# YangHai-1218/RADet

Hardware: AMD Instinct MI355X
Metric: images/sec train-step, r50_ycbv_pbr 640x480 bs=4/GPU (higher is better)
Workload: dtype f32

## Files before the change

### include/radet_hip.h

```cpp
#ifndef RADET_HIP_H
#define RADET_HIP_H
#include <stdint.h>

#ifdef __cplusplus
extern "C" {
#endif


typedef struct RadetConvDesc {
    const float* w;
    const float* bias;
    const float* bn_gamma;
    const float* bn_beta;
    const float* bn_mean;
    const float* bn_var;
    float* wf;
    float* wft;
    float* bias_f;
    const float* dwf_slabs;
    const float* dbias_partials;
    float* dw;
    float* dbias;
    float* dgamma;
    float* dbeta;
// ... 124 lines not shown
                     void* stream);

int radet_gn_workspace_floats(int B, const int* seg_desc, int nseg);
int radet_gn_relu_fwd(const float* z, const float* gamma, const float* beta, float* y, float* stats ,
                      float* partial_ws, int B, int C, int groups, float eps, int relu, const int* seg_desc, int nseg,
                      void* stream);
int radet_gn_relu_bwd(const float* dy, const float* z, const float* stats, const float* gamma, const float* beta,
                      float* dz, float* dgamma, float* dbeta, float* partial_ws, int B, int C, int groups, int relu,
                      const int* seg_desc, int nseg, void* stream);

int radet_upsample_add(float* dst, const float* src, int B, int Ho, int Wo, int Hi, int Wi, int C, void* stream);
int radet_upsample_add_bwd(float* dsrc, const float* ddst, int B, int Ho, int Wo, int Hi, int Wi, int C, void* stream);
int radet_relu_bwd(const float* dy, const float* addend, const float* act, float* dx, size_t n, void* stream);
int radet_stem_conv_bn_relu_h(const float* img_nchw, const float* wf_ohwi, const float* bias, void* y_nhwc, int B, int H,
                              int W, void* stream);
int radet_maxpool3x3s2_h(const void* x, void* y, int B, int H, int W, int C, void* stream);
int radet_gn_relu_fwd_pair(const float* z0, const float* gamma0, const float* beta0, float* y0, float* stats0,
                           float* partial_ws0, const float* z1, const float* gamma1, const float* beta1, float* y1,
                           float* stats1, float* partial_ws1, int B, int C, int groups, float eps, int relu,
                           const int* seg_desc, int nseg, void* stream);
int radet_gn_relu_fwd_pair_h(const void* z0, const float* gamma0, const float* beta0, void* y0, float* stats0,
                             float* partial_ws0, const void* z1, const float* gamma1, const float* beta1, void* y1,
                             float* stats1, float* partial_ws1, int B, int C, int groups, float eps, int relu,
                             const int* seg_desc, int nseg, void* stream);
int radet_gn_relu_fwd_h(const void* z, const float* gamma, const float* beta, void* y, float* stats, float* partial_ws,
                        int B, int C, int groups, float eps, int relu, const int* seg_desc, int nseg, void* stream);
int radet_gn_relu_bwd_h(const void* dy, const void* z, const float* stats, const float* gamma, const float* beta, void* dz,
                        float* dgamma, float* dbeta, float* partial_ws, int B, int C, int groups, int relu,
                        const int* seg_desc, int nseg, void* stream);
int radet_upsample_add_h(void* dst, const void* src, int B, int Ho, int Wo, int Hi, int Wi, int C, void* stream);
int radet_upsample_add_bwd_h(void* dsrc, const void* ddst, int B, int Ho, int Wo, int Hi, int Wi, int C, void* stream);
int radet_relu_bwd_h(const void* dy, const void* addend, const void* act, void* dx, size_t n, void* stream);
int radet_convert_rows(const void* src, void* dst, size_t rows, int ncols, int src_ld, int src_off, int dst_ld,
                       int dst_off, int to_bf16, void* stream);
int radet_split_planes(const float* src, void* dst_planes, size_t rows, int C, int src_ld, void* stream);
int radet_merge_planes(const void* src_planes, float* dst, size_t rows, int C, int dst_ld, void* stream);
int radet_split_pairs(const float* src, void* dst_pairs, size_t rows, int C, int src_ld, const void* src_amax, void* dst_amax,
                      void* stream);
int radet_merge_pairs(const void* src_pairs, float* dst, size_t rows, int C, int dst_ld, const void* amax, void* stream);
int radet_gn_relu_fwd_q(const float* z, const float* gamma, const float* beta, float* y, void* yq, float* stats,
                        float* partial_ws, int B, int C, int groups, float eps, int relu, const int* seg_desc, int nseg,
                        void* stream, void* y_amax, void* yq_amax, void* zhat_amax);
int radet_gn_relu_fwd_pair_q(const float* z0, const float* gamma0, const float* beta0, float* y0, void* yq0, float* stats0,
                             float* partial_ws0, void* y_amax0, void* yq_amax0, void* zhat_amax0, const float* z1,
                             const float* gamma1, const float* beta1, float* y1, void* yq1, float* stats1,
                             float* partial_ws1, void* y_amax1, void* yq_amax1, void* zhat_amax1, int B, int C, int groups,
                             float eps, int relu, const int* seg_desc, int nseg, void* stream);
int radet_gn_relu_bwd_q(const float* dy, const float* z, const float* stats, const float* gamma, const float* beta, float* dz,
                        void* dzq, float* dgamma, float* dbeta, float* partial_ws, int B, int C, int groups, int relu,
                        const int* seg_desc, int nseg, void* stream, const void* dy_amax, const void* zhat_amax,
                        void* dzq_amax);
int radet_maxpool3x3s2_a(const float* x, float* y, int B, int H, int W, int C, void* y_amax, void* stream);
int radet_maxpool3x3s2_q(const float* x, float* y, int B, int H, int W, int C, void* y_amax, void* yq, void* yq_amax,
                         const void* x_amax, void* stream);
int radet_stem_conv_bn_relu_a(const float* img_nchw, const float* wf_ohwi, const float* bias, float* y_nhwc, int B, int H, int W,
                              void* y_amax, void* stream);
int radet_upsample_add_a(float* dst, const float* src, int B, int Ho, int Wo, int Hi, int Wi, int C, void* dst_amax,
                         void* stream);
int radet_upsample_add_bwd_a(float* dsrc, const float* ddst, int B, int Ho, int Wo, int Hi, int Wi, int C, void* dsrc_amax,
                             void* stream);
int radet_relu_bwd_a(const float* dy, const float* addend, const float* act, float* dx, size_t n, void* dx_amax, void* stream);
int radet_absmax(const float* x, size_t n, void* amax, void* stream);
int radet_amax_slot_words(void);
int radet_gn_relu_fwd_p(const float* z, const float* gamma, const float* beta, float* y, void* yp, float* stats,
                        float* partial_ws, int B, int C, int groups, float eps, int relu, const int* seg_desc, int nseg,
                        void* stream);
int radet_gn_relu_fwd_pair_p(const float* z0, const float* gamma0, const float* beta0, float* y0, void* yp0, float* stats0,
                             float* partial_ws0, const float* z1, const float* gamma1, const float* beta1, float* y1,
                             void* yp1, float* stats1, float* partial_ws1, int B, int C, int groups, float eps, int relu,
                             const int* seg_desc, int nseg, void* stream);
int radet_gn_relu_bwd_p(const float* dy, const float* z, const float* stats, const float* gamma, const float* beta,
                        float* dz, void* dzp, float* dgamma, float* dbeta, float* partial_ws, int B, int C, int groups,
                        int relu, const int* seg_desc, int nseg, void* stream);
int radet_nchw_to_nhwc(const float* x, float* y, int B, int C, int H, int W, void* stream);
int radet_nhwc_to_nchw(const float* x, float* y, int B, int C, int H, int W, void* stream);

int radet_head_loss_ws_ints(int R);
int radet_head_loss(const float* cls, const float* reg_u, const float* iou, const float* scales,
                    const float* gt_boxes, const int64_t* gt_labels, const int* gt_off, const int64_t* p2g,
                    const float* pw, const int* level_desc, int nlvl, int B, int num_classes, float alpha,
                    float gamma, float loss_bbox_weight, float giou_eps, const float* grad_scale, float* losses,
                    float* dcls, int dcls_ld, float* dreg_u, int dreg_ld, float* diou, int diou_ld, float* dscales,
                    int64_t* labels_out, float* bbox_targets_out, int flags, int* ws, void* stream);
int radet_scale_relu(const float* reg_u, const float* scales, float* out, const int* level_desc, int nlvl, int B,
                     void* stream);

size_t radet_decode_ws_bytes(int B, int nlvl, int nms_pre);
int radet_decode_candidates(const float* cls, const float* reg_u, const float* iou, const float* scales,
                            const int* level_desc, int nlvl, int B, int num_classes, float score_thr, int nms_pre,
                            const float* img_hw , const float* scale_factor ,
                            float* cand_boxes, float* cand_scores, float* cand_ctr, int64_t* cand_labels,
                            int* cand_count, void* ws, void* stream);

size_t radet_nms_ws_bytes(int B, int cap);
int radet_nms(const float* boxes, const float* cluster_scores, const float* vote_scores, const int64_t* labels,
              const int* counts, int B, int cap, int mode, float iou_thr, int iou_enable, float sigma, int max_out,
              float* out_boxes, float* out_scores, int64_t* out_labels, int* out_count, int64_t* aux0, int64_t* aux1,
              void* ws, void* stream);

size_t radet_assign_ws_bytes(int B, int N);
int radet_assign_points(const float* gt_boxes, const int* gt_off, const uint8_t* masks, int H, int W,
                        const uint32_t* rng_words, int U, const int* level_desc, const float* regress_ranges ,
                        int nlvl, int B, int positive_num, int flags, float neg_threshold, int64_t* p2g, float* pw, int* used,
                        void* ws, void* stream);

int radet_assign_points_f(const float* gt_boxes, const int* gt_off, const float* distance_maps, int H, int W,
                          const uint32_t* rng_words, int U, const int* level_desc, const float* regress_ranges ,
                          int nlvl, int B, int positive_num, int flags, float neg_threshold, int64_t* p2g, float* pw, int* used,
                          void* ws, void* stream);

size_t radet_mbd_ws_bytes(size_t total_px);
int radet_mbd(const uint8_t* images, const int* img_desc_dev, int nimg, const int* seeds_x, const int* seeds_y, float alpha,
              int niter, int base_size, double* dmap, size_t total_px, void* ws, void* stream);
int radet_gdt(const float* cost, const int* img_desc_dev, int nimg, const int* seeds_x, const int* seeds_y, float* dist,
              void* ws_labels , void* stream);

int radet_resize_linear_u8(const uint8_t* src, const int* src_desc, uint8_t* dst, const int* dst_desc, int ncrop,
                           int max_dst_px, int channels, void* stream);
int radet_resize_linear_f(const void* src, const int* src_desc, void* dst, const int* dst_desc, int ncrop, int max_dst_px,
                          int is_f64, void* stream);
#define RESIZE_WIN_DESC_INTS 7
int radet_resize_linear_u8_window(const uint8_t* src, const int* src_desc, uint8_t* dst, const int* win_desc, int ncrop,
                                  int max_dst_px, int channels, void* stream);
#define RESIZE_SRC_WIN_DESC_INTS 8
int radet_resize_linear_u8_src_window(const uint8_t* src, const int* src_desc, uint8_t* dst, const int* win_desc, int ncrop,
                                      int max_dst_px, int channels, void* stream);
int radet_gaussian_blur9_u8(const uint8_t* src, const int* desc, uint8_t* dst, float* tmp, const float* kernel5, int ncrop,
                            int max_px, void* stream);
int radet_sobel_edge(const uint8_t* src, const int* desc, float* edge, uint8_t* gray_ws, uint32_t* max_ws, int ncrop,
                     int max_px, void* stream);

int radet_mask_max(const uint8_t* masks, uint32_t* maxes , int G, size_t hw, void* stream);
int radet_mask_transform(const uint8_t* src, uint8_t* dst, const uint32_t* norm_max, int G, int Hs, int Ws, int Hr, int Wr,
                         int Hd, int Wd, int flip, int pad_val, void* stream);
#define MASK_WIN_INTS 7
int radet_mask_transform_window(const uint8_t* src, uint8_t* dst, const uint32_t* norm_max, const int* win_desc, int G, int Hs,
                                int Ws, int Hd, int Wd, int pad_val, void* stream);
#define MASK_SRC_WIN_INTS 7
int radet_mask_transform_src_window(const uint8_t* src, uint8_t* dst, const uint32_t* norm_max, const int* win_desc, int G, int Hs,
                                    int Ws, int Hd, int Wd, int pad_val, void* stream);

#define RLE_MASK_INTS 5
#define RLE_PART_INTS 2
int radet_rle_masks(const uint32_t* run_ends, int n_ends, const int* part_desc, int n_parts, const int* mask_desc, int G,
                    uint8_t* dst, uint8_t* dst_plain, int Hr, int Wr, int Hd, int Wd, int pad_val, void* stream);
int radet_rle_masks_window(const uint32_t* run_ends, int n_ends, const int* part_desc, int n_parts, const int* mask_desc,
                           const int* win_desc, int G, uint8_t* dst, uint8_t* dst_plain, int Hd, int Wd, int pad_val, void* stream);
int radet_rle_masks_src_window(const uint32_t* run_ends, int n_ends, const int* part_desc, int n_parts, const int* mask_desc,
                               const int* win_desc, int G, uint8_t* dst, uint8_t* dst_plain, int Hd, int Wd, int pad_val,
                               void* stream);

#define JPEG_ROW_INTS 8
#define JPEG_DESC_INTS 20
#define JPEG_HUFF_BYTES 1424
int radet_jpeg_index(const uint8_t* file, int scan_lo, int scan_hi, int ncomp, const int* comp_blocks, const void* huff,
                     int n_mcus, int restart_interval, int seg_mcus, int* rows, int max_rows);
int radet_jpeg_decode(const uint8_t* files, const int* desc, int nimg, const int* wgs, int n_wg, const void* huff,
                      const uint16_t* quant, const int* rows, int n_rows, int16_t* coef, uint8_t* planes, uint8_t* dst,
                      int* err, int max_blocks, int max_px, int stages, void* stream);

#define AUG_PARAM_INTS 16
#define AUG_MAX_W 8192
int radet_augment_merge_hblur(const uint8_t* src, const uint8_t* bg, const int* params, uint8_t* dst, int nimg, int max_h,
                              int max_w, void* stream);
int radet_augment_vblur(const uint8_t* src, const int* params, uint8_t* dst, int nimg, int max_h, int max_w, void* stream);
int radet_augment_sharp(const uint8_t* src, const int* params, uint8_t* dst, unsigned long long* lsum, int nimg, int max_px,
// ... 101 lines not shown
```

### radet_amd/_lib.py

```python
import ctypes as C
import os

_HERE = os.path.dirname(os.path.abspath(__file__))
LIB_PATH = os.path.join(_HERE, os.environ.get("RADET_LIB", "libradet_hip.so"))

_p = C.c_void_p
_i = C.c_int
_f = C.c_float
_sz = C.c_size_t


class RadetConvDesc(C.Structure):
    _fields_ = [("w", _p), ("bias", _p), ("bn_gamma", _p), ("bn_beta", _p), ("bn_mean", _p), ("bn_var", _p),
                ("wf", _p), ("wft", _p), ("bias_f", _p), ("dwf_slabs", _p), ("dbias_partials", _p),
                ("dw", _p), ("dbias", _p), ("dgamma", _p), ("dbeta", _p),
                ("cout", _i), ("cin", _i), ("kh", _i), ("kw", _i), ("nsplit", _i), ("eps", _f),
                ("wft_ld", _i), ("wft_off", _i), ("w16", _i), ("w_amax", _p), ("wfq", _p), ("w_l1", _p), ("bias_amax", _p),
                ("w_l1t", _p)]


class RadetScales(C.Structure):
    _fields_ = [("x_amax", _p), ("w_amax", _p), ("y_amax", _p), ("x1_amax", _p), ("w1_amax", _p), ("y1_amax", _p),
                ("yq", _p), ("yq_amax", _p), ("x_true_amax", _p), ("w_l1", _p), ("bias_amax", _p), ("addend_amax", _p)]


class RadetWgradJob(C.Structure):
    _fields_ = [("dy", _p), ("x", _p), ("slabs", _p), ("dbias_partials", _p), ("gather_table", _p),
                ("M", _i), ("Cin", _i), ("Cout", _i), ("ld_dy", _i), ("KH", _i), ("KW", _i), ("S", _i)]


class RadetTapeOp(C.Structure):
    _fields_ = [("kind", C.c_int32), ("fn", C.c_int32), ("stream", _p), ("event", _p), ("args", C.c_uint64 * 32)]


SIGNATURES = {
    "radet_gather_table_rows": (_i, [_i]),
    "radet_build_gather_table": (_i, [_p, _i, _i, _i, _i, _i, _i, _i, _p, _i, _p]),
    "radet_conv2d_igemm": (_i, [_p, _p, _p, _p, _p, _p, _p, _i, _i, _i, _i, _i, _i, _i, _p, _sz, _p]),
    "radet_conv2d_igemm_pair": (_i, [_p] * 13 + [_i, _i, _i, _i, _i, _i, _i, _p, _sz, _p]),
    "radet_conv2d_igemm_taps": (_i, [_p, _p, _p, _p, _p, _p, _p, _p, _i, _i, _i, _i, _i, _i, _p, _sz, _p]),
    "radet_conv2d_igemm_classes": (_i, [_p, _p, _p, _p, _p, _p, _p, _p, _p, _p, _i, _i, _i, _i, _i, _i, _p, _sz, _p]),
    "radet_conv2d_igemm_s": (_i, [_p, _p, _p, _p, _p, _p, _p, _i, _i, _i, _i, _i, _i, _i, _p, _sz, _p, _p]),
    "radet_conv2d_igemm_pair_s": (_i, [_p] * 13 + [_i, _i, _i, _i, _i, _i, _i, _p, _sz, _p, _p]),
    "radet_conv2d_igemm_taps_s": (_i, [_p, _p, _p, _p, _p, _p, _p, _p, _i, _i, _i, _i, _i, _i, _p, _sz, _p, _p]),
    "radet_conv2d_igemm_classes_s": (_i, [_p, _p, _p, _p, _p, _p, _p, _p, _p, _p, _i, _i, _i, _i, _i, _i, _p, _sz, _p, _p]),
    "radet_conv2d_wgrad_s": (_i, [_p, _p, _p, _p, _p, _i, _i, _i, _i, _i, _i, _i, _i, _p, _p]),
    "radet_split_pairs": (_i, [_p, _p, _sz, _i, _i, _p, _p, _p]),
    "radet_merge_pairs": (_i, [_p, _p, _sz, _i, _i, _p, _p]),
    "radet_gn_relu_fwd_q": (_i, [_p, _p, _p, _p, _p, _p, _p, _i, _i, _i, _f, _i, _p, _i, _p, _p, _p, _p]),
    "radet_gn_relu_fwd_pair_q": (_i, [_p] * 20 + [_i, _i, _i, _f, _i, _p, _i, _p]),
    "radet_gn_relu_bwd_q": (_i, [_p, _p, _p, _p, _p, _p, _p, _p, _p, _p, _i, _i, _i, _i, _p, _i, _p, _p, _p, _p]),
    "radet_maxpool3x3s2_a": (_i, [_p, _p, _i, _i, _i, _i, _p, _p]),
    "radet_maxpool3x3s2_q": (_i, [_p, _p, _i, _i, _i, _i, _p, _p, _p, _p, _p]),
    "radet_stem_conv_bn_relu_a": (_i, [_p, _p, _p, _p, _i, _i, _i, _p, _p]),
    "radet_upsample_add_a": (_i, [_p, _p, _i, _i, _i, _i, _i, _i, _p, _p]),
    "radet_upsample_add_bwd_a": (_i, [_p, _p, _i, _i, _i, _i, _i, _i, _p, _p]),
    "radet_relu_bwd_a": (_i, [_p, _p, _p, _p, _sz, _p, _p]),
    "radet_absmax": (_i, [_p, _sz, _p, _p]),
    "radet_amax_slot_words": (_i, []),
    "radet_pred3x3_patch": (_i, [_p, _i, _p, _i, _p, _p, _p, _i, _p, _p, _p, _i, _p]),
    "radet_conv2d_wgrad_splits": (_i, [_i, _i, _i, _i, _i]),
    "radet_conv2d_wgrad": (_i, [_p, _p, _p, _p, _p, _i, _i, _i, _i, _i, _i, _i, _i, _p]),
    "radet_conv2d_wgrad_group": (_i, [_p, _i, _i, _p]),
    "radet_fold_weights": (_i, [_p, _i, _p]),
    "radet_unfold_grads": (_i, [_p, _i, _i, _p]),
    "radet_stem_conv_bn_relu": (_i, [_p, _p, _p, _p, _i, _i, _i, _p]),
    "radet_maxpool3x3s2": (_i, [_p, _p, _i, _i, _i, _i, _p]),
    "radet_maxpool3x3s2_bwd_relu": (_i, [_p, _p, _p, _i, _i, _i, _i, _p]),
    "radet_stem_wgrad_splits": (_i, [_i, _i, _i]),
    "radet_stem_wgrad": (_i, [_p, _p, _p, _p, _i, _i, _i, _i, _p]),
    "radet_gn_workspace_floats": (_i, [_i, _p, _i]),
    "radet_gn_relu_fwd": (_i, [_p, _p, _p, _p, _p, _p, _i, _i, _i, _f, _i, _p, _i, _p]),
    "radet_gn_relu_fwd_pair": (_i, [_p] * 12 + [_i, _i, _i, _f, _i, _p, _i, _p]),
    "radet_gn_relu_fwd_pair_h": (_i, [_p] * 12 + [_i, _i, _i, _f, _i, _p, _i, _p]),
    "radet_gn_relu_bwd": (_i, [_p, _p, _p, _p, _p, _p, _p, _p, _p, _i, _i, _i, _i, _p, _i, _p]),
    "radet_upsample_add": (_i, [_p, _p, _i, _i, _i, _i, _i, _i, _p]),
    "radet_upsample_add_bwd": (_i, [_p, _p, _i, _i, _i, _i, _i, _i, _p]),
    "radet_relu_bwd": (_i, [_p, _p, _p, _p, _sz, _p]),
    "radet_nchw_to_nhwc": (_i, [_p, _p, _i, _i, _i, _i, _p]),
    "radet_nhwc_to_nchw": (_i, [_p, _p, _i, _i, _i, _i, _p]),
    "radet_head_loss_ws_ints": (_i, [_i]),
    "radet_head_loss": (_i, [_p, _p, _p, _p, _p, _p, _p, _p, _p, _p, _i, _i, _i, _f, _f, _f, _f, _p, _p, _p, _i, _p,
                             _i, _p, _i, _p, _p, _p, _i, _p, _p]),
    "radet_scale_relu": (_i, [_p, _p, _p, _p, _i, _i, _p]),
    "radet_decode_ws_bytes": (_sz, [_i, _i, _i]),
    "radet_decode_candidates": (_i, [_p, _p, _p, _p, _p, _i, _i, _i, _f, _i, _p, _p, _p, _p, _p, _p, _p, _p, _p]),
    "radet_nms_ws_bytes": (_sz, [_i, _i]),
    "radet_nms": (_i, [_p, _p, _p, _p, _p, _i, _i, _i, _f, _i, _f, _i, _p, _p, _p, _p, _p, _p, _p, _p]),
    "radet_assign_ws_bytes": (_sz, [_i, _i]),
    "radet_assign_points": (_i, [_p, _p, _p, _i, _i, _p, _i, _p, _p, _i, _i, _i, _i, _f, _p, _p, _p, _p, _p]),
    "radet_assign_points_f": (_i, [_p, _p, _p, _i, _i, _p, _i, _p, _p, _i, _i, _i, _i, _f, _p, _p, _p, _p, _p]),
    "radet_resize_linear_u8": (_i, [_p, _p, _p, _p, _i, _i, _i, _p]),
    "radet_resize_linear_u8_window": (_i, [_p, _p, _p, _p, _i, _i, _i, _p]),
    "radet_resize_linear_u8_src_window": (_i, [_p, _p, _p, _p, _i, _i, _i, _p]),
    "radet_resize_linear_f": (_i, [_p, _p, _p, _p, _i, _i, _i, _p]),
    "radet_warp_affine_u8": (_i, [_p, _sz, _p, _sz, _p, _i, _i, _i, _p]),
    "radet_gaussian_blur9_u8": (_i, [_p, _p, _p, _p, _p, _i, _i, _p]),
    "radet_sobel_edge": (_i, [_p, _p, _p, _p, _p, _i, _i, _p]),
    "radet_stem_conv_bn_relu_h": (_i, [_p, _p, _p, _p, _i, _i, _i, _p]),
    "radet_maxpool3x3s2_h": (_i, [_p, _p, _i, _i, _i, _i, _p]),
    "radet_gn_relu_fwd_h": (_i, [_p, _p, _p, _p, _p, _p, _i, _i, _i, _f, _i, _p, _i, _p]),
    "radet_gn_relu_bwd_h": (_i, [_p, _p, _p, _p, _p, _p, _p, _p, _p, _i, _i, _i, _i, _p, _i, _p]),
    "radet_upsample_add_h": (_i, [_p, _p, _i, _i, _i, _i, _i, _i, _p]),
    "radet_upsample_add_bwd_h": (_i, [_p, _p, _i, _i, _i, _i, _i, _i, _p]),
    "radet_relu_bwd_h": (_i, [_p, _p, _p, _p, _sz, _p]),
    "radet_convert_rows": (_i, [_p, _p, _sz, _i, _i, _i, _i, _i, _i, _p]),
    "radet_split_planes": (_i, [_p, _p, _sz, _i, _i, _p]),
    "radet_merge_planes": (_i, [_p, _p, _sz, _i, _i, _p]),
    "radet_gn_relu_fwd_p": (_i, [_p, _p, _p, _p, _p, _p, _p, _i, _i, _i, _f, _i, _p, _i, _p]),
    "radet_gn_relu_fwd_pair_p": (_i, [_p] * 14 + [_i, _i, _i, _f, _i, _p, _i, _p]),
    "radet_gn_relu_bwd_p": (_i, [_p, _p, _p, _p, _p, _p, _p, _p, _p, _p, _i, _i, _i, _i, _p, _i, _p]),
    "radet_mbd_ws_bytes": (_sz, [_sz]),
    "radet_mbd": (_i, [_p, _p, _i, _p, _p, _f, _i, _i, _p, _sz, _p, _p]),
    "radet_gdt": (_i, [_p, _p, _i, _p, _p, _p, _p, _p]),
    "radet_mask_max": (_i, [_p, _p, _i, _sz, _p]),
    "radet_mask_transform": (_i, [_p, _p, _p, _i, _i, _i, _i, _i, _i, _i, _i, _i, _p]),
    "radet_mask_transform_window": (_i, [_p, _p, _p, _p, _i, _i, _i, _i, _i, _i, _p]),
    "radet_mask_transform_src_window": (_i, [_p, _p, _p, _p, _i, _i, _i, _i, _i, _i, _p]),
    "radet_rle_masks": (_i, [_p, _i, _p, _i, _p, _i, _p, _p, _i, _i, _i, _i, _i, _p]),
    "radet_rle_masks_window": (_i, [_p, _i, _p, _i, _p, _p, _i, _p, _p, _i, _i, _i, _p]),
    "radet_rle_masks_src_window": (_i, [_p, _i, _p, _i, _p, _p, _i, _p, _p, _i, _i, _i, _p]),
    "radet_jpeg_index": (_i, [_p, _i, _i, _i, _p, _p, _i, _i, _i, _p, _i]),
    "radet_jpeg_decode": (_i, [_p, _p, _i, _p, _i, _p, _p, _p, _i, _p, _p, _p, _p, _i, _i, _i, _p]),
    "radet_augment_merge_hblur": (_i, [_p, _p, _p, _p, _i, _i, _i, _p]),
    "radet_augment_vblur": (_i, [_p, _p, _p, _i, _i, _i, _p]),
    "radet_augment_sharp": (_i, [_p, _p, _p, _p, _i, _i, _p]),
    "radet_augment_finish": (_i, [_p, _p, _p, _p, _i, _i, _i, _f, _f, _f, _f, _f, _f, _p]),
    "radet_augment_hsv_noise": (_i, [_p, _p, _p, _i, _i, _p]),
    "radet_augment_box": (_i, [_p, _p, _p, _sz, _i, _i, _i, _p]),
    "radet_crop_canvases": (_i, [_p, _sz, _p, _p, _i, _p, _i, _i, _p, _sz, _p]),
    "radet_paste_maps": (_i, [_p, _sz, _i, _p, _i, _i, _i, _p, _p]),
    "radet_preprocess_frames": (_i, [_p, _i, _i, _i, _f, _f, _f, _f, _f, _f, _p, _p]),
    "radet_grid_anchors": (_i, [_p, _p, _i, _i, _p]),
    "radet_bbox_overlaps": (_i, [_p, _p, _p, _i, _i, _i, _i, _i, _f, _p]),
    "radet_tblr_encode": (_i, [_p, _p, _p, _i, _p, _i, _p]),
    "radet_tblr_decode": (_i, [_p, _p, _p, _i, _p, _i, _f, _f, _i, _p]),
    "radet_loss_partials": (_i, [_sz]),
    "radet_loss_finalize": (_i, [_p, _i, _p, _f, _p, _p]),
    "radet_sigmoid_focal_loss": (_i, [_p, _p, _p, _i, _sz, _i, _f, _f, _p, _f, _p, _p]),
    "radet_sigmoid_focal_loss_bwd": (_i, [_p, _p, _p, _i, _sz, _i, _f, _f, _p, _p, _p, _f, _p, _p]),
    "radet_bce_logits_loss": (_i, [_p, _p, _p, _i, _sz, _i, _p, _f, _p, _p]),
    "radet_bce_logits_loss_bwd": (_i, [_p, _p, _p, _i, _sz, _i, _p, _p, _p, _f, _p, _p]),
    "radet_giou_loss": (_i, [_p, _p, _p, _sz, _f, _p, _f, _p, _p]),
    "radet_giou_loss_bwd": (_i, [_p, _p, _p, _sz, _f, _p, _p, _p, _f, _p, _p]),
    "radet_threshold_compact": (_i, [_p, _sz, _f, _p, _p, _p]),
    "radet_sqnorm_partials": (_i, [_p, _sz, _p, _i, _p]),
    "radet_adamw_step": (_i, [_p, _p, _p, _p, _sz, _f, _f, _f, _f, _f, _i, _f, _f, _p, _i, _p, _p]),
    "radet_coco_match": (_i, [_p, _p, _p, _p, _p, _p, _i, _i, _p, _i, _p, _i, _p, _p, _p, _p, _p]),
    "radet_coco_accumulate": (_i, [_p, _p, _p, _p, _p, _p, _p, _p, _i, _i, _i, _i, _i, _p, _p, _p, _p]),
    "radet_tape_fn_index": (_i, [C.c_char_p]),
    "radet_tape_replay": (_i, [_p, _i, _i, _p]),
    "radet_fill_zero": (_i, [_p, _sz, _p]),
    "radet_copy_d2d": (_i, [_p, _p, _sz, _p]),
    "radet_stream_create_cumask": (_i, [_p, _i, _p]),
    "radet_copy_segments": (_i, [_p, _i, _i, _p]),
}

_lib = None


class RadetHipError(RuntimeError):
    pass


def load():
    global _lib
# ... 41 lines not shown
```

### radet_amd/csrc/loss.hip

```cpp
#include "common.h"
#include "../../include/radet_hip.h"

struct LossLevels {
    int n;
    int h[RADET_MAX_SEG], w[RADET_MAX_SEG], stride[RADET_MAX_SEG];
    int row_off[RADET_MAX_SEG + 1];
    int pt_off[RADET_MAX_SEG + 1];
};

struct RowInfo { int lvl, n, pix, pt; float cx, cy, stride; };

__device__ __forceinline__ RowInfo decode_row(const LossLevels& L, int r) {
    RowInfo o;
    int l = 0;
#pragma unroll
    for (int i = 1; i < RADET_MAX_SEG; ++i)
        if (i < L.n && r >= L.row_off[i]) l = i;
    const int hw = L.h[l] * L.w[l];
    const int local = r - L.row_off[l];
    o.lvl = l;
    o.n = local / hw;
    o.pix = local - o.n * hw;
    o.pt = L.pt_off[l] + o.pix;
    const int iy = o.pix / L.w[l], ix = o.pix - iy * L.w[l];
// ... 26 lines not shown
        const int G = gt_off[ri.n + 1] - gt_off[ri.n];
        const int64_t g = p2g[(size_t)ri.n * N + ri.pt];
        int64_t lab = num_classes;
        if (G > 0 && g > -1) lab = gt_labels[gt_off[ri.n] + (g == 0 ? G - 1 : (int)g - 1)];
        if (labels_out) labels_out[r] = lab;
        if (tgt_out) {
            float4 t = make_float4(0.f, 0.f, 0.f, 0.f);
            if (G > 0 && g > 0) {
                const float* gb = gt_boxes + (size_t)(gt_off[ri.n] + (int)g - 1) * 4;
                const float hw8 = 8.f * ri.stride;
                t.x = (ri.cy - gb[1]) / hw8 / 0.125f;
                t.y = (gb[3] - ri.cy) / hw8 / 0.125f;
                t.z = (ri.cx - gb[0]) / hw8 / 0.125f;
                t.w = (gb[2] - ri.cx) / hw8 / 0.125f;
            }
            *reinterpret_cast<float4*>(tgt_out + (size_t)r * 4) = t;
        }
        if (lab >= 0 && lab < num_classes) {
            pos = true;
            w = pw[(size_t)ri.n * N + ri.pt];
        }
    }
    const unsigned long long bal = __ballot(pos);
    const int before = __popcll(bal & ((1ull << lane) - 1ull));
    const float wsum = wave_sum(w);
    __shared__ int wc[LP_BLK / 64];
    __shared__ float ww[LP_BLK / 64];
    if (lane == 0) { wc[wave] = __popcll(bal); ww[wave] = wsum; }
    __syncthreads();
    int base = 0;
    for (int i = 0; i < wave; ++i) base += wc[i];
    int* scratch = lp_scratch(ws, R);
    const int nb = lp_blocks(R);
    if (pos) scratch[blockIdx.x * LP_BLK + base + before] = r;
    if (tid == 0) {
        scratch[nb * LP_BLK + blockIdx.x] = (wc[0] + wc[1]) + (wc[2] + wc[3]);
        scratch[nb * LP_BLK + nb + blockIdx.x] = __float_as_int((ww[0] + ww[1]) + (ww[2] + ww[3]));
    }
}

__global__ __launch_bounds__(1024) void loss_prep_scan_kernel(int R, int* __restrict__ ws) {
    const int tid = threadIdx.x;
    const int nb = lp_blocks(R);
    const int* scratch = lp_scratch(ws, R);
    const int* bcnt = scratch + nb * LP_BLK;
    const int* bw = bcnt + nb;
    const int per = (nb + 1023) / 1024;
    const int b0 = tid * per, b1 = min(nb, b0 + per);
    int cnt = 0;
    float wsum = 0.f;
    for (int b = b0; b < b1; ++b) {
        cnt += bcnt[b];
        wsum += __int_as_float(bw[b]);
    }
    __shared__ int scnt[1024];
    __shared__ float swt[1024];
    scnt[tid] = cnt;
    swt[tid] = wsum;
    __syncthreads();
    for (int o = 1; o < 1024; o <<= 1) {
        const int v = tid >= o ? scnt[tid - o] : 0;
        __syncthreads();
        scnt[tid] += v;
        __syncthreads();
    }
    for (int o = 512; o > 0; o >>= 1) {
        if (tid < o) swt[tid] += swt[tid + o];
        __syncthreads();
    }
    int pos = scnt[tid] - cnt;
    for (int b = b0; b < b1; ++b) {
        const int n = bcnt[b];
        for (int i = 0; i < n; ++i) ws[WS_HDR + pos + i] = scratch[b * LP_BLK + i];
        pos += n;
    }
    if (tid == 0) {
        ws[0] = scnt[1023];
        ws[1] = __float_as_int(swt[0]);
    }
}

__device__ __forceinline__ float softplus_f(float x) { return fmaxf(x, 0.f) + log1pf(expf(-fabsf(x))); }

__global__ __launch_bounds__(256) void focal_kernel(const float* __restrict__ cls, const int64_t* __restrict__ gt_labels,
                                                    const int* __restrict__ gt_off, const int64_t* __restrict__ p2g,
                                                    const float* __restrict__ pw, const LossLevels L, int B, int N,
                                                    int R, int C, float alpha, float gamma,
                                                    const float* __restrict__ grad_scale, float* __restrict__ dcls,
                                                    int dcls_ld, int* __restrict__ ws) {
    const float num_pos = __int_as_float(ws[1]);
    const float avg = num_pos + (float)B;
    const float gs = (grad_scale ? grad_scale[0] : 1.f) / avg;
    const size_t total = (size_t)R * C;
    float acc = 0.f;
    for (size_t i = (size_t)blockIdx.x * 256 + threadIdx.x; i < total; i += (size_t)gridDim.x * 256) {
        const int r = (int)(i / C);
        const int c = (int)(i - (size_t)r * C);
        const RowInfo ri = decode_row(L, r);
        const int G = gt_off[ri.n + 1] - gt_off[ri.n];
        const int64_t g = p2g[(size_t)ri.n * N + ri.pt];
        int64_t lab = C;
        if (G > 0 && g > -1) lab = gt_labels[gt_off[ri.n] + (g == 0 ? G - 1 : (int)g - 1)];
        const float wt = pw[(size_t)ri.n * N + ri.pt];
        const float x = cls[i];
        const float p = 1.f / (1.f + expf(-x));
        float loss, dx;
        if (lab == c) {
            const float q = 1.f - p;
            const float logp = -softplus_f(-x);
            const float mod = gamma == 2.f ? q * q : powf(q, gamma);
            loss = -alpha * mod * logp;
            dx = alpha * mod * (gamma * p * logp - q);
        } else {
            const float log1mp = -softplus_f(x);
            const float mod = gamma == 2.f ? p * p : powf(p, gamma);
            loss = -(1.f - alpha) * mod * log1mp;
            dx = (1.f - alpha) * mod * (p - gamma * (1.f - p) * log1mp);
        }
        acc += loss * wt;
        dcls[(size_t)r * dcls_ld + c] = dx * wt * gs;
    }
    __shared__ float red[4];
    acc = wave_sum(acc);
    if ((threadIdx.x & 63) == 0) red[threadIdx.x >> 6] = acc;
    __syncthreads();
    if (threadIdx.x == 0) ws[WS_HDR + R + blockIdx.x] = __float_as_int((red[0] + red[1]) + (red[2] + red[3]));
}

struct PosTerms { float w, one_minus_giou, bce, pwt; };

__device__ __forceinline__ float sel_gt(float a, float b) { return a > b ? 1.f : (a == b ? 0.5f : 0.f); }
__device__ __forceinline__ float sel_lt(float a, float b) { return a < b ? 1.f : (a == b ? 0.5f : 0.f); }

template <int NT>
__device__ __forceinline__ float block_sum(float v, float* red) {
    const int tid = threadIdx.x;
    __syncthreads();
    red[tid] = v;
    __syncthreads();
    for (int o = NT / 2; o > 0; o >>= 1) {
        if (tid < o) red[tid] += red[tid + o];
        __syncthreads();
    }
    const float r = red[0];
    __syncthreads();
    return r;
}

__global__ __launch_bounds__(256) void pos_loss_kernel(const float* __restrict__ reg_u, const float* __restrict__ iou_logit,
                                                       const float* __restrict__ scales,
                                                       const float* __restrict__ gt_boxes,
                                                       const int* __restrict__ gt_off, const int64_t* __restrict__ p2g,
                                                       const float* __restrict__ pw, const LossLevels L, int B, int N,
                                                       int R, float lbw, float eps, const float* __restrict__ grad_scale,
                                                       float* __restrict__ losses, float* __restrict__ dreg_u,
                                                       int dreg_ld, float* __restrict__ diou, int diou_ld,
                                                       float* __restrict__ dscales, const int* __restrict__ ws,
                                                       int n_focal_partials, int postact) {
    __shared__ float red[256];
    const int tid = threadIdx.x;
    const int P = ws[0];
    const float num_pos = __int_as_float(ws[1]);
    {
        double a = 0.0;
        for (int k = tid; k < n_focal_partials; k += 256) a += (double)__int_as_float(ws[WS_HDR + R + k]);
        const float s = block_sum<256>((float)a, red);
        if (tid == 0) losses[0] = s / (num_pos + (float)B);
    }
    if (!(num_pos > 0.f)) {
        if (tid == 0) { losses[1] = 0.f; losses[2] = 0.f; }
        if (tid < L.n) dscales[tid] = 0.f;
        return;
    }
    float sw = 0.f, swl = 0.f, sb = 0.f, sp = 0.f;
    for (int pass = 0; pass < 2; ++pass) {
        float inv_sw = 0.f, inv_sp = 0.f, g1 = 1.f, g2 = 1.f;
        float ds[RADET_MAX_SEG];
#pragma unroll
        for (int l = 0; l < RADET_MAX_SEG; ++l) ds[l] = 0.f;
        if (pass == 1) {
            inv_sw = 1.f / sw;
            inv_sp = 1.f / sp;
            if (grad_scale) { g1 = grad_scale[1]; g2 = grad_scale[2]; }
        }
        for (int k = tid; k < P; k += 256) {
            const int r = ws[WS_HDR + k];
            const RowInfo ri = decode_row(L, r);
            const int64_t g = p2g[(size_t)ri.n * N + ri.pt];
            const float pwt = pw[(size_t)ri.n * N + ri.pt];
            const float sc = scales[ri.lvl];
            const float4 u = *reinterpret_cast<const float4*>(reg_u + (size_t)r * 4);
            const float v0 = u.x * sc, v1 = u.y * sc, v2 = u.z * sc, v3 = u.w * sc;
            const float p0 = postact ? v0 : fmaxf(v0, 0.f), p1 = postact ? v1 : fmaxf(v1, 0.f);
            const float p2 = postact ? v2 : fmaxf(v2, 0.f), p3 = postact ? v3 : fmaxf(v3, 0.f);
            float t0 = 0.f, t1 = 0.f, t2 = 0.f, t3 = 0.f;
            if (g > 0) {
                const float* gb = gt_boxes + (size_t)(gt_off[ri.n] + (int)g - 1) * 4;
                const float hw8 = 8.f * ri.stride;
                t0 = (ri.cy - gb[1]) / hw8 / 0.125f;
                t1 = (gb[3] - ri.cy) / hw8 / 0.125f;
                t2 = (ri.cx - gb[0]) / hw8 / 0.125f;
                t3 = (gb[2] - ri.cx) / hw8 / 0.125f;
            }
            const float hw8 = 8.f * ri.stride;
            const float px1 = ri.cx - p2 * 0.125f * hw8, py1 = ri.cy - p0 * 0.125f * hw8;
            const float px2 = ri.cx + p3 * 0.125f * hw8, py2 = ri.cy + p1 * 0.125f * hw8;
            const float tx1 = ri.cx - t2 * 0.125f * hw8, ty1 = ri.cy - t0 * 0.125f * hw8;
            const float tx2 = ri.cx + t3 * 0.125f * hw8, ty2 = ri.cy + t1 * 0.125f * hw8;
            const float area1 = (px2 - px1) * (py2 - py1), area2 = (tx2 - tx1) * (ty2 - ty1);
            const float ltx = fmaxf(px1, tx1), lty = fmaxf(py1, ty1), rbx = fminf(px2, tx2), rby = fminf(py2, ty2);
            const float dw = rbx - ltx, dh = rby - lty;
            const float iw = fmaxf(dw, 0.f), ih = fmaxf(dh, 0.f);
            const float I = iw * ih;
            const float Uraw = area1 + area2 - I;
            const float U = fmaxf(Uraw, eps);
            const float iou = I / U;
            const float eltx = fminf(px1, tx1), elty = fminf(py1, ty1), erbx = fmaxf(px2, tx2), erby = fmaxf(py2, ty2);
            const float dew = erbx - eltx, deh = erby - elty;
            const float ew = fmaxf(dew, 0.f), eh = fmaxf(deh, 0.f);
            const float Eraw = ew * eh;
            const float E = fmaxf(Eraw, eps);
            const float giou = iou - (E - U) / E;
            const float wgt = fmaxf(iou, 1e-12f) * pwt;
            const float x = iou_logit[r];
            if (pass == 0) {
                sw += wgt;
                swl += wgt * (1.f - giou);
                sb += pwt * (fmaxf(x, 0.f) - x * iou + log1pf(expf(-fabsf(x))));
                sp += pwt;
            } else {
                const float gg = -lbw * wgt * inv_sw * g1;
                const float g_E = -gg * U / (E * E);
                float g_U = gg / E - gg * I / (U * U);
                float g_I = gg / U;
                const float g_Uraw = g_U * sel_gt(Uraw, eps);
                const float g_area1 = g_Uraw;
                g_I -= g_Uraw;
                const float g_dw = g_I * ih * (dw >= 0.f ? 1.f : 0.f);
                const float g_dh = g_I * iw * (dh >= 0.f ? 1.f : 0.f);
                const float g_Eraw = g_E * sel_gt(Eraw, eps);
                const float g_dew = g_Eraw * eh * (dew >= 0.f ? 1.f : 0.f);
                const float g_deh = g_Eraw * ew * (deh >= 0.f ? 1.f : 0.f);
                float gx1 = -g_dw * sel_gt(px1, tx1) - g_dew * sel_lt(px1, tx1) - g_area1 * (py2 - py1);
                float gy1 = -g_dh * sel_gt(py1, ty1) - g_deh * sel_lt(py1, ty1) - g_area1 * (px2 - px1);
                float gx2 = g_dw * sel_lt(px2, tx2) + g_dew * sel_gt(px2, tx2) + g_area1 * (py2 - py1);
                float gy2 = g_dh * sel_lt(py2, ty2) + g_deh * sel_gt(py2, ty2) + g_area1 * (px2 - px1);
                const float k8 = 0.125f * hw8;
                const float gp0 = -gy1 * k8, gp1 = gy2 * k8, gp2 = -gx1 * k8, gp3 = gx2 * k8;
                const float gv0 = (postact || p0 > 0.f) ? gp0 : 0.f, gv1 = (postact || p1 > 0.f) ? gp1 : 0.f;
                const float gv2 = (postact || p2 > 0.f) ? gp2 : 0.f, gv3 = (postact || p3 > 0.f) ? gp3 : 0.f;
                float4 du;
                du.x = gv0 * sc; du.y = gv1 * sc; du.z = gv2 * sc; du.w = gv3 * sc;
                *reinterpret_cast<float4*>(dreg_u + (size_t)r * dreg_ld) = du;
                const float dsv = (gv0 * u.x + gv1 * u.y) + (gv2 * u.z + gv3 * u.w);
#pragma unroll
                for (int l = 0; l < RADET_MAX_SEG; ++l)
                    if (l == ri.lvl) ds[l] += dsv;
                const float sig = 1.f / (1.f + expf(-x));
                diou[(size_t)r * diou_ld] = pwt * (sig - iou) * inv_sp * g2;
            }
        }
        if (pass == 0) {
            sw = block_sum<256>(sw, red);
            swl = block_sum<256>(swl, red);
            sb = block_sum<256>(sb, red);
            sp = block_sum<256>(sp, red);
            if (tid == 0) {
                losses[1] = lbw * swl / sw;
                losses[2] = sb / sp;
            }
        } else {
#pragma unroll
            for (int l = 0; l < RADET_MAX_SEG; ++l) {
                if (l < L.n) {
                    const float s = block_sum<256>(ds[l], red);
                    if (tid == 0) dscales[l] = s;
                }
            }
        }
    }
}

__global__ void zero_sparse_kernel(float* __restrict__ dreg, int dreg_ld, float* __restrict__ diou, int diou_ld, int R) {
    const int r = blockIdx.x * blockDim.x + threadIdx.x;
    if (r < R) {
        *reinterpret_cast<float4*>(dreg + (size_t)r * dreg_ld) = make_float4(0.f, 0.f, 0.f, 0.f);
        diou[(size_t)r * diou_ld] = 0.f;
    }
}

static int fill_levels(LossLevels* L, const int* level_desc, int nlvl, int B) {
    if (nlvl < 1 || nlvl > RADET_MAX_SEG) return RADET_ERR_ARG;
    L->n = nlvl;
    int row = 0, pt = 0;
    for (int l = 0; l < nlvl; ++l) {
        L->h[l] = level_desc[3 * l];
        L->w[l] = level_desc[3 * l + 1];
        L->stride[l] = level_desc[3 * l + 2];
        L->row_off[l] = row;
        L->pt_off[l] = pt;
        row += B * L->h[l] * L->w[l];
        pt += L->h[l] * L->w[l];
    }
    L->row_off[nlvl] = row;
    L->pt_off[nlvl] = pt;
    for (int l = nlvl; l < RADET_MAX_SEG; ++l) { L->h[l] = 1; L->w[l] = 1; L->stride[l] = 1; }
    return RADET_OK;
}

#define FOCAL_BLOCKS 1024

static_assert(FOCAL_BLOCKS == 1024, "lp_scratch() hard-codes the focal partial count");
extern "C" int radet_head_loss_ws_ints(int R) {
    const int nb = (R + LP_BLK - 1) / LP_BLK;
    return WS_HDR + R + FOCAL_BLOCKS + 16 + nb * LP_BLK + 2 * nb;
}

extern "C" int radet_head_loss(const float* cls, const float* reg_u, const float* iou, const float* scales,
                               const float* gt_boxes, const int64_t* gt_labels, const int* gt_off, const int64_t* p2g,
                               const float* pw, const int* level_desc, int nlvl, int B, int num_classes, float alpha,
                               float gamma, float loss_bbox_weight, float giou_eps, const float* grad_scale,
                               float* losses, float* dcls, int dcls_ld, float* dreg_u, int dreg_ld, float* diou,
                               int diou_ld, float* dscales, int64_t* labels_out, float* bbox_targets_out, int flags,
                               int* ws, void* stream) {
    LossLevels L;
    int rc = fill_levels(&L, level_desc, nlvl, B);
    if (rc) return rc;
    const int R = L.row_off[nlvl], N = L.pt_off[nlvl];
    if (dcls_ld < num_classes || dreg_ld < 4 || (dreg_ld & 3) || diou_ld < 1) return RADET_ERR_ARG;
    hipStream_t st = (hipStream_t)stream;
    hipLaunchKernelGGL(loss_prep_rows_kernel, dim3((R + LP_BLK - 1) / LP_BLK), dim3(LP_BLK), 0, st, gt_labels, gt_boxes,
                       gt_off, p2g, pw, L, B, N, R, num_classes, labels_out, bbox_targets_out, ws);
    hipLaunchKernelGGL(loss_prep_scan_kernel, dim3(1), dim3(1024), 0, st, R, ws);
    const size_t total = (size_t)R * num_classes;
    int fb = (int)((total + 255) / 256);
    if (fb > FOCAL_BLOCKS) fb = FOCAL_BLOCKS;
    hipLaunchKernelGGL(focal_kernel, dim3(fb), dim3(256), 0, st, cls, gt_labels, gt_off, p2g, pw, L, B, N, R, num_classes,
                       alpha, gamma, grad_scale, dcls, dcls_ld, ws);
    hipLaunchKernelGGL(zero_sparse_kernel, dim3((R + 255) / 256), dim3(256), 0, st, dreg_u, dreg_ld, diou, diou_ld, R);
    hipLaunchKernelGGL(pos_loss_kernel, dim3(1), dim3(256), 0, st, reg_u, iou, scales, gt_boxes, gt_off, p2g, pw, L, B, N,
                       R, loss_bbox_weight, giou_eps, grad_scale, losses, dreg_u, dreg_ld, diou, diou_ld, dscales, ws,
                       fb, flags & 1);
    return radet_check_launch();
}

__global__ void scale_relu_kernel(const float4* __restrict__ u, const float* __restrict__ scales, float4* __restrict__ out,
                                  const LossLevels L, int R) {
    for (int r = blockIdx.x * blockDim.x + threadIdx.x; r < R; r += gridDim.x * blockDim.x) {
        int l = 0;
#pragma unroll
        for (int i = 1; i < RADET_MAX_SEG; ++i)
            if (i < L.n && r >= L.row_off[i]) l = i;
        const float s = scales[l];
        const float4 v = u[r];
        out[r] = make_float4(fmaxf(v.x * s, 0.f), fmaxf(v.y * s, 0.f), fmaxf(v.z * s, 0.f), fmaxf(v.w * s, 0.f));
    }
}

extern "C" int radet_scale_relu(const float* reg_u, const float* scales, float* out, const int* level_desc, int nlvl,
                                int B, void* stream) {
    LossLevels L;
    int rc = fill_levels(&L, level_desc, nlvl, B);
    if (rc) return rc;
    const int R = L.row_off[nlvl];
    hipLaunchKernelGGL(scale_relu_kernel, dim3((R + 255) / 256), dim3(256), 0, (hipStream_t)stream, (const float4*)reg_u,
                       scales, (float4*)out, L, R);
    return radet_check_launch();
}

__global__ void anchors_kernel(float4* __restrict__ out, const LossLevels L, int base_scale) {
    const int N = L.pt_off[L.n];
    for (int p = blockIdx.x * blockDim.x + threadIdx.x; p < N; p += gridDim.x * blockDim.x) {
        int l = 0;
#pragma unroll
        for (int i = 1; i < RADET_MAX_SEG; ++i)
            if (i < L.n && p >= L.pt_off[i]) l = i;
        const int pix = p - L.pt_off[l];
        const int iy = pix / L.w[l], ix = pix - iy * L.w[l];
        const float half = 0.5f * (float)(base_scale * L.stride[l]);
        const float cx = (float)(ix * L.stride[l]), cy = (float)(iy * L.stride[l]);
        out[p] = make_float4(cx - half, cy - half, cx + half, cy + half);
    }
}

extern "C" int radet_grid_anchors(float* out, const int* level_desc, int nlvl, int octave_base_scale, void* stream) {
    LossLevels L;
    int rc = fill_levels(&L, level_desc, nlvl, 1);
    if (rc) return rc;
    const int N = L.pt_off[nlvl];
    hipLaunchKernelGGL(anchors_kernel, dim3((N + 255) / 256), dim3(256), 0, (hipStream_t)stream, (float4*)out, L,
                       octave_base_scale);
    return radet_check_launch();
}
```

### radet_amd/csrc/tape_thunks.c

```c
#include <stdint.h>
#include <stddef.h>
#include <string.h>
#include "radet_hip.h"

static float f32(uint64_t w) { uint32_t u = (uint32_t)w; float f; memcpy(&f, &u, 4); return f; }

static int t_radet_absmax(const uint64_t* a) { return radet_absmax((void*)(uintptr_t)a[0], (size_t)a[1], (void*)(uintptr_t)a[2], (void*)(uintptr_t)a[3]); }
static int t_radet_adamw_step(const uint64_t* a) { return radet_adamw_step((void*)(uintptr_t)a[0], (void*)(uintptr_t)a[1], (void*)(uintptr_t)a[2], (void*)(uintptr_t)a[3], (size_t)a[4], f32(a[5]), f32(a[6]), f32(a[7]), f32(a[8]), f32(a[9]), (int)(int64_t)a[10], f32(a[11]), f32(a[12]), (void*)(uintptr_t)a[13], (int)(int64_t)a[14], (void*)(uintptr_t)a[15], (void*)(uintptr_t)a[16]); }
static int t_radet_amax_slot_words(const uint64_t* a) { (void)a; return radet_amax_slot_words(); }
static int t_radet_assign_points(const uint64_t* a) { return radet_assign_points((void*)(uintptr_t)a[0], (void*)(uintptr_t)a[1], (void*)(uintptr_t)a[2], (int)(int64_t)a[3], (int)(int64_t)a[4], (void*)(uintptr_t)a[5], (int)(int64_t)a[6], (void*)(uintptr_t)a[7], (void*)(uintptr_t)a[8], (int)(int64_t)a[9], (int)(int64_t)a[10], (int)(int64_t)a[11], (int)(int64_t)a[12], f32(a[13]), (void*)(uintptr_t)a[14], (void*)(uintptr_t)a[15], (void*)(uintptr_t)a[16], (void*)(uintptr_t)a[17], (void*)(uintptr_t)a[18]); }
static int t_radet_assign_points_f(const uint64_t* a) { return radet_assign_points_f((void*)(uintptr_t)a[0], (void*)(uintptr_t)a[1], (void*)(uintptr_t)a[2], (int)(int64_t)a[3], (int)(int64_t)a[4], (void*)(uintptr_t)a[5], (int)(int64_t)a[6], (void*)(uintptr_t)a[7], (void*)(uintptr_t)a[8], (int)(int64_t)a[9], (int)(int64_t)a[10], (int)(int64_t)a[11], (int)(int64_t)a[12], f32(a[13]), (void*)(uintptr_t)a[14], (void*)(uintptr_t)a[15], (void*)(uintptr_t)a[16], (void*)(uintptr_t)a[17], (void*)(uintptr_t)a[18]); }
static int t_radet_augment_box(const uint64_t* a) { return radet_augment_box((void*)(uintptr_t)a[0], (void*)(uintptr_t)a[1], (void*)(uintptr_t)a[2], (size_t)a[3], (int)(int64_t)a[4], (int)(int64_t)a[5], (int)(int64_t)a[6], (void*)(uintptr_t)a[7]); }
static int t_radet_augment_finish(const uint64_t* a) { return radet_augment_finish((void*)(uintptr_t)a[0], (void*)(uintptr_t)a[1], (void*)(uintptr_t)a[2], (void*)(uintptr_t)a[3], (int)(int64_t)a[4], (int)(int64_t)a[5], (int)(int64_t)a[6], f32(a[7]), f32(a[8]), f32(a[9]), f32(a[10]), f32(a[11]), f32(a[12]), (void*)(uintptr_t)a[13]); }
static int t_radet_augment_hsv_noise(const uint64_t* a) { return radet_augment_hsv_noise((void*)(uintptr_t)a[0], (void*)(uintptr_t)a[1], (void*)(uintptr_t)a[2], (int)(int64_t)a[3], (int)(int64_t)a[4], (void*)(uintptr_t)a[5]); }
static int t_radet_augment_merge_hblur(const uint64_t* a) { return radet_augment_merge_hblur((void*)(uintptr_t)a[0], (void*)(uintptr_t)a[1], (void*)(uintptr_t)a[2], (void*)(uintptr_t)a[3], (int)(int64_t)a[4], (int)(int64_t)a[5], (int)(int64_t)a[6], (void*)(uintptr_t)a[7]); }
static int t_radet_augment_sharp(const uint64_t* a) { return radet_augment_sharp((void*)(uintptr_t)a[0], (void*)(uintptr_t)a[1], (void*)(uintptr_t)a[2], (void*)(uintptr_t)a[3], (int)(int64_t)a[4], (int)(int64_t)a[5], (void*)(uintptr_t)a[6]); }
static int t_radet_augment_vblur(const uint64_t* a) { return radet_augment_vblur((void*)(uintptr_t)a[0], (void*)(uintptr_t)a[1], (void*)(uintptr_t)a[2], (int)(int64_t)a[3], (int)(int64_t)a[4], (int)(int64_t)a[5], (void*)(uintptr_t)a[6]); }
static int t_radet_bbox_overlaps(const uint64_t* a) { return radet_bbox_overlaps((void*)(uintptr_t)a[0], (void*)(uintptr_t)a[1], (void*)(uintptr_t)a[2], (int)(int64_t)a[3], (int)(int64_t)a[4], (int)(int64_t)a[5], (int)(int64_t)a[6], (int)(int64_t)a[7], f32(a[8]), (void*)(uintptr_t)a[9]); }
static int t_radet_bce_logits_loss(const uint64_t* a) { return radet_bce_logits_loss((void*)(uintptr_t)a[0], (void*)(uintptr_t)a[1], (void*)(uintptr_t)a[2], (int)(int64_t)a[3], (size_t)a[4], (int)(int64_t)a[5], (void*)(uintptr_t)a[6], f32(a[7]), (void*)(uintptr_t)a[8], (void*)(uintptr_t)a[9]); }
static int t_radet_bce_logits_loss_bwd(const uint64_t* a) { return radet_bce_logits_loss_bwd((void*)(uintptr_t)a[0], (void*)(uintptr_t)a[1], (void*)(uintptr_t)a[2], (int)(int64_t)a[3], (size_t)a[4], (int)(int64_t)a[5], (void*)(uintptr_t)a[6], (void*)(uintptr_t)a[7], (void*)(uintptr_t)a[8], f32(a[9]), (void*)(uintptr_t)a[10], (void*)(uintptr_t)a[11]); }
static int t_radet_build_gather_table(const uint64_t* a) { return radet_build_gather_table((void*)(uintptr_t)a[0], (int)(int64_t)a[1], (int)(int64_t)a[2], (int)(int64_t)a[3], (int)(int64_t)a[4], (int)(int64_t)a[5], (int)(int64_t)a[6], (int)(int64_t)a[7], (void*)(uintptr_t)a[8], (int)(int64_t)a[9], (void*)(uintptr_t)a[10]); }
static int t_radet_coco_accumulate(const uint64_t* a) { return radet_coco_accumulate((void*)(uintptr_t)a[0], (void*)(uintptr_t)a[1], (void*)(uintptr_t)a[2], (void*)(uintptr_t)a[3], (void*)(uintptr_t)a[4], (void*)(uintptr_t)a[5], (void*)(uintptr_t)a[6], (void*)(uintptr_t)a[7], (int)(int64_t)a[8], (int)(int64_t)a[9], (int)(int64_t)a[10], (int)(int64_t)a[11], (int)(int64_t)a[12], (void*)(uintptr_t)a[13], (void*)(uintptr_t)a[14], (void*)(uintptr_t)a[15], (void*)(uintptr_t)a[16]); }
static int t_radet_coco_match(const uint64_t* a) { return radet_coco_match((void*)(uintptr_t)a[0], (void*)(uintptr_t)a[1], (void*)(uintptr_t)a[2], (void*)(uintptr_t)a[3], (void*)(uintptr_t)a[4], (void*)(uintptr_t)a[5], (int)(int64_t)a[6], (int)(int64_t)a[7], (void*)(uintptr_t)a[8], (int)(int64_t)a[9], (void*)(uintptr_t)a[10], (int)(int64_t)a[11], (void*)(uintptr_t)a[12], (void*)(uintptr_t)a[13], (void*)(uintptr_t)a[14], (void*)(uintptr_t)a[15], (void*)(uintptr_t)a[16]); }
static int t_radet_conv2d_igemm(const uint64_t* a) { return radet_conv2d_igemm((void*)(uintptr_t)a[0], (void*)(uintptr_t)a[1], (void*)(uintptr_t)a[2], (void*)(uintptr_t)a[3], (void*)(uintptr_t)a[4], (void*)(uintptr_t)a[5], (void*)(uintptr_t)a[6], (int)(int64_t)a[7], (int)(int64_t)a[8], (int)(int64_t)a[9], (int)(int64_t)a[10], (int)(int64_t)a[11], (int)(int64_t)a[12], (int)(int64_t)a[13], (void*)(uintptr_t)a[14], (size_t)a[15], (void*)(uintptr_t)a[16]); }
static int t_radet_conv2d_igemm_classes(const uint64_t* a) { return radet_conv2d_igemm_classes((void*)(uintptr_t)a[0], (void*)(uintptr_t)a[1], (void*)(uintptr_t)a[2], (void*)(uintptr_t)a[3], (void*)(uintptr_t)a[4], (void*)(uintptr_t)a[5], (void*)(uintptr_t)a[6], (void*)(uintptr_t)a[7], (void*)(uintptr_t)a[8], (void*)(uintptr_t)a[9], (int)(int64_t)a[10], (int)(int64_t)a[11], (int)(int64_t)a[12], (int)(int64_t)a[13], (int)(int64_t)a[14], (int)(int64_t)a[15], (void*)(uintptr_t)a[16], (size_t)a[17], (void*)(uintptr_t)a[18]); }
static int t_radet_conv2d_igemm_classes_s(const uint64_t* a) { return radet_conv2d_igemm_classes_s((void*)(uintptr_t)a[0], (void*)(uintptr_t)a[1], (void*)(uintptr_t)a[2], (void*)(uintptr_t)a[3], (void*)(uintptr_t)a[4], (void*)(uintptr_t)a[5], (void*)(uintptr_t)a[6], (void*)(uintptr_t)a[7], (void*)(uintptr_t)a[8], (void*)(uintptr_t)a[9], (int)(int64_t)a[10], (int)(int64_t)a[11], (int)(int64_t)a[12], (int)(int64_t)a[13], (int)(int64_t)a[14], (int)(int64_t)a[15], (void*)(uintptr_t)a[16], (size_t)a[17], (void*)(uintptr_t)a[18], (void*)(uintptr_t)a[19]); }
static int t_radet_conv2d_igemm_pair(const uint64_t* a) { return radet_conv2d_igemm_pair((void*)(uintptr_t)a[0], (void*)(uintptr_t)a[1], (void*)(uintptr_t)a[2], (void*)(uintptr_t)a[3], (void*)(uintptr_t)a[4], (void*)(uintptr_t)a[5], (void*)(uintptr_t)a[6], (void*)(uintptr_t)a[7], (void*)(uintptr_t)a[8], (void*)(uintptr_t)a[9], (void*)(uintptr_t)a[10], (void*)(uintptr_t)a[11], (void*)(uintptr_t)a[12], (int)(int64_t)a[13], (int)(int64_t)a[14], (int)(int64_t)a[15], (int)(int64_t)a[16], (int)(int64_t)a[17], (int)(int64_t)a[18], (int)(int64_t)a[19], (void*)(uintptr_t)a[20], (size_t)a[21], (void*)(uintptr_t)a[22]); }
static int t_radet_conv2d_igemm_pair_s(const uint64_t* a) { return radet_conv2d_igemm_pair_s((void*)(uintptr_t)a[0], (void*)(uintptr_t)a[1], (void*)(uintptr_t)a[2], (void*)(uintptr_t)a[3], (void*)(uintptr_t)a[4], (void*)(uintptr_t)a[5], (void*)(uintptr_t)a[6], (void*)(uintptr_t)a[7], (void*)(uintptr_t)a[8], (void*)(uintptr_t)a[9], (void*)(uintptr_t)a[10], (void*)(uintptr_t)a[11], (void*)(uintptr_t)a[12], (int)(int64_t)a[13], (int)(int64_t)a[14], (int)(int64_t)a[15], (int)(int64_t)a[16], (int)(int64_t)a[17], (int)(int64_t)a[18], (int)(int64_t)a[19], (void*)(uintptr_t)a[20], (size_t)a[21], (void*)(uintptr_t)a[22], (void*)(uintptr_t)a[23]); }
static int t_radet_conv2d_igemm_s(const uint64_t* a) { return radet_conv2d_igemm_s((void*)(uintptr_t)a[0], (void*)(uintptr_t)a[1], (void*)(uintptr_t)a[2], (void*)(uintptr_t)a[3], (void*)(uintptr_t)a[4], (void*)(uintptr_t)a[5], (void*)(uintptr_t)a[6], (int)(int64_t)a[7], (int)(int64_t)a[8], (int)(int64_t)a[9], (int)(int64_t)a[10], (int)(int64_t)a[11], (int)(int64_t)a[12], (int)(int64_t)a[13], (void*)(uintptr_t)a[14], (size_t)a[15], (void*)(uintptr_t)a[16], (void*)(uintptr_t)a[17]); }
static int t_radet_conv2d_igemm_taps(const uint64_t* a) { return radet_conv2d_igemm_taps((void*)(uintptr_t)a[0], (void*)(uintptr_t)a[1], (void*)(uintptr_t)a[2], (void*)(uintptr_t)a[3], (void*)(uintptr_t)a[4], (void*)(uintptr_t)a[5], (void*)(uintptr_t)a[6], (void*)(uintptr_t)a[7], (int)(int64_t)a[8], (int)(int64_t)a[9], (int)(int64_t)a[10], (int)(int64_t)a[11], (int)(int64_t)a[12], (int)(int64_t)a[13], (void*)(uintptr_t)a[14], (size_t)a[15], (void*)(uintptr_t)a[16]); }
static int t_radet_conv2d_igemm_taps_s(const uint64_t* a) { return radet_conv2d_igemm_taps_s((void*)(uintptr_t)a[0], (void*)(uintptr_t)a[1], (void*)(uintptr_t)a[2], (void*)(uintptr_t)a[3], (void*)(uintptr_t)a[4], (void*)(uintptr_t)a[5], (void*)(uintptr_t)a[6], (void*)(uintptr_t)a[7], (int)(int64_t)a[8], (int)(int64_t)a[9], (int)(int64_t)a[10], (int)(int64_t)a[11], (int)(int64_t)a[12], (int)(int64_t)a[13], (void*)(uintptr_t)a[14], (size_t)a[15], (void*)(uintptr_t)a[16], (void*)(uintptr_t)a[17]); }
static int t_radet_conv2d_wgrad(const uint64_t* a) { return radet_conv2d_wgrad((void*)(uintptr_t)a[0], (void*)(uintptr_t)a[1], (void*)(uintptr_t)a[2], (void*)(uintptr_t)a[3], (void*)(uintptr_t)a[4], (int)(int64_t)a[5], (int)(int64_t)a[6], (int)(int64_t)a[7], (int)(int64_t)a[8], (int)(int64_t)a[9], (int)(int64_t)a[10], (int)(int64_t)a[11], (int)(int64_t)a[12], (void*)(uintptr_t)a[13]); }
static int t_radet_conv2d_wgrad_group(const uint64_t* a) { return radet_conv2d_wgrad_group((void*)(uintptr_t)a[0], (int)(int64_t)a[1], (int)(int64_t)a[2], (void*)(uintptr_t)a[3]); }
static int t_radet_conv2d_wgrad_s(const uint64_t* a) { return radet_conv2d_wgrad_s((void*)(uintptr_t)a[0], (void*)(uintptr_t)a[1], (void*)(uintptr_t)a[2], (void*)(uintptr_t)a[3], (void*)(uintptr_t)a[4], (int)(int64_t)a[5], (int)(int64_t)a[6], (int)(int64_t)a[7], (int)(int64_t)a[8], (int)(int64_t)a[9], (int)(int64_t)a[10], (int)(int64_t)a[11], (int)(int64_t)a[12], (void*)(uintptr_t)a[13], (void*)(uintptr_t)a[14]); }
static int t_radet_conv2d_wgrad_splits(const uint64_t* a) { return radet_conv2d_wgrad_splits((int)(int64_t)a[0], (int)(int64_t)a[1], (int)(int64_t)a[2], (int)(int64_t)a[3], (int)(int64_t)a[4]); }
static int t_radet_convert_rows(const uint64_t* a) { return radet_convert_rows((void*)(uintptr_t)a[0], (void*)(uintptr_t)a[1], (size_t)a[2], (int)(int64_t)a[3], (int)(int64_t)a[4], (int)(int64_t)a[5], (int)(int64_t)a[6], (int)(int64_t)a[7], (int)(int64_t)a[8], (void*)(uintptr_t)a[9]); }
static int t_radet_copy_d2d(const uint64_t* a) { return radet_copy_d2d((void*)(uintptr_t)a[0], (void*)(uintptr_t)a[1], (size_t)a[2], (void*)(uintptr_t)a[3]); }
static int t_radet_copy_segments(const uint64_t* a) { return radet_copy_segments((void*)(uintptr_t)a[0], (int)(int64_t)a[1], (int)(int64_t)a[2], (void*)(uintptr_t)a[3]); }
static int t_radet_crop_canvases(const uint64_t* a) { return radet_crop_canvases((void*)(uintptr_t)a[0], (size_t)a[1], (void*)(uintptr_t)a[2], (void*)(uintptr_t)a[3], (int)(int64_t)a[4], (void*)(uintptr_t)a[5], (int)(int64_t)a[6], (int)(int64_t)a[7], (void*)(uintptr_t)a[8], (size_t)a[9], (void*)(uintptr_t)a[10]); }
static int t_radet_decode_candidates(const uint64_t* a) { return radet_decode_candidates((void*)(uintptr_t)a[0], (void*)(uintptr_t)a[1], (void*)(uintptr_t)a[2], (void*)(uintptr_t)a[3], (void*)(uintptr_t)a[4], (int)(int64_t)a[5], (int)(int64_t)a[6], (int)(int64_t)a[7], f32(a[8]), (int)(int64_t)a[9], (void*)(uintptr_t)a[10], (void*)(uintptr_t)a[11], (void*)(uintptr_t)a[12], (void*)(uintptr_t)a[13], (void*)(uintptr_t)a[14], (void*)(uintptr_t)a[15], (void*)(uintptr_t)a[16], (void*)(uintptr_t)a[17], (void*)(uintptr_t)a[18]); }
static int t_radet_fill_zero(const uint64_t* a) { return radet_fill_zero((void*)(uintptr_t)a[0], (size_t)a[1], (void*)(uintptr_t)a[2]); }
static int t_radet_fold_weights(const uint64_t* a) { return radet_fold_weights((void*)(uintptr_t)a[0], (int)(int64_t)a[1], (void*)(uintptr_t)a[2]); }
static int t_radet_gather_table_rows(const uint64_t* a) { return radet_gather_table_rows((int)(int64_t)a[0]); }
static int t_radet_gaussian_blur9_u8(const uint64_t* a) { return radet_gaussian_blur9_u8((void*)(uintptr_t)a[0], (void*)(uintptr_t)a[1], (void*)(uintptr_t)a[2], (void*)(uintptr_t)a[3], (void*)(uintptr_t)a[4], (int)(int64_t)a[5], (int)(int64_t)a[6], (void*)(uintptr_t)a[7]); }
static int t_radet_gdt(const uint64_t* a) { return radet_gdt((void*)(uintptr_t)a[0], (void*)(uintptr_t)a[1], (int)(int64_t)a[2], (void*)(uintptr_t)a[3], (void*)(uintptr_t)a[4], (void*)(uintptr_t)a[5], (void*)(uintptr_t)a[6], (void*)(uintptr_t)a[7]); }
static int t_radet_giou_loss(const uint64_t* a) { return radet_giou_loss((void*)(uintptr_t)a[0], (void*)(uintptr_t)a[1], (void*)(uintptr_t)a[2], (size_t)a[3], f32(a[4]), (void*)(uintptr_t)a[5], f32(a[6]), (void*)(uintptr_t)a[7], (void*)(uintptr_t)a[8]); }
static int t_radet_giou_loss_bwd(const uint64_t* a) { return radet_giou_loss_bwd((void*)(uintptr_t)a[0], (void*)(uintptr_t)a[1], (void*)(uintptr_t)a[2], (size_t)a[3], f32(a[4]), (void*)(uintptr_t)a[5], (void*)(uintptr_t)a[6], (void*)(uintptr_t)a[7], f32(a[8]), (void*)(uintptr_t)a[9], (void*)(uintptr_t)a[10]); }
static int t_radet_gn_relu_bwd(const uint64_t* a) { return radet_gn_relu_bwd((void*)(uintptr_t)a[0], (void*)(uintptr_t)a[1], (void*)(uintptr_t)a[2], (void*)(uintptr_t)a[3], (void*)(uintptr_t)a[4], (void*)(uintptr_t)a[5], (void*)(uintptr_t)a[6], (void*)(uintptr_t)a[7], (void*)(uintptr_t)a[8], (int)(int64_t)a[9], (int)(int64_t)a[10], (int)(int64_t)a[11], (int)(int64_t)a[12], (void*)(uintptr_t)a[13], (int)(int64_t)a[14], (void*)(uintptr_t)a[15]); }
static int t_radet_gn_relu_bwd_h(const uint64_t* a) { return radet_gn_relu_bwd_h((void*)(uintptr_t)a[0], (void*)(uintptr_t)a[1], (void*)(uintptr_t)a[2], (void*)(uintptr_t)a[3], (void*)(uintptr_t)a[4], (void*)(uintptr_t)a[5], (void*)(uintptr_t)a[6], (void*)(uintptr_t)a[7], (void*)(uintptr_t)a[8], (int)(int64_t)a[9], (int)(int64_t)a[10], (int)(int64_t)a[11], (int)(int64_t)a[12], (void*)(uintptr_t)a[13], (int)(int64_t)a[14], (void*)(uintptr_t)a[15]); }
static int t_radet_gn_relu_bwd_p(const uint64_t* a) { return radet_gn_relu_bwd_p((void*)(uintptr_t)a[0], (void*)(uintptr_t)a[1], (void*)(uintptr_t)a[2], (void*)(uintptr_t)a[3], (void*)(uintptr_t)a[4], (void*)(uintptr_t)a[5], (void*)(uintptr_t)a[6], (void*)(uintptr_t)a[7], (void*)(uintptr_t)a[8], (void*)(uintptr_t)a[9], (int)(int64_t)a[10], (int)(int64_t)a[11], (int)(int64_t)a[12], (int)(int64_t)a[13], (void*)(uintptr_t)a[14], (int)(int64_t)a[15], (void*)(uintptr_t)a[16]); }
static int t_radet_gn_relu_bwd_q(const uint64_t* a) { return radet_gn_relu_bwd_q((void*)(uintptr_t)a[0], (void*)(uintptr_t)a[1], (void*)(uintptr_t)a[2], (void*)(uintptr_t)a[3], (void*)(uintptr_t)a[4], (void*)(uintptr_t)a[5], (void*)(uintptr_t)a[6], (void*)(uintptr_t)a[7], (void*)(uintptr_t)a[8], (void*)(uintptr_t)a[9], (int)(int64_t)a[10], (int)(int64_t)a[11], (int)(int64_t)a[12], (int)(int64_t)a[13], (void*)(uintptr_t)a[14], (int)(int64_t)a[15], (void*)(uintptr_t)a[16], (void*)(uintptr_t)a[17], (void*)(uintptr_t)a[18], (void*)(uintptr_t)a[19]); }
static int t_radet_gn_relu_fwd(const uint64_t* a) { return radet_gn_relu_fwd((void*)(uintptr_t)a[0], (void*)(uintptr_t)a[1], (void*)(uintptr_t)a[2], (void*)(uintptr_t)a[3], (void*)(uintptr_t)a[4], (void*)(uintptr_t)a[5], (int)(int64_t)a[6], (int)(int64_t)a[7], (int)(int64_t)a[8], f32(a[9]), (int)(int64_t)a[10], (void*)(uintptr_t)a[11], (int)(int64_t)a[12], (void*)(uintptr_t)a[13]); }
static int t_radet_gn_relu_fwd_h(const uint64_t* a) { return radet_gn_relu_fwd_h((void*)(uintptr_t)a[0], (void*)(uintptr_t)a[1], (void*)(uintptr_t)a[2], (void*)(uintptr_t)a[3], (void*)(uintptr_t)a[4], (void*)(uintptr_t)a[5], (int)(int64_t)a[6], (int)(int64_t)a[7], (int)(int64_t)a[8], f32(a[9]), (int)(int64_t)a[10], (void*)(uintptr_t)a[11], (int)(int64_t)a[12], (void*)(uintptr_t)a[13]); }
static int t_radet_gn_relu_fwd_p(const uint64_t* a) { return radet_gn_relu_fwd_p((void*)(uintptr_t)a[0], (void*)(uintptr_t)a[1], (void*)(uintptr_t)a[2], (void*)(uintptr_t)a[3], (void*)(uintptr_t)a[4], (void*)(uintptr_t)a[5], (void*)(uintptr_t)a[6], (int)(int64_t)a[7], (int)(int64_t)a[8], (int)(int64_t)a[9], f32(a[10]), (int)(int64_t)a[11], (void*)(uintptr_t)a[12], (int)(int64_t)a[13], (void*)(uintptr_t)a[14]); }
static int t_radet_gn_relu_fwd_pair(const uint64_t* a) { return radet_gn_relu_fwd_pair((void*)(uintptr_t)a[0], (void*)(uintptr_t)a[1], (void*)(uintptr_t)a[2], (void*)(uintptr_t)a[3], (void*)(uintptr_t)a[4], (void*)(uintptr_t)a[5], (void*)(uintptr_t)a[6], (void*)(uintptr_t)a[7], (void*)(uintptr_t)a[8], (void*)(uintptr_t)a[9], (void*)(uintptr_t)a[10], (void*)(uintptr_t)a[11], (int)(int64_t)a[12], (int)(int64_t)a[13], (int)(int64_t)a[14], f32(a[15]), (int)(int64_t)a[16], (void*)(uintptr_t)a[17], (int)(int64_t)a[18], (void*)(uintptr_t)a[19]); }
static int t_radet_gn_relu_fwd_pair_h(const uint64_t* a) { return radet_gn_relu_fwd_pair_h((void*)(uintptr_t)a[0], (void*)(uintptr_t)a[1], (void*)(uintptr_t)a[2], (void*)(uintptr_t)a[3], (void*)(uintptr_t)a[4], (void*)(uintptr_t)a[5], (void*)(uintptr_t)a[6], (void*)(uintptr_t)a[7], (void*)(uintptr_t)a[8], (void*)(uintptr_t)a[9], (void*)(uintptr_t)a[10], (void*)(uintptr_t)a[11], (int)(int64_t)a[12], (int)(int64_t)a[13], (int)(int64_t)a[14], f32(a[15]), (int)(int64_t)a[16], (void*)(uintptr_t)a[17], (int)(int64_t)a[18], (void*)(uintptr_t)a[19]); }
static int t_radet_gn_relu_fwd_pair_p(const uint64_t* a) { return radet_gn_relu_fwd_pair_p((void*)(uintptr_t)a[0], (void*)(uintptr_t)a[1], (void*)(uintptr_t)a[2], (void*)(uintptr_t)a[3], (void*)(uintptr_t)a[4], (void*)(uintptr_t)a[5], (void*)(uintptr_t)a[6], (void*)(uintptr_t)a[7], (void*)(uintptr_t)a[8], (void*)(uintptr_t)a[9], (void*)(uintptr_t)a[10], (void*)(uintptr_t)a[11], (void*)(uintptr_t)a[12], (void*)(uintptr_t)a[13], (int)(int64_t)a[14], (int)(int64_t)a[15], (int)(int64_t)a[16], f32(a[17]), (int)(int64_t)a[18], (void*)(uintptr_t)a[19], (int)(int64_t)a[20], (void*)(uintptr_t)a[21]); }
static int t_radet_gn_relu_fwd_pair_q(const uint64_t* a) { return radet_gn_relu_fwd_pair_q((void*)(uintptr_t)a[0], (void*)(uintptr_t)a[1], (void*)(uintptr_t)a[2], (void*)(uintptr_t)a[3], (void*)(uintptr_t)a[4], (void*)(uintptr_t)a[5], (void*)(uintptr_t)a[6], (void*)(uintptr_t)a[7], (void*)(uintptr_t)a[8], (void*)(uintptr_t)a[9], (void*)(uintptr_t)a[10], (void*)(uintptr_t)a[11], (void*)(uintptr_t)a[12], (void*)(uintptr_t)a[13], (void*)(uintptr_t)a[14], (void*)(uintptr_t)a[15], (void*)(uintptr_t)a[16], (void*)(uintptr_t)a[17], (void*)(uintptr_t)a[18], (void*)(uintptr_t)a[19], (int)(int64_t)a[20], (int)(int64_t)a[21], (int)(int64_t)a[22], f32(a[23]), (int)(int64_t)a[24], (void*)(uintptr_t)a[25], (int)(int64_t)a[26], (void*)(uintptr_t)a[27]); }
static int t_radet_gn_relu_fwd_q(const uint64_t* a) { return radet_gn_relu_fwd_q((void*)(uintptr_t)a[0], (void*)(uintptr_t)a[1], (void*)(uintptr_t)a[2], (void*)(uintptr_t)a[3], (void*)(uintptr_t)a[4], (void*)(uintptr_t)a[5], (void*)(uintptr_t)a[6], (int)(int64_t)a[7], (int)(int64_t)a[8], (int)(int64_t)a[9], f32(a[10]), (int)(int64_t)a[11], (void*)(uintptr_t)a[12], (int)(int64_t)a[13], (void*)(uintptr_t)a[14], (void*)(uintptr_t)a[15], (void*)(uintptr_t)a[16], (void*)(uintptr_t)a[17]); }
static int t_radet_gn_workspace_floats(const uint64_t* a) { return radet_gn_workspace_floats((int)(int64_t)a[0], (void*)(uintptr_t)a[1], (int)(int64_t)a[2]); }
static int t_radet_grid_anchors(const uint64_t* a) { return radet_grid_anchors((void*)(uintptr_t)a[0], (void*)(uintptr_t)a[1], (int)(int64_t)a[2], (int)(int64_t)a[3], (void*)(uintptr_t)a[4]); }
static int t_radet_head_loss(const uint64_t* a) { return radet_head_loss((void*)(uintptr_t)a[0], (void*)(uintptr_t)a[1], (void*)(uintptr_t)a[2], (void*)(uintptr_t)a[3], (void*)(uintptr_t)a[4], (void*)(uintptr_t)a[5], (void*)(uintptr_t)a[6], (void*)(uintptr_t)a[7], (void*)(uintptr_t)a[8], (void*)(uintptr_t)a[9], (int)(int64_t)a[10], (int)(int64_t)a[11], (int)(int64_t)a[12], f32(a[13]), f32(a[14]), f32(a[15]), f32(a[16]), (void*)(uintptr_t)a[17], (void*)(uintptr_t)a[18], (void*)(uintptr_t)a[19], (int)(int64_t)a[20], (void*)(uintptr_t)a[21], (int)(int64_t)a[22], (void*)(uintptr_t)a[23], (int)(int64_t)a[24], (void*)(uintptr_t)a[25], (void*)(uintptr_t)a[26], (void*)(uintptr_t)a[27], (int)(int64_t)a[28], (void*)(uintptr_t)a[29], (void*)(uintptr_t)a[30]); }
static int t_radet_head_loss_ws_ints(const uint64_t* a) { return radet_head_loss_ws_ints((int)(int64_t)a[0]); }
static int t_radet_jpeg_decode(const uint64_t* a) { return radet_jpeg_decode((void*)(uintptr_t)a[0], (void*)(uintptr_t)a[1], (int)(int64_t)a[2], (void*)(uintptr_t)a[3], (int)(int64_t)a[4], (void*)(uintptr_t)a[5], (void*)(uintptr_t)a[6], (void*)(uintptr_t)a[7], (int)(int64_t)a[8], (void*)(uintptr_t)a[9], (void*)(uintptr_t)a[10], (void*)(uintptr_t)a[11], (void*)(uintptr_t)a[12], (int)(int64_t)a[13], (int)(int64_t)a[14], (int)(int64_t)a[15], (void*)(uintptr_t)a[16]); }
static int t_radet_jpeg_index(const uint64_t* a) { return radet_jpeg_index((void*)(uintptr_t)a[0], (int)(int64_t)a[1], (int)(int64_t)a[2], (int)(int64_t)a[3], (void*)(uintptr_t)a[4], (void*)(uintptr_t)a[5], (int)(int64_t)a[6], (int)(int64_t)a[7], (int)(int64_t)a[8], (void*)(uintptr_t)a[9], (int)(int64_t)a[10]); }
static int t_radet_loss_finalize(const uint64_t* a) { return radet_loss_finalize((void*)(uintptr_t)a[0], (int)(int64_t)a[1], (void*)(uintptr_t)a[2], f32(a[3]), (void*)(uintptr_t)a[4], (void*)(uintptr_t)a[5]); }
static int t_radet_loss_partials(const uint64_t* a) { return radet_loss_partials((size_t)a[0]); }
static int t_radet_mask_max(const uint64_t* a) { return radet_mask_max((void*)(uintptr_t)a[0], (void*)(uintptr_t)a[1], (int)(int64_t)a[2], (size_t)a[3], (void*)(uintptr_t)a[4]); }
static int t_radet_mask_transform(const uint64_t* a) { return radet_mask_transform((void*)(uintptr_t)a[0], (void*)(uintptr_t)a[1], (void*)(uintptr_t)a[2], (int)(int64_t)a[3], (int)(int64_t)a[4], (int)(int64_t)a[5], (int)(int64_t)a[6], (int)(int64_t)a[7], (int)(int64_t)a[8], (int)(int64_t)a[9], (int)(int64_t)a[10], (int)(int64_t)a[11], (void*)(uintptr_t)a[12]); }
static int t_radet_mask_transform_src_window(const uint64_t* a) { return radet_mask_transform_src_window((void*)(uintptr_t)a[0], (void*)(uintptr_t)a[1], (void*)(uintptr_t)a[2], (void*)(uintptr_t)a[3], (int)(int64_t)a[4], (int)(int64_t)a[5], (int)(int64_t)a[6], (int)(int64_t)a[7], (int)(int64_t)a[8], (int)(int64_t)a[9], (void*)(uintptr_t)a[10]); }
static int t_radet_mask_transform_window(const uint64_t* a) { return radet_mask_transform_window((void*)(uintptr_t)a[0], (void*)(uintptr_t)a[1], (void*)(uintptr_t)a[2], (void*)(uintptr_t)a[3], (int)(int64_t)a[4], (int)(int64_t)a[5], (int)(int64_t)a[6], (int)(int64_t)a[7], (int)(int64_t)a[8], (int)(int64_t)a[9], (void*)(uintptr_t)a[10]); }
static int t_radet_maxpool3x3s2(const uint64_t* a) { return radet_maxpool3x3s2((void*)(uintptr_t)a[0], (void*)(uintptr_t)a[1], (int)(int64_t)a[2], (int)(int64_t)a[3], (int)(int64_t)a[4], (int)(int64_t)a[5], (void*)(uintptr_t)a[6]); }
static int t_radet_maxpool3x3s2_a(const uint64_t* a) { return radet_maxpool3x3s2_a((void*)(uintptr_t)a[0], (void*)(uintptr_t)a[1], (int)(int64_t)a[2], (int)(int64_t)a[3], (int)(int64_t)a[4], (int)(int64_t)a[5], (void*)(uintptr_t)a[6], (void*)(uintptr_t)a[7]); }
static int t_radet_maxpool3x3s2_bwd_relu(const uint64_t* a) { return radet_maxpool3x3s2_bwd_relu((void*)(uintptr_t)a[0], (void*)(uintptr_t)a[1], (void*)(uintptr_t)a[2], (int)(int64_t)a[3], (int)(int64_t)a[4], (int)(int64_t)a[5], (int)(int64_t)a[6], (void*)(uintptr_t)a[7]); }
static int t_radet_maxpool3x3s2_h(const uint64_t* a) { return radet_maxpool3x3s2_h((void*)(uintptr_t)a[0], (void*)(uintptr_t)a[1], (int)(int64_t)a[2], (int)(int64_t)a[3], (int)(int64_t)a[4], (int)(int64_t)a[5], (void*)(uintptr_t)a[6]); }
static int t_radet_maxpool3x3s2_q(const uint64_t* a) { return radet_maxpool3x3s2_q((void*)(uintptr_t)a[0], (void*)(uintptr_t)a[1], (int)(int64_t)a[2], (int)(int64_t)a[3], (int)(int64_t)a[4], (int)(int64_t)a[5], (void*)(uintptr_t)a[6], (void*)(uintptr_t)a[7], (void*)(uintptr_t)a[8], (void*)(uintptr_t)a[9], (void*)(uintptr_t)a[10]); }
static int t_radet_mbd(const uint64_t* a) { return radet_mbd((void*)(uintptr_t)a[0], (void*)(uintptr_t)a[1], (int)(int64_t)a[2], (void*)(uintptr_t)a[3], (void*)(uintptr_t)a[4], f32(a[5]), (int)(int64_t)a[6], (int)(int64_t)a[7], (void*)(uintptr_t)a[8], (size_t)a[9], (void*)(uintptr_t)a[10], (void*)(uintptr_t)a[11]); }
static int t_radet_merge_pairs(const uint64_t* a) { return radet_merge_pairs((void*)(uintptr_t)a[0], (void*)(uintptr_t)a[1], (size_t)a[2], (int)(int64_t)a[3], (int)(int64_t)a[4], (void*)(uintptr_t)a[5], (void*)(uintptr_t)a[6]); }
static int t_radet_merge_planes(const uint64_t* a) { return radet_merge_planes((void*)(uintptr_t)a[0], (void*)(uintptr_t)a[1], (size_t)a[2], (int)(int64_t)a[3], (int)(int64_t)a[4], (void*)(uintptr_t)a[5]); }
static int t_radet_nchw_to_nhwc(const uint64_t* a) { return radet_nchw_to_nhwc((void*)(uintptr_t)a[0], (void*)(uintptr_t)a[1], (int)(int64_t)a[2], (int)(int64_t)a[3], (int)(int64_t)a[4], (int)(int64_t)a[5], (void*)(uintptr_t)a[6]); }
static int t_radet_nhwc_to_nchw(const uint64_t* a) { return radet_nhwc_to_nchw((void*)(uintptr_t)a[0], (void*)(uintptr_t)a[1], (int)(int64_t)a[2], (int)(int64_t)a[3], (int)(int64_t)a[4], (int)(int64_t)a[5], (void*)(uintptr_t)a[6]); }
static int t_radet_nms(const uint64_t* a) { return radet_nms((void*)(uintptr_t)a[0], (void*)(uintptr_t)a[1], (void*)(uintptr_t)a[2], (void*)(uintptr_t)a[3], (void*)(uintptr_t)a[4], (int)(int64_t)a[5], (int)(int64_t)a[6], (int)(int64_t)a[7], f32(a[8]), (int)(int64_t)a[9], f32(a[10]), (int)(int64_t)a[11], (void*)(uintptr_t)a[12], (void*)(uintptr_t)a[13], (void*)(uintptr_t)a[14], (void*)(uintptr_t)a[15], (void*)(uintptr_t)a[16], (void*)(uintptr_t)a[17], (void*)(uintptr_t)a[18], (void*)(uintptr_t)a[19]); }
static int t_radet_paste_maps(const uint64_t* a) { return radet_paste_maps((void*)(uintptr_t)a[0], (size_t)a[1], (int)(int64_t)a[2], (void*)(uintptr_t)a[3], (int)(int64_t)a[4], (int)(int64_t)a[5], (int)(int64_t)a[6], (void*)(uintptr_t)a[7], (void*)(uintptr_t)a[8]); }
static int t_radet_pred3x3_patch(const uint64_t* a) { return radet_pred3x3_patch((void*)(uintptr_t)a[0], (int)(int64_t)a[1], (void*)(uintptr_t)a[2], (int)(int64_t)a[3], (void*)(uintptr_t)a[4], (void*)(uintptr_t)a[5], (void*)(uintptr_t)a[6], (int)(int64_t)a[7], (void*)(uintptr_t)a[8], (void*)(uintptr_t)a[9], (void*)(uintptr_t)a[10], (int)(int64_t)a[11], (void*)(uintptr_t)a[12]); }
static int t_radet_preprocess_frames(const uint64_t* a) { return radet_preprocess_frames((void*)(uintptr_t)a[0], (int)(int64_t)a[1], (int)(int64_t)a[2], (int)(int64_t)a[3], f32(a[4]), f32(a[5]), f32(a[6]), f32(a[7]), f32(a[8]), f32(a[9]), (void*)(uintptr_t)a[10], (void*)(uintptr_t)a[11]); }
static int t_radet_relu_bwd(const uint64_t* a) { return radet_relu_bwd((void*)(uintptr_t)a[0], (void*)(uintptr_t)a[1], (void*)(uintptr_t)a[2], (void*)(uintptr_t)a[3], (size_t)a[4], (void*)(uintptr_t)a[5]); }
static int t_radet_relu_bwd_a(const uint64_t* a) { return radet_relu_bwd_a((void*)(uintptr_t)a[0], (void*)(uintptr_t)a[1], (void*)(uintptr_t)a[2], (void*)(uintptr_t)a[3], (size_t)a[4], (void*)(uintptr_t)a[5], (void*)(uintptr_t)a[6]); }
static int t_radet_relu_bwd_h(const uint64_t* a) { return radet_relu_bwd_h((void*)(uintptr_t)a[0], (void*)(uintptr_t)a[1], (void*)(uintptr_t)a[2], (void*)(uintptr_t)a[3], (size_t)a[4], (void*)(uintptr_t)a[5]); }
static int t_radet_resize_linear_f(const uint64_t* a) { return radet_resize_linear_f((void*)(uintptr_t)a[0], (void*)(uintptr_t)a[1], (void*)(uintptr_t)a[2], (void*)(uintptr_t)a[3], (int)(int64_t)a[4], (int)(int64_t)a[5], (int)(int64_t)a[6], (void*)(uintptr_t)a[7]); }
static int t_radet_resize_linear_u8(const uint64_t* a) { return radet_resize_linear_u8((void*)(uintptr_t)a[0], (void*)(uintptr_t)a[1], (void*)(uintptr_t)a[2], (void*)(uintptr_t)a[3], (int)(int64_t)a[4], (int)(int64_t)a[5], (int)(int64_t)a[6], (void*)(uintptr_t)a[7]); }
static int t_radet_resize_linear_u8_src_window(const uint64_t* a) { return radet_resize_linear_u8_src_window((void*)(uintptr_t)a[0], (void*)(uintptr_t)a[1], (void*)(uintptr_t)a[2], (void*)(uintptr_t)a[3], (int)(int64_t)a[4], (int)(int64_t)a[5], (int)(int64_t)a[6], (void*)(uintptr_t)a[7]); }
static int t_radet_resize_linear_u8_window(const uint64_t* a) { return radet_resize_linear_u8_window((void*)(uintptr_t)a[0], (void*)(uintptr_t)a[1], (void*)(uintptr_t)a[2], (void*)(uintptr_t)a[3], (int)(int64_t)a[4], (int)(int64_t)a[5], (int)(int64_t)a[6], (void*)(uintptr_t)a[7]); }
static int t_radet_rle_masks(const uint64_t* a) { return radet_rle_masks((void*)(uintptr_t)a[0], (int)(int64_t)a[1], (void*)(uintptr_t)a[2], (int)(int64_t)a[3], (void*)(uintptr_t)a[4], (int)(int64_t)a[5], (void*)(uintptr_t)a[6], (void*)(uintptr_t)a[7], (int)(int64_t)a[8], (int)(int64_t)a[9], (int)(int64_t)a[10], (int)(int64_t)a[11], (int)(int64_t)a[12], (void*)(uintptr_t)a[13]); }
static int t_radet_rle_masks_src_window(const uint64_t* a) { return radet_rle_masks_src_window((void*)(uintptr_t)a[0], (int)(int64_t)a[1], (void*)(uintptr_t)a[2], (int)(int64_t)a[3], (void*)(uintptr_t)a[4], (void*)(uintptr_t)a[5], (int)(int64_t)a[6], (void*)(uintptr_t)a[7], (void*)(uintptr_t)a[8], (int)(int64_t)a[9], (int)(int64_t)a[10], (int)(int64_t)a[11], (void*)(uintptr_t)a[12]); }
static int t_radet_rle_masks_window(const uint64_t* a) { return radet_rle_masks_window((void*)(uintptr_t)a[0], (int)(int64_t)a[1], (void*)(uintptr_t)a[2], (int)(int64_t)a[3], (void*)(uintptr_t)a[4], (void*)(uintptr_t)a[5], (int)(int64_t)a[6], (void*)(uintptr_t)a[7], (void*)(uintptr_t)a[8], (int)(int64_t)a[9], (int)(int64_t)a[10], (int)(int64_t)a[11], (void*)(uintptr_t)a[12]); }
static int t_radet_scale_relu(const uint64_t* a) { return radet_scale_relu((void*)(uintptr_t)a[0], (void*)(uintptr_t)a[1], (void*)(uintptr_t)a[2], (void*)(uintptr_t)a[3], (int)(int64_t)a[4], (int)(int64_t)a[5], (void*)(uintptr_t)a[6]); }
static int t_radet_sigmoid_focal_loss(const uint64_t* a) { return radet_sigmoid_focal_loss((void*)(uintptr_t)a[0], (void*)(uintptr_t)a[1], (void*)(uintptr_t)a[2], (int)(int64_t)a[3], (size_t)a[4], (int)(int64_t)a[5], f32(a[6]), f32(a[7]), (void*)(uintptr_t)a[8], f32(a[9]), (void*)(uintptr_t)a[10], (void*)(uintptr_t)a[11]); }
static int t_radet_sigmoid_focal_loss_bwd(const uint64_t* a) { return radet_sigmoid_focal_loss_bwd((void*)(uintptr_t)a[0], (void*)(uintptr_t)a[1], (void*)(uintptr_t)a[2], (int)(int64_t)a[3], (size_t)a[4], (int)(int64_t)a[5], f32(a[6]), f32(a[7]), (void*)(uintptr_t)a[8], (void*)(uintptr_t)a[9], (void*)(uintptr_t)a[10], f32(a[11]), (void*)(uintptr_t)a[12], (void*)(uintptr_t)a[13]); }
static int t_radet_sobel_edge(const uint64_t* a) { return radet_sobel_edge((void*)(uintptr_t)a[0], (void*)(uintptr_t)a[1], (void*)(uintptr_t)a[2], (void*)(uintptr_t)a[3], (void*)(uintptr_t)a[4], (int)(int64_t)a[5], (int)(int64_t)a[6], (void*)(uintptr_t)a[7]); }
static int t_radet_split_pairs(const uint64_t* a) { return radet_split_pairs((void*)(uintptr_t)a[0], (void*)(uintptr_t)a[1], (size_t)a[2], (int)(int64_t)a[3], (int)(int64_t)a[4], (void*)(uintptr_t)a[5], (void*)(uintptr_t)a[6], (void*)(uintptr_t)a[7]); }
static int t_radet_split_planes(const uint64_t* a) { return radet_split_planes((void*)(uintptr_t)a[0], (void*)(uintptr_t)a[1], (size_t)a[2], (int)(int64_t)a[3], (int)(int64_t)a[4], (void*)(uintptr_t)a[5]); }
static int t_radet_sqnorm_partials(const uint64_t* a) { return radet_sqnorm_partials((void*)(uintptr_t)a[0], (size_t)a[1], (void*)(uintptr_t)a[2], (int)(int64_t)a[3], (void*)(uintptr_t)a[4]); }
static int t_radet_stem_conv_bn_relu(const uint64_t* a) { return radet_stem_conv_bn_relu((void*)(uintptr_t)a[0], (void*)(uintptr_t)a[1], (void*)(uintptr_t)a[2], (void*)(uintptr_t)a[3], (int)(int64_t)a[4], (int)(int64_t)a[5], (int)(int64_t)a[6], (void*)(uintptr_t)a[7]); }
static int t_radet_stem_conv_bn_relu_a(const uint64_t* a) { return radet_stem_conv_bn_relu_a((void*)(uintptr_t)a[0], (void*)(uintptr_t)a[1], (void*)(uintptr_t)a[2], (void*)(uintptr_t)a[3], (int)(int64_t)a[4], (int)(int64_t)a[5], (int)(int64_t)a[6], (void*)(uintptr_t)a[7], (void*)(uintptr_t)a[8]); }
static int t_radet_stem_conv_bn_relu_h(const uint64_t* a) { return radet_stem_conv_bn_relu_h((void*)(uintptr_t)a[0], (void*)(uintptr_t)a[1], (void*)(uintptr_t)a[2], (void*)(uintptr_t)a[3], (int)(int64_t)a[4], (int)(int64_t)a[5], (int)(int64_t)a[6], (void*)(uintptr_t)a[7]); }
static int t_radet_stem_wgrad(const uint64_t* a) { return radet_stem_wgrad((void*)(uintptr_t)a[0], (void*)(uintptr_t)a[1], (void*)(uintptr_t)a[2], (void*)(uintptr_t)a[3], (int)(int64_t)a[4], (int)(int64_t)a[5], (int)(int64_t)a[6], (int)(int64_t)a[7], (void*)(uintptr_t)a[8]); }
static int t_radet_stem_wgrad_splits(const uint64_t* a) { return radet_stem_wgrad_splits((int)(int64_t)a[0], (int)(int64_t)a[1], (int)(int64_t)a[2]); }
static int t_radet_stream_create_cumask(const uint64_t* a) { return radet_stream_create_cumask((void*)(uintptr_t)a[0], (int)(int64_t)a[1], (void*)(uintptr_t)a[2]); }
static int t_radet_tblr_decode(const uint64_t* a) { return radet_tblr_decode((void*)(uintptr_t)a[0], (void*)(uintptr_t)a[1], (void*)(uintptr_t)a[2], (int)(int64_t)a[3], (void*)(uintptr_t)a[4], (int)(int64_t)a[5], f32(a[6]), f32(a[7]), (int)(int64_t)a[8], (void*)(uintptr_t)a[9]); }
static int t_radet_tblr_encode(const uint64_t* a) { return radet_tblr_encode((void*)(uintptr_t)a[0], (void*)(uintptr_t)a[1], (void*)(uintptr_t)a[2], (int)(int64_t)a[3], (void*)(uintptr_t)a[4], (int)(int64_t)a[5], (void*)(uintptr_t)a[6]); }
static int t_radet_threshold_compact(const uint64_t* a) { return radet_threshold_compact((void*)(uintptr_t)a[0], (size_t)a[1], f32(a[2]), (void*)(uintptr_t)a[3], (void*)(uintptr_t)a[4], (void*)(uintptr_t)a[5]); }
static int t_radet_unfold_grads(const uint64_t* a) { return radet_unfold_grads((void*)(uintptr_t)a[0], (int)(int64_t)a[1], (int)(int64_t)a[2], (void*)(uintptr_t)a[3]); }
static int t_radet_upsample_add(const uint64_t* a) { return radet_upsample_add((void*)(uintptr_t)a[0], (void*)(uintptr_t)a[1], (int)(int64_t)a[2], (int)(int64_t)a[3], (int)(int64_t)a[4], (int)(int64_t)a[5], (int)(int64_t)a[6], (int)(int64_t)a[7], (void*)(uintptr_t)a[8]); }
static int t_radet_upsample_add_a(const uint64_t* a) { return radet_upsample_add_a((void*)(uintptr_t)a[0], (void*)(uintptr_t)a[1], (int)(int64_t)a[2], (int)(int64_t)a[3], (int)(int64_t)a[4], (int)(int64_t)a[5], (int)(int64_t)a[6], (int)(int64_t)a[7], (void*)(uintptr_t)a[8], (void*)(uintptr_t)a[9]); }
static int t_radet_upsample_add_bwd(const uint64_t* a) { return radet_upsample_add_bwd((void*)(uintptr_t)a[0], (void*)(uintptr_t)a[1], (int)(int64_t)a[2], (int)(int64_t)a[3], (int)(int64_t)a[4], (int)(int64_t)a[5], (int)(int64_t)a[6], (int)(int64_t)a[7], (void*)(uintptr_t)a[8]); }
static int t_radet_upsample_add_bwd_a(const uint64_t* a) { return radet_upsample_add_bwd_a((void*)(uintptr_t)a[0], (void*)(uintptr_t)a[1], (int)(int64_t)a[2], (int)(int64_t)a[3], (int)(int64_t)a[4], (int)(int64_t)a[5], (int)(int64_t)a[6], (int)(int64_t)a[7], (void*)(uintptr_t)a[8], (void*)(uintptr_t)a[9]); }
static int t_radet_upsample_add_bwd_h(const uint64_t* a) { return radet_upsample_add_bwd_h((void*)(uintptr_t)a[0], (void*)(uintptr_t)a[1], (int)(int64_t)a[2], (int)(int64_t)a[3], (int)(int64_t)a[4], (int)(int64_t)a[5], (int)(int64_t)a[6], (int)(int64_t)a[7], (void*)(uintptr_t)a[8]); }
static int t_radet_upsample_add_h(const uint64_t* a) { return radet_upsample_add_h((void*)(uintptr_t)a[0], (void*)(uintptr_t)a[1], (int)(int64_t)a[2], (int)(int64_t)a[3], (int)(int64_t)a[4], (int)(int64_t)a[5], (int)(int64_t)a[6], (int)(int64_t)a[7], (void*)(uintptr_t)a[8]); }
static int t_radet_warp_affine_u8(const uint64_t* a) { return radet_warp_affine_u8((void*)(uintptr_t)a[0], (size_t)a[1], (void*)(uintptr_t)a[2], (size_t)a[3], (void*)(uintptr_t)a[4], (int)(int64_t)a[5], (int)(int64_t)a[6], (int)(int64_t)a[7], (void*)(uintptr_t)a[8]); }

typedef int (*radet_thunk_fn)(const uint64_t*);
const struct RadetTapeThunk { const char* name; radet_thunk_fn fn; int nargs; } radet_tape_thunks[] = {
    {"radet_absmax", t_radet_absmax, 4},
    {"radet_adamw_step", t_radet_adamw_step, 17},
    {"radet_amax_slot_words", t_radet_amax_slot_words, 0},
    {"radet_assign_points", t_radet_assign_points, 19},
    {"radet_assign_points_f", t_radet_assign_points_f, 19},
    {"radet_augment_box", t_radet_augment_box, 8},
    {"radet_augment_finish", t_radet_augment_finish, 14},
    {"radet_augment_hsv_noise", t_radet_augment_hsv_noise, 6},
    {"radet_augment_merge_hblur", t_radet_augment_merge_hblur, 8},
    {"radet_augment_sharp", t_radet_augment_sharp, 7},
    {"radet_augment_vblur", t_radet_augment_vblur, 7},
    {"radet_bbox_overlaps", t_radet_bbox_overlaps, 10},
    {"radet_bce_logits_loss", t_radet_bce_logits_loss, 10},
    {"radet_bce_logits_loss_bwd", t_radet_bce_logits_loss_bwd, 12},
    {"radet_build_gather_table", t_radet_build_gather_table, 11},
    {"radet_coco_accumulate", t_radet_coco_accumulate, 17},
    {"radet_coco_match", t_radet_coco_match, 17},
    {"radet_conv2d_igemm", t_radet_conv2d_igemm, 17},
    {"radet_conv2d_igemm_classes", t_radet_conv2d_igemm_classes, 19},
    {"radet_conv2d_igemm_classes_s", t_radet_conv2d_igemm_classes_s, 20},
    {"radet_conv2d_igemm_pair", t_radet_conv2d_igemm_pair, 23},
    {"radet_conv2d_igemm_pair_s", t_radet_conv2d_igemm_pair_s, 24},
    {"radet_conv2d_igemm_s", t_radet_conv2d_igemm_s, 18},
    {"radet_conv2d_igemm_taps", t_radet_conv2d_igemm_taps, 17},
    {"radet_conv2d_igemm_taps_s", t_radet_conv2d_igemm_taps_s, 18},
    {"radet_conv2d_wgrad", t_radet_conv2d_wgrad, 14},
    {"radet_conv2d_wgrad_group", t_radet_conv2d_wgrad_group, 4},
    {"radet_conv2d_wgrad_s", t_radet_conv2d_wgrad_s, 15},
    {"radet_conv2d_wgrad_splits", t_radet_conv2d_wgrad_splits, 5},
    {"radet_convert_rows", t_radet_convert_rows, 10},
    {"radet_copy_d2d", t_radet_copy_d2d, 4},
    {"radet_copy_segments", t_radet_copy_segments, 4},
    {"radet_crop_canvases", t_radet_crop_canvases, 11},
    {"radet_decode_candidates", t_radet_decode_candidates, 19},
    {"radet_fill_zero", t_radet_fill_zero, 3},
    {"radet_fold_weights", t_radet_fold_weights, 3},
    {"radet_gather_table_rows", t_radet_gather_table_rows, 1},
    {"radet_gaussian_blur9_u8", t_radet_gaussian_blur9_u8, 8},
    {"radet_gdt", t_radet_gdt, 8},
    {"radet_giou_loss", t_radet_giou_loss, 9},
    {"radet_giou_loss_bwd", t_radet_giou_loss_bwd, 11},
    {"radet_gn_relu_bwd", t_radet_gn_relu_bwd, 16},
    {"radet_gn_relu_bwd_h", t_radet_gn_relu_bwd_h, 16},
    {"radet_gn_relu_bwd_p", t_radet_gn_relu_bwd_p, 17},
    {"radet_gn_relu_bwd_q", t_radet_gn_relu_bwd_q, 20},
    {"radet_gn_relu_fwd", t_radet_gn_relu_fwd, 14},
    {"radet_gn_relu_fwd_h", t_radet_gn_relu_fwd_h, 14},
    {"radet_gn_relu_fwd_p", t_radet_gn_relu_fwd_p, 15},
    {"radet_gn_relu_fwd_pair", t_radet_gn_relu_fwd_pair, 20},
    {"radet_gn_relu_fwd_pair_h", t_radet_gn_relu_fwd_pair_h, 20},
    {"radet_gn_relu_fwd_pair_p", t_radet_gn_relu_fwd_pair_p, 22},
    {"radet_gn_relu_fwd_pair_q", t_radet_gn_relu_fwd_pair_q, 28},
    {"radet_gn_relu_fwd_q", t_radet_gn_relu_fwd_q, 18},
    {"radet_gn_workspace_floats", t_radet_gn_workspace_floats, 3},
    {"radet_grid_anchors", t_radet_grid_anchors, 5},
    {"radet_head_loss", t_radet_head_loss, 31},
    {"radet_head_loss_ws_ints", t_radet_head_loss_ws_ints, 1},
    {"radet_jpeg_decode", t_radet_jpeg_decode, 17},
    {"radet_jpeg_index", t_radet_jpeg_index, 11},
    {"radet_loss_finalize", t_radet_loss_finalize, 6},
    {"radet_loss_partials", t_radet_loss_partials, 1},
    {"radet_mask_max", t_radet_mask_max, 5},
    {"radet_mask_transform", t_radet_mask_transform, 13},
    {"radet_mask_transform_src_window", t_radet_mask_transform_src_window, 11},
    {"radet_mask_transform_window", t_radet_mask_transform_window, 11},
    {"radet_maxpool3x3s2", t_radet_maxpool3x3s2, 7},
    {"radet_maxpool3x3s2_a", t_radet_maxpool3x3s2_a, 8},
    {"radet_maxpool3x3s2_bwd_relu", t_radet_maxpool3x3s2_bwd_relu, 8},
    {"radet_maxpool3x3s2_h", t_radet_maxpool3x3s2_h, 7},
    {"radet_maxpool3x3s2_q", t_radet_maxpool3x3s2_q, 11},
    {"radet_mbd", t_radet_mbd, 12},
    {"radet_merge_pairs", t_radet_merge_pairs, 7},
    {"radet_merge_planes", t_radet_merge_planes, 6},
    {"radet_nchw_to_nhwc", t_radet_nchw_to_nhwc, 7},
    {"radet_nhwc_to_nchw", t_radet_nhwc_to_nchw, 7},
    {"radet_nms", t_radet_nms, 20},
    {"radet_paste_maps", t_radet_paste_maps, 9},
    {"radet_pred3x3_patch", t_radet_pred3x3_patch, 13},
    {"radet_preprocess_frames", t_radet_preprocess_frames, 12},
    {"radet_relu_bwd", t_radet_relu_bwd, 6},
    {"radet_relu_bwd_a", t_radet_relu_bwd_a, 7},
    {"radet_relu_bwd_h", t_radet_relu_bwd_h, 6},
    {"radet_resize_linear_f", t_radet_resize_linear_f, 8},
    {"radet_resize_linear_u8", t_radet_resize_linear_u8, 8},
    {"radet_resize_linear_u8_src_window", t_radet_resize_linear_u8_src_window, 8},
    {"radet_resize_linear_u8_window", t_radet_resize_linear_u8_window, 8},
    {"radet_rle_masks", t_radet_rle_masks, 14},
    {"radet_rle_masks_src_window", t_radet_rle_masks_src_window, 13},
    {"radet_rle_masks_window", t_radet_rle_masks_window, 13},
    {"radet_scale_relu", t_radet_scale_relu, 7},
    {"radet_sigmoid_focal_loss", t_radet_sigmoid_focal_loss, 12},
    {"radet_sigmoid_focal_loss_bwd", t_radet_sigmoid_focal_loss_bwd, 14},
    {"radet_sobel_edge", t_radet_sobel_edge, 8},
    {"radet_split_pairs", t_radet_split_pairs, 8},
    {"radet_split_planes", t_radet_split_planes, 6},
    {"radet_sqnorm_partials", t_radet_sqnorm_partials, 5},
    {"radet_stem_conv_bn_relu", t_radet_stem_conv_bn_relu, 8},
    {"radet_stem_conv_bn_relu_a", t_radet_stem_conv_bn_relu_a, 9},
    {"radet_stem_conv_bn_relu_h", t_radet_stem_conv_bn_relu_h, 8},
    {"radet_stem_wgrad", t_radet_stem_wgrad, 9},
    {"radet_stem_wgrad_splits", t_radet_stem_wgrad_splits, 3},
    {"radet_stream_create_cumask", t_radet_stream_create_cumask, 3},
    {"radet_tblr_decode", t_radet_tblr_decode, 10},
    {"radet_tblr_encode", t_radet_tblr_encode, 7},
    {"radet_threshold_compact", t_radet_threshold_compact, 6},
    {"radet_unfold_grads", t_radet_unfold_grads, 4},
    {"radet_upsample_add", t_radet_upsample_add, 9},
    {"radet_upsample_add_a", t_radet_upsample_add_a, 10},
    {"radet_upsample_add_bwd", t_radet_upsample_add_bwd, 9},
    {"radet_upsample_add_bwd_a", t_radet_upsample_add_bwd_a, 10},
    {"radet_upsample_add_bwd_h", t_radet_upsample_add_bwd_h, 9},
    {"radet_upsample_add_h", t_radet_upsample_add_h, 9},
    {"radet_warp_affine_u8", t_radet_warp_affine_u8, 9},
};
const int radet_tape_nthunks = 113;
```

### radet_amd/engine.py

```python
import contextlib
import ctypes as C
import os

import torch

from . import _lib
from . import kernels as K
from .kernels import ConvGeom, Levels

ARCH = {50: (3, 4, 6, 3), 101: (3, 4, 23, 3)}


def conv_out_hw(h, w, k, s, p):
    return (h + 2 * p - k) // s + 1, (w + 2 * p - k) // s + 1


class _StemSplits:

    def __init__(self, nsplit):
        self.nsplit = nsplit


class Conv:

# ... 593 lines not shown
        if blk["po"]:
            K.conv_fwd(c1.geom, x, c1.wf, c1.bias_f, None, relu=True, yq=o1, wmeta=c1.wmeta)
            K.conv_fwd(c2.geom, o1, c2.wf, c2.bias_f, o2, relu=True, tile=c2.geom.fwd_tile_q)
        else:
            K.conv_fwd(blk["c1"].geom, x, blk["c1"].wf, blk["c1"].bias_f, o1, relu=True)
            K.conv_fwd(blk["c2"].geom, o1, blk["c2"].wf, blk["c2"].bias_f, o2, relu=True)
        if blk["ds"] is not None:
            idt = b[pfx + ".idt"]
            K.conv_fwd(blk["ds"].geom, x, blk["ds"].wf, blk["ds"].bias_f, idt)
        else:
            idt = x
        outq = b.get(pfx + ".out@q")
        K.conv_fwd(blk["c3"].geom, o2, blk["c3"].wf, blk["c3"].bias_f, out, addend=idt, relu=True, yq=outq,
                   wmeta=c3.wmeta if outq is not None else None)
        return out

    def _n_frozen_stages(self):
        n = 0
        while n < len(self.stages) and not self.stages[n][0]["train"]:
            n += 1
        return n

    def _prefix_forward(self, img, which):
        B, H, W = self.B, self.H, self.W
        b = self._pfx_sets[which]
        if self.h2:
            K.fill_zero(self.amax_pfx[which])
        K.STAGE = "stem"
        K.stem(img, self.stem.wf, self.stem.bias_f, b["stem"], B, H, W)
        K.maxpool(b["stem"], b["pool"], B, self.stem_hw[0], self.stem_hw[1], 64, yq=b.get("pool@q"))
        x, xq = b["pool"], b.get("pool@q")
        for li in range(self._n_frozen_stages()):
            K.STAGE = f"layer{li + 1}"
            for bi, blk in enumerate(self.stages[li]):
                x = self._block_forward(blk, f"l{li + 1}.{bi}", x, b, xq)
                xq = b.get(f"l{li + 1}.{bi}.out@q")
        return b

    @staticmethod
    def _img_key(img, geo):
        return (img.data_ptr(), img._version, tuple(img.shape), geo)

    def prefetch_prefix(self, next_img):
        if self.stem.trainable or not self.use_streams or next_img is None or self.geo_key is None:
            return False
        if tuple(next_img.shape) != (self.B, 3, self.H, self.W) or not next_img.is_contiguous():
            return False
        other = 1 - self._pfx_active
        if self._pfx_sets[other] is None:
            self._pfx_sets[other] = {}
            if self.h2:
                self.amax_pfx[other] = K.new_amax(self.dev, 128)
            for i, (name, (rows, ch, dt, twin)) in enumerate(self._pfx_shapes.items()):
                if dt == "pairs-only":
                    q = K.Planes(rows, ch, device=self.dev, kind="h2")
                    q.true_amax = self.amax_pfx[other][i]
                    self._pfx_sets[other][name] = q
                    continue
                t = torch.empty(rows, ch, device=self.dev, dtype=dt)
                self._pfx_sets[other][name] = t
                if self.h2 and dt == torch.float32:
                    self._amax_keys.append(K.register_amax(t, self.amax_pfx[other][i], by_storage=True))
                if twin:
                    q = K.Planes(rows, ch, device=self.dev, kind="h2")
                    q.true_amax = self.amax_pfx[other][i]
                    self._pfx_sets[other][name + "@q"] = q
        cs = self._chain_stream()
        self._fork(cs)
        stage = K.STAGE
        if self._pfx_event is None:
            self._pfx_event = torch.cuda.Event()
        ev = self._pfx_event
        with torch.cuda.stream(cs):
            self._prefix_forward(next_img, other)
            K.ev_record(ev)
        K.STAGE = stage
        self._pfx_ready = (self._img_key(next_img, self.geo_key), other, ev, next_img)
        return True

    _pfx_event = None

    def backbone_forward(self, img):
        b = self.buf
        self._img = img if self.stem.trainable else None
        if self.h2:
            K.fill_zero(self.amax_act)
        nf = self._n_frozen_stages() if not self.stem.trainable else 0
        rdy, self._pfx_ready = self._pfx_ready, None
        if not self.stem.trainable and rdy is not None and rdy[3] is img and rdy[0] == self._img_key(img, self.geo_key):
            K.ev_wait(rdy[2])
            self._pfx_active = rdy[1]
            pb = self._pfx_sets[self._pfx_active]
        elif not self.stem.trainable:
            pb = self._prefix_forward(img, self._pfx_active)
        else:
            K.STAGE = "stem"
            K.stem(img, self.stem.wf, self.stem.bias_f, b["stem"], self.B, self.H, self.W)
            K.maxpool(b["stem"], b["pool"], self.B, self.stem_hw[0], self.stem_hw[1], 64, yq=b.get("pool@q"))
            pb = b
        if not self.stem.trainable:
            b.update(pb)
        last = "pool" if nf == 0 else f"l{nf}.{len(self.stages[nf - 1]) - 1}.out"
        x, xq = pb[last], pb.get(last + "@q")
        outs = [pb[f"l{li + 1}.{len(self.stages[li]) - 1}.out"] for li in range(nf)]
        for li in range(nf, len(self.stages)):
            blocks = self.stages[li]
            K.STAGE = f"layer{li + 1}"
            if blocks[0]["train"]:
                self._await_fold()
            for bi, blk in enumerate(blocks):
                x = self._block_forward(blk, f"l{li + 1}.{bi}", x, b, xq)
                xq = b.get(f"l{li + 1}.{bi}.out@q")
            outs.append(x)
        return outs


    def neck_forward(self, feats):
        K.STAGE = "neck"
        self._await_fold()
        b, B = self.buf, self.B
        c = feats[1:]
        for i in range(3):
            cq = b.get(f"l{i + 2}.{len(self.stages[i + 1]) - 1}.out@q")
            if cq is not None and self.lat[i].wfq is not None:
                K.conv_fwd(self.lat[i].geom, cq, self.lat[i].wfq, self.lat[i].bias_f, b[f"lat{i}"], tile=self.lat[i].geom.fwd_tile_q)
            else:
                K.conv_fwd(self.lat[i].geom, c[i], self.lat[i].wf, self.lat[i].bias_f, b[f"lat{i}"])
        hw = self.plv.hw
        for i in (2, 1):
            K.upsample_add(b[f"lat{i - 1}"], b[f"lat{i}"], B, hw[i - 1][0], hw[i - 1][1], hw[i][0], hw[i][1], self.feat)
        P = b["P"]
        for i in range(3):
            r0, r1 = self.plv.level_rows(i)
            K.conv_fwd(self.fpn[i].geom, b[f"lat{i}"], self.fpn[i].wf, self.fpn[i].bias_f, P[r0:r1])
        for i in (3, 4):
            s0, s1 = self.plv.level_rows(i - 1)
            r0, r1 = self.plv.level_rows(i)
            K.conv_fwd(self.fpn[i].geom, P[s0:s1], self.fpn[i].wf, self.fpn[i].bias_f, P[r0:r1])
        return P

    use_streams = True

    _SHARED_STREAMS = {}

    def _shared_stream(self, role):
        key = (torch.device(self.dev).index if torch.device(self.dev).index is not None else torch.cuda.current_device(), role)
        st = Engine._SHARED_STREAMS.get(key)
        if st is None:
            mask = os.environ.get("RADET_WGRAD_CU_MASK")
            if mask and role in ("side", "side2"):
                words = (C.c_uint32 * 8)(*([int(mask, 0) & 0xFFFFFFFF] * 8))
                out = C.c_void_p()
                with torch.cuda.device(self.dev):
                    _lib.check(_lib.load().radet_stream_create_cumask(words, 8, C.byref(out)), "radet_stream_create_cumask")
                st = torch.cuda.ExternalStream(out.value, device=self.dev)
            else:
                st = torch.cuda.Stream(device=self.dev)
            Engine._SHARED_STREAMS[key] = st
        return st

    def caller_stream(self):
        key = (torch.device(self.dev).index if torch.device(self.dev).index is not None else torch.cuda.current_device(), "caller")
        st = Engine._SHARED_STREAMS.get(key)
        if st is None:
            touch = [self._side(), self._side2(), self._chain_stream()]
            touch += [torch.cuda.Stream(device=self.dev) for _ in range(2)]
# ... 157 lines not shown
                                                b[f"cls.stats{i}"], self.gn_ws, b[f"cls.zhat{i}"]),
                                     (zr, p[gr + ".weight"], p[gr + ".bias"], None if pl else yr, yr if pl else None,
                                      b[f"reg.stats{i}"], self.gn_ws2, b[f"reg.zhat{i}"]))
                return yc, yr
            K.gn_relu_fwd_pair_p(self.plv, (zc, p[gc + ".weight"], p[gc + ".bias"], None if pl else yc, yc if pl else None,
                                            b[f"cls.stats{i}"], self.gn_ws),
                                 (zr, p[gr + ".weight"], p[gr + ".bias"], None if pl else yr, yr if pl else None,
                                  b[f"reg.stats{i}"], self.gn_ws2))
            return yc, yr
        if self.h2:
            K.gn_relu_fwd_pair_q(self.plv, (zc, p[gc + ".weight"], p[gc + ".bias"], yc, None, b[f"cls.stats{i}"], self.gn_ws, None),
                                 (zr, p[gr + ".weight"], p[gr + ".bias"], yr, None, b[f"reg.stats{i}"], self.gn_ws2, None))
            return yc, yr
        K.gn_relu_fwd_pair(self.plv, (zc, p[gc + ".weight"], p[gc + ".bias"], yc, b[f"cls.stats{i}"], self.gn_ws),
                           (zr, p[gr + ".weight"], p[gr + ".bias"], yr, b[f"reg.stats{i}"], self.gn_ws2))
        return yc, yr

    def head_forward(self, P):
        K.STAGE = "head"
        b = self.buf
        n = self.stacked_convs
        if self.tower_mode in ("pair", "hybrid", "pairbwd"):
            xc = xr = P
            if self.p3:
                K.split_planes(P, b["Pp"])
                xc = xr = b["Pp"]
            if self.p3 and self.tower_fwd_streams and self.use_streams:
                side = self._side()
                self._fork(side)
                for i in range(n):
                    xc = self._tower_fwd_layer_p("cls", self.cls_tower, i, xc, self.gn_ws)
                    with torch.cuda.stream(side):
                        xr = self._tower_fwd_layer_p("reg", self.reg_tower, i, xr, self.gn_ws2)
            else:
                side = None
                for i in range(n):
                    xc, xr = self._tower_pair_fwd(i, xc, xr)
            reg_stream = torch.cuda.stream(side) if side is not None else contextlib.nullcontext()
            if self.x3 and self.feat % 16 == 0 and self.pred_cls.cout <= 32 and self.pred_reg.cout + self.pred_iou.cout <= 32 \
                    and os.environ.get("RADET_PRED_PATCH", "1") != "0":
                pc, pr, pi = self.pred_cls, self.pred_reg, self.pred_iou
                K.pred_conv_patch(self.plv, xc, (pc.wf, pc.bias_f, b["cls"], pc.cout))
                with reg_stream:
                    K.pred_conv_patch(self.plv, xr, (pr.wf, pr.bias_f, b["reg_u"], pr.cout), (pi.wf, pi.bias_f, b["iou"], pi.cout))
            else:
                K.conv_fwd(self.pred_cls.geom, xc, self.pred_cls.wf, self.pred_cls.bias_f, b["cls"])
                with reg_stream:
                    K.conv_fwd(self.pred_reg.geom, xr, self.pred_reg.wf, self.pred_reg.bias_f, b["reg_u"])
                    K.conv_fwd(self.pred_iou.geom, xr, self.pred_iou.wf, self.pred_iou.bias_f, b["iou"])
            if side is not None:
                self._join(side)
        elif self.use_streams:
            side = self._side()
            self._fork(side)
            xc = xr = P
            for i in range(n):
                xc = self._tower_fwd_layer("cls", self.cls_tower, i, xc, self.gn_ws)
                with torch.cuda.stream(side):
                    xr = self._tower_fwd_layer("reg", self.reg_tower, i, xr, self.gn_ws2)
            K.conv_fwd(self.pred_cls.geom, xc, self.pred_cls.wf, self.pred_cls.bias_f, b["cls"])
            with torch.cuda.stream(side):
                K.conv_fwd(self.pred_reg.geom, xr, self.pred_reg.wf, self.pred_reg.bias_f, b["reg_u"])
                K.conv_fwd(self.pred_iou.geom, xr, self.pred_iou.wf, self.pred_iou.bias_f, b["iou"])
            self._join(side)
        else:
            xc = xr = P
            for i in range(n):
                xc = self._tower_fwd_layer("cls", self.cls_tower, i, xc, self.gn_ws)
            for i in range(n):
                xr = self._tower_fwd_layer("reg", self.reg_tower, i, xr, self.gn_ws)
            K.conv_fwd(self.pred_cls.geom, xc, self.pred_cls.wf, self.pred_cls.bias_f, b["cls"])
            K.conv_fwd(self.pred_reg.geom, xr, self.pred_reg.wf, self.pred_reg.bias_f, b["reg_u"])
            K.conv_fwd(self.pred_iou.geom, xr, self.pred_iou.wf, self.pred_iou.bias_f, b["iou"])
        return b["cls"], b["reg_u"], b["iou"]

    def scales_tensor(self):
        names = [f"bbox_head.scales.{i}.scale" for i in range(len(self.strides))]
        ts = [self.p[n] for n in names]
        base = ts[0].data_ptr()
        if all(t.data_ptr() == base + 4 * i for i, t in enumerate(ts)):
            return torch.as_strided(ts[0], (len(ts),), (1,))
        return torch.stack([t.reshape(()) for t in ts]).contiguous()

    def loss(self, gt_boxes, gt_labels, gt_off, p2g, pw, grad_scale=None, alpha=0.25, gamma=2.0, lbw=2.0,
             labels_out=None, tgt_out=None):
        b = self.buf
        dri = b["dregiou"]
        K.head_loss(b["cls"], b["reg_u"], b["iou"], self.scales_tensor(), gt_boxes, gt_labels, gt_off, p2g, pw, self.ldesc,
                    self.nlvl, self.B, self.num_classes, alpha, gamma, lbw, 1e-6, grad_scale, self.losses, b["dcls"],
                    self.cls_pad, dri, 16, dri.view(-1)[4:], 16, self.dscales, self.loss_ws, labels_out, tgt_out)
        if self.h2:
            K.absmax(b["dcls"], K.amax_slot(b["dcls"]))
            K.absmax(dri, K.amax_slot(dri))
        if self.h16:
            K.convert_rows(b["dcls"], b["dcls16"])
            K.convert_rows(dri, b["dregiou16"], ncols=4)
            K.convert_rows(dri, b["dregiou16"], ncols=1, src_off=4, dst_off=self.iou_col)
        return self.losses

    def _head_grads(self):
        b = self.buf
        return (b["dcls16"], b["dregiou16"]) if self.h16 else (b["dcls"], b["dregiou"])

    def _tower_bwd_head(self, t):
        b = self.buf
        ylast = b[f"{t}.y{self.stacked_convs - 1}"]
        dy = b[f"{t}.dy"]
        dcls, dri = self._head_grads()
        if t == "cls":
            pc = self.pred_cls
            K.conv_wgrad(pc.geom, dcls, ylast, pc.slabs, pc.dbias_partials, cout=pc.cout, ld_dy=self.cls_pad)
            K.conv_dgrad(pc.geom, dcls, pc.wft, dy, k_channels=self.cls_pad)
        else:
            pr, pi = self.pred_reg, self.pred_iou
            K.conv_wgrad(pr.geom, dri, ylast, pr.slabs, pr.dbias_partials, cout=4, ld_dy=self.ri_pad)
            K.conv_wgrad(pi.geom, dri.view(-1)[self.iou_col:], ylast, pi.slabs, pi.dbias_partials, cout=1, ld_dy=self.ri_pad)
            K.conv_dgrad(pr.geom, dri, pr.wft, dy, k_channels=self.ri_pad)

    def _tower_bwd_head_async(self, t):
        b = self.buf
        ylast = b[f"{t}.y{self.stacked_convs - 1}"]
        dy = b[f"{t}.dy"]
        side = self._side() if self.use_streams else None

        def wg(*a, **k):
            if side is None:
                K.conv_wgrad(*a, **k)
            else:
                self._fork(side)
                with torch.cuda.stream(side):
                    K.conv_wgrad(*a, **k)

        dcls, dri = self._head_grads()
        if t == "cls":
            pc = self.pred_cls
            wg(pc.geom, dcls, ylast, pc.slabs, pc.dbias_partials, cout=pc.cout, ld_dy=self.cls_pad)
            K.conv_dgrad(pc.geom, dcls, pc.wft, dy, k_channels=self.cls_pad)
        else:
            pr, pi = self.pred_reg, self.pred_iou
            wg(pr.geom, dri, ylast, pr.slabs, pr.dbias_partials, cout=4, ld_dy=self.ri_pad)
            wg(pi.geom, dri.view(-1)[self.iou_col:], ylast, pi.slabs, pi.dbias_partials, cout=1, ld_dy=self.ri_pad)
            K.conv_dgrad(pr.geom, dri, pr.wft, dy, k_channels=self.ri_pad)

    def _tower_bwd_layer(self, t, tower, i, ws, dP, addend):
        b, p, g = self.buf, self.p, self.g
        c = tower[i]
        dy, dz = b[f"{t}.dy"], b[f"{t}.dz"]
        gn = f"bbox_head.{t}_convs.{i}.gn"
        self._gn_bwd(dy, b[f"{t}.z{i}"], b[f"{t}.stats{i}"], p[gn + ".weight"], p[gn + ".bias"], dz,
                     g[gn + ".weight"], g[gn + ".bias"], ws)
        x = b[f"{t}.y{i - 1}"] if i > 0 else b["P"]
        K.conv_wgrad(c.geom, dz, x, c.slabs, None)
        if self.tower_mode == "hybrid":
            K.conv_dgrad(c.geom, dz, c.wft, dy if i > 0 else dP, addend=None if i > 0 else addend,
                         tile=self._ttile(c, bwd=True, tag=False))
        elif i > 0:
            self._tower_launch(K.conv_dgrad, c.geom, dz, c.wft, dy, tile=self._ttile(c, bwd=True))
        else:
            self._tower_launch(K.conv_dgrad, c.geom, dz, c.wft, dP, addend=addend, tile=self._ttile(c, bwd=True))

    def head_backward(self):
        K.STAGE = "head"
        b = self.buf
        n = self.stacked_convs
        dP = b["dP"]
        if self.p3 and self.tower_mode == "pairbwd" and self.use_streams and os.environ.get("RADET_TOWER_BWD_CHAINS", "1") != "0":
            p, g = self.p, self.g
            cs = self._chain_stream()
            wg_done = {}

            def layer(t, tower, ws, i):
                gn = f"bbox_head.{t}_convs.{i}.gn"
                ev = wg_done.get((t, i + 2))
                if ev is not None:
                    K.ev_wait(ev)
                if self.h2:
                    K.gn_relu_bwd_q(self.plv, b[f"{t}.dy"], b[f"{t}.z{i}"], b[f"{t}.stats{i}"], p[gn + ".weight"],
                                    p[gn + ".bias"], None, b[f"{t}.dz{i & 1}"], g[gn + ".weight"], g[gn + ".bias"], ws,
                                    zhat_amax=b[f"{t}.zhat{i}"])
                else:
                    K.gn_relu_bwd_p(self.plv, b[f"{t}.dy"], b[f"{t}.z{i}"], b[f"{t}.stats{i}"], p[gn + ".weight"],
# ... 3 lines not shown
                if i > 0:
                    K.conv_dgrad(tower[i].geom, b[f"{t}.dz{i & 1}"], tower[i].wft, b[f"{t}.dy"], tile=self.tower_tile | K.splitk(1))
            self._tower_bwd_head_async("cls")
            self._fork(cs)
            with torch.cuda.stream(cs):
                self._tower_bwd_head_async("reg")
            for i in range(n - 1, -1, -1):
                layer("cls", self.cls_tower, self.gn_ws, i)
                with torch.cuda.stream(cs):
                    layer("reg", self.reg_tower, self.gn_ws2, i)
            K.conv_dgrad(self.cls_tower[0].geom, b["cls.dz0"], self.cls_tower[0].wft, dP, tile=self.tower_tile | K.splitk(1))
            self._fork(cs)
            with torch.cuda.stream(cs):
                K.conv_dgrad(self.reg_tower[0].geom, b["reg.dz0"], self.reg_tower[0].wft, dP, addend=dP, tile=self.tower_tile | K.splitk(1))
            self._join(cs)
        elif self.tower_mode in ("pair", "pairbwd"):
            p, g = self.p, self.g
            tagged = self.tower_mode == "pair"
            launch = self._tower_launch if tagged else (lambda fn, *a, **k: fn(*a, **k))
            self._tower_bwd_head_async("cls")
            self._tower_bwd_head_async("reg")
            wg_done = {}
            gn_first = self.p3 and os.environ.get("RADET_GN_FIRST", "1") != "0"
            for i in range(n - 1, -1, -1):
                pending = []
                for t, tower in (("cls", self.cls_tower), ("reg", self.reg_tower)):
                    gn = f"bbox_head.{t}_convs.{i}.gn"
                    ev = wg_done.get((t, i + 2))
                    if ev is not None:
                        K.ev_wait(ev)
                    if self.p3 and self.h2:
                        K.gn_relu_bwd_q(self.plv, b[f"{t}.dy"], b[f"{t}.z{i}"], b[f"{t}.stats{i}"], p[gn + ".weight"],
                                        p[gn + ".bias"], None, b[f"{t}.dz{i & 1}"], g[gn + ".weight"], g[gn + ".bias"], self.gn_ws,
                                        zhat_amax=b[f"{t}.zhat{i}"])
                    elif self.p3:
                        K.gn_relu_bwd_p(self.plv, b[f"{t}.dy"], b[f"{t}.z{i}"], b[f"{t}.stats{i}"], p[gn + ".weight"],
                                        p[gn + ".bias"], None, b[f"{t}.dz{i & 1}"], g[gn + ".weight"], g[gn + ".bias"], self.gn_ws)
                    else:
                        self._gn_bwd(b[f"{t}.dy"], b[f"{t}.z{i}"], b[f"{t}.stats{i}"], p[gn + ".weight"],
                                     p[gn + ".bias"], b[f"{t}.dz{i & 1}"], g[gn + ".weight"], g[gn + ".bias"], self.gn_ws)
                    x = b[f"{t}.y{i - 1}"] if i > 0 else (b["Pp"] if self.p3 else b["P"])
                    if gn_first:
                        pending.append((t, tower, x))
                    else:
                        wg_done[(t, i)] = self._wgrad_async(tower[i].geom, b[f"{t}.dz{i & 1}"], x, tower[i].slabs, None)
                if pending and os.environ.get("RADET_TOWER_WGRAD_MAIN") == "1":
                    for t, tower, x in pending:
                        K.conv_wgrad(tower[i].geom, b[f"{t}.dz{i & 1}"], x, tower[i].slabs, None)
                    pending = []
                for t, tower, x in pending:
                    wg_done[(t, i)] = self._wgrad_async(tower[i].geom, b[f"{t}.dz{i & 1}"], x, tower[i].slabs, None)
                cc, cr = self.cls_tower[i], self.reg_tower[i]
                dzc, dzr = b[f"cls.dz{i & 1}"], b[f"reg.dz{i & 1}"]
                if i > 0:
                    launch(K.conv_dgrad_pair, cc.geom, dict(x=dzc, w=cc.wft, y=b["cls.dy"]),
                                       dict(x=dzr, w=cr.wft, y=b["reg.dy"]), tile=self._ttile(cc, bwd=True, tag=tagged))
                else:
                    launch(K.conv_dgrad, cc.geom, dzc, cc.wft, dP, tile=self._ttile(cc, bwd=True, tag=tagged, pair=False))
                    launch(K.conv_dgrad, cr.geom, dzr, cr.wft, dP, addend=dP, tile=self._ttile(cr, bwd=True, tag=tagged, pair=False))
        elif self.use_streams:
            side = self._side()
            self._fork(side)
            self._tower_bwd_head("cls")
            with torch.cuda.stream(side):
                self._tower_bwd_head("reg")
            for i in range(n - 1, 0, -1):
                self._tower_bwd_layer("cls", self.cls_tower, i, self.gn_ws, dP, None)
                with torch.cuda.stream(side):
                    self._tower_bwd_layer("reg", self.reg_tower, i, self.gn_ws2, dP, None)
            self._tower_bwd_layer("cls", self.cls_tower, 0, self.gn_ws, dP, None)
            self._fork(side)
            with torch.cuda.stream(side):
                self._tower_bwd_layer("reg", self.reg_tower, 0, self.gn_ws2, dP, dP)
            self._join(side)
        else:
            for t, tower, first in (("cls", self.cls_tower, True), ("reg", self.reg_tower, False)):
                self._tower_bwd_head(t)
                for i in range(n - 1, -1, -1):
                    self._tower_bwd_layer(t, tower, i, self.gn_ws, dP, None if first else dP)
        self._write_scale_grads()
        return dP

    def _write_scale_grads(self):
        g = self.g
        ts = [g[f"bbox_head.scales.{i}.scale"] for i in range(len(self.strides))]
        base = ts[0].data_ptr()
        if all(t.data_ptr() == base + 4 * i for i, t in enumerate(ts)):
            K.copy_d2d(torch.as_strided(ts[0], (len(ts),), (1,)), self.dscales)
            return
        for i, t in enumerate(ts):
            K.copy_d2d(t, self.dscales[i])

    def neck_backward(self, dP):
        K.STAGE = "neck"
        b, B, f = self.buf, self.B, self.feat
        P = b["P"]
        lr = [self.plv.level_rows(i) for i in range(5)]
        sl = lambda t, i: t[lr[i][0]:lr[i][1]]
        tmp2, tmp3 = b["dP_tmp2"], b["dP_tmp3"]
        c4, c3 = self.fpn[4], self.fpn[3]
        self._wgrad_async(c4.geom, sl(dP, 4), sl(P, 3), c4.slabs, c4.dbias_partials, conv=c4)
        K.conv_dgrad(c4.geom, sl(dP, 4), c4.wft, tmp3, addend=sl(dP, 3))
        self._wgrad_async(c3.geom, tmp3, sl(P, 2), c3.slabs, c3.dbias_partials, conv=c3)
        K.conv_dgrad(c3.geom, tmp3, c3.wft, tmp2, addend=sl(dP, 2))
        srcs = [sl(dP, 0), sl(dP, 1), tmp2]
        for i in range(3):
            c = self.fpn[i]
            self._wgrad_async(c.geom, srcs[i], b[f"lat{i}"], c.slabs, c.dbias_partials, conv=c)
            K.conv_dgrad(c.geom, srcs[i], c.wft, b[f"d_lat{i}"])
        hw = self.plv.hw
        for i in (1, 2):
            K.upsample_add_bwd(b[f"d_lat{i}"], b[f"d_lat{i - 1}"], B, hw[i - 1][0], hw[i - 1][1], hw[i][0], hw[i][1], f)
        feats = [self.stages[i][-1] for i in (1, 2, 3)]
        for i in range(3):
            c = self.lat[i]
            x = b[f"l{i + 2}.{len(self.stages[i + 1]) - 1}.out"]
            self._wgrad_async(c.geom, b[f"d_lat{i}"], x, c.slabs, c.dbias_partials, conv=c)
            K.conv_dgrad(c.geom, b[f"d_lat{i}"], c.wft, b[f"d_c{i}"])
        del feats
        self.flush_wgrads()
        return [b["d_c0"], b["d_c1"], b["d_c2"]]

    def backbone_backward(self, d_feats, after_stage=None, block_ends=()):
        b = self.buf
        d_next_pre = None
        nxt = None
        for li in range(len(self.stages) - 1, -1, -1):
            blocks = self.stages[li]
            if not blocks[0]["train"]:
                break
            K.STAGE = f"layer{li + 1}"
            for bi in range(len(blocks) - 1, -1, -1):
                blk = blocks[bi]
                pfx = f"l{li + 1}.{bi}"
                out, o1, o2 = b[pfx + ".out"], b[pfx + ".o1"], b[pfx + ".o2"]
                d_pre, d_o1, d_o2 = b[pfx + ".d_pre"], b[pfx + ".d_o1"], b[pfx + ".d_o2"]
                last_of_stage = bi == len(blocks) - 1
                ext = d_feats[li - 1] if (last_of_stage and li >= 1) else None
                if nxt is None:
                    K.relu_bwd(ext, None, out, d_pre)
                elif nxt["ds"] is not None:
                    K.conv_dgrad(nxt["c1"].geom, nxt["d_o1"], nxt["c1"].wft, d_pre, addend=ext, mask=out)
                    K.conv_dgrad(nxt["ds"].geom, nxt["d_pre"], nxt["ds"].wft, d_pre, addend=d_pre, mask=out,
                                 skip_zero_rows=True)
                else:
                    K.conv_dgrad(nxt["c1"].geom, nxt["d_o1"], nxt["c1"].wft, d_pre, addend=nxt["d_pre"], mask=out)
                blk["d_pre"], blk["d_o1"] = d_pre, d_o1
                c1, c2, c3, ds = blk["c1"], blk["c2"], blk["c3"], blk["ds"]
                self._wgrad_async(c3.geom, d_pre, o2, c3.slabs, c3.dbias_partials, conv=c3)
                if blk["po"]:
                    K.conv_dgrad(c3.geom, d_pre, c3.wft, None, mask=o2, yq=d_o2, wmeta=c3.wmeta_t)
                else:
                    K.conv_dgrad(c3.geom, d_pre, c3.wft, d_o2, mask=o2)
                self._wgrad_async(c2.geom, d_o2, o1, c2.slabs, c2.dbias_partials, conv=c2)
                K.conv_dgrad(c2.geom, d_o2, c2.wft, d_o1, mask=o1)
                self._wgrad_async(c1.geom, d_o1, blk["x"], c1.slabs, c1.dbias_partials, conv=c1)
                if ds is not None:
                    self._wgrad_async(ds.geom, d_pre, blk["x"], ds.slabs, ds.dbias_partials, conv=ds)
                nxt = blk
                if (li, bi) in block_ends and after_stage is not None:
                    self.flush_wgrads()
                    after_stage(li, bi)
                elif self.wgrad_flush_blocks and (len(blocks) - bi) % self.wgrad_flush_blocks == 0:
                    self.flush_wgrads()
            self.flush_wgrads()
            if after_stage is not None:
# ... 13 lines not shown
```

### radet_amd/kernels.py

```python
import ctypes as C
import os

import torch

from . import _lib

ID_MASK = 0xFF
SYMBOL = 0x100
BK32 = 0x200
MATH_BF16 = 0x400
STORE_BF16, OUT_F32 = 0x800, 0x10000
SPLITK, SPLITK_MASK = 0x1000, 0xF000
STAGES3 = 0x20000
STAGES4 = 0x40000
ROWPAIRS = 0x80000
STREAMK, STREAMK_MASK = 0x100000, 0x700000
X3 = 0x1000000
P3 = 0x2000000
H2 = 0x8000000
MASKQ = 0x10000000
WG_MATH_BF16, WG_STORE_BF16 = 0x1, 0x2
WG_TILE, WG_TILE_MASK = 0x10, 0x30
WG_ONE_TAP = 0x40
WG_PX32 = 0x80
# ... 920 lines not shown
            if g.stride == 1 and g.pad == 1 and WGRAD9_DEEP and -(-g.lout.rows // (16 * (g.nsplit_pairs or g.nsplit))) * 16 <= 1664:
                return "conv_wgrad9d_kernel"
            return "conv_wgrad9r_kernel" if (g.stride == 1 and g.pad == 1 and WGRAD9_WINDOWS) else "conv_wgrad9q_kernel"
        return "conv_wgrad9p_kernel"
    tile, px = onetap(g.wgrad_flags)
    if getattr(g, "h2", False) and getattr(g, "x3", False) and not g.math and not _is16(dy):
        return f"conv_wgradg_kernel<{tile}> (fp16 hi/lo in registers{px})"
    nine = g.k == 3 and g.cin % 32 == 0 and co >= 256 and g.lout.rows >= 16384 and not (g.wgrad_flags & WG_ONE_TAP)
    mode = "bf16 storage" if _is16(dy) else ("bf16 math" if g.math else ("planes in registers" if getattr(g, "x3", False) else "fp32 MFMA"))
    if nine:
        return f"conv_wgrad9{'h' if _is16(dy) else 'g'}_kernel ({mode})"
    return f"conv_wgrad{'h' if _is16(dy) else 'g'}_kernel<{tile}> ({mode}{px})"


def conv_wgrad(g, dy, x, slabs, dbias_partials=None, cout=None, ld_dy=None):
    if EVENTS is not None:
        co_ = g.cout if cout is None else cout
        _timed(_wgrad_key(g, dy, co_), 2.0 * g.lout.rows * co_ * g.cin * g.k * g.k,
               lambda: _conv_wgrad(g, dy, x, slabs, dbias_partials, cout, ld_dy),
               4.0 * (g.lout.rows * co_ + g.lin.rows * g.cin + g.nsplit * co_ * g.k * g.k * g.cin), kind="wgrad", geom=g)
        return
    _conv_wgrad(g, dy, x, slabs, dbias_partials, cout, ld_dy)


def _conv_wgrad(g, dy, x, slabs, dbias_partials=None, cout=None, ld_dy=None):
    co = g.cout if cout is None else cout
    if _isp(dy):
        assert _isp(x) and x.kind == dy.kind
        if dy.kind == "h2":
            nine = g.k == 3 and not (g.wgrad_pair_flags & WG_ONE_TAP)
            fl = WG_H2 | WG_P3 | (g.wgrad_pair_flags if nine else (WG_ONE_TAP | (g.wgrad_pair_flags & WG_TILE_MASK)))
            if nine and g.stride == 1 and g.pad == 1:
                fl |= (WG_DEEP if WGRAD9_DEEP else 0) | (WG_WINDOWS if WGRAD9_WINDOWS else 0)
            _lib.call("radet_conv2d_wgrad_s", _ptr(dy.t), _ptr(x.t), _ptr(slabs), _ptr(dbias_partials), _ptr(g.fwd_table),
                      g.lout.rows, g.cin, co, co if ld_dy is None else ld_dy, g.k, g.k,
                      g.nsplit_pairs or g.nsplit, fl, _stream(), _scales(dy, x, None))
            return
        _lib.call("radet_conv2d_wgrad", _ptr(dy.t), _ptr(x.t), _ptr(slabs), _ptr(dbias_partials), _ptr(g.fwd_table), g.lout.rows,
                  g.cin, co, co if ld_dy is None else ld_dy, g.k, g.k, g.nsplit, WG_P3 | (g.wgrad_flags & WG_ONE_TAP), _stream())
        return
    if getattr(g, "h2", False) and getattr(g, "x3", False) and not g.math and not _is16(dy):
        _lib.call("radet_conv2d_wgrad_s", _ptr(dy), _ptr(x), _ptr(slabs), _ptr(dbias_partials), _ptr(g.fwd_table), g.lout.rows,
                  g.cin, co, co if ld_dy is None else ld_dy, g.k, g.k, g.nsplit, WG_H2 | WG_ONE_TAP | g.wgrad_flags, _stream(),
                  _scales(dy, x, None))
        return
    _lib.call("radet_conv2d_wgrad", _ptr(dy), _ptr(x), _ptr(slabs), _ptr(dbias_partials), _ptr(g.fwd_table), g.lout.rows,
              g.cin, co, co if ld_dy is None else ld_dy, g.k, g.k, g.nsplit,
              (WG_STORE_BF16 if _is16(dy) else (WG_MATH_BF16 if g.math else (WG_X3 if getattr(g, "x3", False) else 0))) | g.wgrad_flags, _stream())


def conv_wgrad_group(jobs, tile=128, math=0):
    jobs = sorted(jobs, key=lambda j: -(j["g"].lout.rows // j["g"].nsplit))
    for i in range(0, len(jobs), 32):
        part = jobs[i:i + 32]
        arr = (_lib.RadetWgradJob * len(part))()
        for a, j in zip(arr, part):
            g = j["g"]
            a.dy, a.x, a.slabs = _ptr(j["dy"]), _ptr(j["x"]), _ptr(j["slabs"])
            a.dbias_partials, a.gather_table = _ptr(j.get("dbias")), _ptr(g.fwd_table)
            a.M, a.Cin, a.Cout, a.ld_dy, a.KH, a.KW, a.S = g.lout.rows, g.cin, g.cout, g.cout, g.k, g.k, g.nsplit
        _lib.call("radet_conv2d_wgrad_group", arr, len(part), (WG_MATH_BF16 if math else 0) | (1 if tile == 128 else 2) * WG_TILE, _stream())


def group_splits(geoms, tile=128, slots=512):
    best = None
    for px in (6400, 4800, 3200, 2400, 1600, 1200, 800, 600, 400):
        S = [max(1, min(64, round(g.lout.rows / px), (g.lout.rows + 127) // 128)) for g in geoms]
        blocks = sum((g.cout // tile) * (g.cin // tile) * g.k * g.k * s for g, s in zip(geoms, S))
        eff = blocks / (slots * -(-blocks // slots))
        cost = -eff + 0.02 * sum(S) / len(S)
        if best is None or cost < best[0] - 1e-9:
            best = (cost, S)
    return best[1]


def fold_weights(table_dev, n):
    _lib.call("radet_fold_weights", _ptr(table_dev), n, _stream())


def unfold_grads(table_dev, n, max_cout):
    _lib.call("radet_unfold_grads", _ptr(table_dev), n, max_cout, _stream())


def _h(name, t):
    return name + "_h" if _is16(t) else name


def stem(img, wf, bias, y, B, H, W):
    ho, wo = (H + 1) // 2, (W + 1) // 2
    if _is16(y):
        fn = lambda: _lib.call("radet_stem_conv_bn_relu_h", _ptr(img), _ptr(wf), _ptr(bias), _ptr(y), B, H, W, _stream())
    else:
        sl = amax_slot(y)
        fn = lambda: _lib.call("radet_stem_conv_bn_relu_a", _ptr(img), _ptr(wf), _ptr(bias), _ptr(y), B, H, W, _ptr(sl), _stream())
    _timed("stem_kernel", 2.0 * B * ho * wo * 64 * 147, fn, 4.0 * (B * 3 * H * W + 64 * 147 + B * ho * wo * 64))


def convert_rows(src, dst, ncols=None, src_off=0, dst_off=0):
    assert src.dim() == 2 and dst.dim() == 2 and src.shape[0] == dst.shape[0] and src.dtype != dst.dtype
    n = src.shape[1] if ncols is None else ncols
    _lib.call("radet_convert_rows", _ptr(src), _ptr(dst), C.c_size_t(src.shape[0]), n, src.stride(0), src_off,
              dst.stride(0), dst_off, 1 if dst.dtype == torch.bfloat16 else 0, _stream())


def maxpool(x, y, B, H, W, Cch, yq=None):
    if _is16(x):
        _lib.call("radet_maxpool3x3s2_h", _ptr(x), _ptr(y), B, H, W, Cch, _stream())
        return
    if yq is not None:
        _lib.call("radet_maxpool3x3s2_q", _ptr(x), _ptr(y), B, H, W, Cch, _ptr(amax_slot(y)), _ptr(yq.t), _ptr(yq.amax),
                  _ptr(amax_slot(x, True)), _stream())
        return
    _lib.call("radet_maxpool3x3s2_a", _ptr(x), _ptr(y), B, H, W, Cch, _ptr(amax_slot(y)), _stream())


def maxpool_bwd_relu(s, dpool, ds, B, H, W, Cch):
    _lib.call("radet_maxpool3x3s2_bwd_relu", _ptr(s), _ptr(dpool), _ptr(ds), B, H, W, Cch, _stream())


def stem_wgrad_splits(B, H, W):
    return _lib.load().radet_stem_wgrad_splits(B, H, W)


def stem_wgrad(img, ds, slabs, dbias_partials, B, H, W, S):
    _lib.call("radet_stem_wgrad", _ptr(img), _ptr(ds), _ptr(slabs), _ptr(dbias_partials), B, H, W, S, _stream())


def gn_ws_floats(levels):
    d, n = _desc([(h, w, h, w, o, o) for (h, w), o in zip(levels.hw, levels.offsets)])
    return _lib.load().radet_gn_workspace_floats(levels.B, d, n)


def _gn_desc(levels):
    return _desc([(h, w, h, w, o, o) for (h, w), o in zip(levels.hw, levels.offsets)])


def gn_relu_fwd(levels, z, gamma, beta, y, stats, ws, eps=1e-5, relu=True):
    d, n = _gn_desc(levels)
    _lib.call(_h("radet_gn_relu_fwd", z), _ptr(z), _ptr(gamma), _ptr(beta), _ptr(y), _ptr(stats), _ptr(ws), levels.B, 256, 32,
              eps, int(relu), d, n, _stream())


def gn_relu_fwd_pair(levels, a, b, eps=1e-5, relu=True):
    d, n = _gn_desc(levels)
    _lib.call(_h("radet_gn_relu_fwd_pair", a[0]), *[_ptr(t) for t in a], *[_ptr(t) for t in b], levels.B, 256, 32, eps,
              int(relu), d, n, _stream())


def gn_relu_fwd_p(levels, z, gamma, beta, y, yp, stats, ws, eps=1e-5, relu=True):
    d, n = _gn_desc(levels)
    _lib.call("radet_gn_relu_fwd_p", _ptr(z), _ptr(gamma), _ptr(beta), _ptr(y), _ptr_any(yp), _ptr(stats), _ptr(ws), levels.B,
              256, 32, eps, int(relu), d, n, _stream())


def gn_relu_fwd_pair_p(levels, a, b, eps=1e-5, relu=True):
    d, n = _gn_desc(levels)
    _lib.call("radet_gn_relu_fwd_pair_p", *[_ptr_any(t) for t in a], *[_ptr_any(t) for t in b], levels.B, 256, 32, eps,
              int(relu), d, n, _stream())


def gn_relu_fwd_q(levels, z, gamma, beta, y, yq, stats, ws, zhat_amax=None, eps=1e-5, relu=True):
    d, n = _gn_desc(levels)
    _lib.call("radet_gn_relu_fwd_q", _ptr(z), _ptr(gamma), _ptr(beta), _ptr(y), _ptr_any(yq), _ptr(stats), _ptr(ws), levels.B,
              256, 32, eps, int(relu), d, n, _stream(), _ptr(amax_slot(y)), _ptr(yq.amax) if yq is not None else None,
              _ptr(zhat_amax))

# ... 8 lines not shown
    _lib.call("radet_gn_relu_fwd_pair_q", *q(a), *q(b), levels.B, 256, 32, eps, int(relu), d, n, _stream())


def gn_relu_bwd_q(levels, dy, z, stats, gamma, beta, dz, dzq, dgamma, dbeta, ws, zhat_amax=None, dy_amax=None, relu=True):
    d, n = _gn_desc(levels)
    da = dy_amax if dy_amax is not None else (amax_slot(dy, compute=True) if dzq is not None else None)
    _lib.call("radet_gn_relu_bwd_q", _ptr(dy), _ptr(z), _ptr(stats), _ptr(gamma), _ptr(beta), _ptr(dz), _ptr_any(dzq),
              _ptr(dgamma), _ptr(dbeta), _ptr(ws), levels.B, 256, 32, int(relu), d, n, _stream(), _ptr(da), _ptr(zhat_amax),
              _ptr(dzq.amax) if dzq is not None else None)


def gn_relu_bwd_p(levels, dy, z, stats, gamma, beta, dz, dzp, dgamma, dbeta, ws, relu=True):
    d, n = _gn_desc(levels)
    _lib.call("radet_gn_relu_bwd_p", _ptr(dy), _ptr(z), _ptr(stats), _ptr(gamma), _ptr(beta), _ptr(dz), _ptr_any(dzp),
              _ptr(dgamma), _ptr(dbeta), _ptr(ws), levels.B, 256, 32, int(relu), d, n, _stream())


def gn_relu_bwd(levels, dy, z, stats, gamma, beta, dz, dgamma, dbeta, ws, relu=True):
    d, n = _gn_desc(levels)
    _lib.call(_h("radet_gn_relu_bwd", dy), _ptr(dy), _ptr(z), _ptr(stats), _ptr(gamma), _ptr(beta), _ptr(dz), _ptr(dgamma),
              _ptr(dbeta), _ptr(ws), levels.B, 256, 32, int(relu), d, n, _stream())


def upsample_add(dst, src, B, ho, wo, hi, wi, ch):
    if _is16(dst):
        _lib.call("radet_upsample_add_h", _ptr(dst), _ptr(src), B, ho, wo, hi, wi, ch, _stream())
        return
    _lib.call("radet_upsample_add_a", _ptr(dst), _ptr(src), B, ho, wo, hi, wi, ch, _ptr(amax_slot(dst)), _stream())


def upsample_add_bwd(dsrc, ddst, B, ho, wo, hi, wi, ch):
    if _is16(dsrc):
        _lib.call("radet_upsample_add_bwd_h", _ptr(dsrc), _ptr(ddst), B, ho, wo, hi, wi, ch, _stream())
        return
    _lib.call("radet_upsample_add_bwd_a", _ptr(dsrc), _ptr(ddst), B, ho, wo, hi, wi, ch, _ptr(amax_slot(dsrc)), _stream())


def relu_bwd(dy, addend, act, dx):
    if _is16(dy):
        _lib.call("radet_relu_bwd_h", _ptr(dy), _ptr(addend), _ptr(act), _ptr(dx), C.c_size_t(dx.numel()), _stream())
        return
    _lib.call("radet_relu_bwd_a", _ptr(dy), _ptr(addend), _ptr(act), _ptr(dx), C.c_size_t(dx.numel()), _ptr(amax_slot(dx)),
              _stream())


def nchw_to_nhwc(x, y, B, ch, H, W):
    if _is16(y):
        tmp = torch.empty(y.shape, device=y.device, dtype=torch.float32)
        _lib.call("radet_nchw_to_nhwc", _ptr(x), _ptr(tmp), B, ch, H, W, _stream())
        convert_rows(tmp.view(-1, ch), y.view(-1, ch))
        return
    _lib.call("radet_nchw_to_nhwc", _ptr(x), _ptr(y), B, ch, H, W, _stream())
    sl = amax_slot(y)
    if sl is not None and y.numel() % 4 == 0:
        absmax(y, sl)


def nhwc_to_nchw(x, y, B, ch, H, W):
    if _is16(x):
        tmp = torch.empty(x.shape, device=x.device, dtype=torch.float32)
        convert_rows(x.reshape(-1, ch), tmp.view(-1, ch))
        x = tmp
    _lib.call("radet_nhwc_to_nchw", _ptr(x), _ptr(y), B, ch, H, W, _stream())


def level_desc(levels, strides):
    flat = []
    for (h, w), s in zip(levels.hw, strides):
        flat += [h, w, int(s)]
    return (C.c_int * len(flat))(*flat), len(levels.hw)


def head_loss_ws_ints(R):
    return _lib.load().radet_head_loss_ws_ints(R)


def head_loss(cls, reg_u, iou, scales, gt_boxes, gt_labels, gt_off, p2g, pw, ldesc, nlvl, B, num_classes, alpha, gamma,
              lbw, giou_eps, grad_scale, losses, dcls, dcls_ld, dreg, dreg_ld, diou, diou_ld, dscales, ws,
              labels_out=None, tgt_out=None, flags=0):
    _lib.call("radet_head_loss", _ptr(cls), _ptr(reg_u), _ptr(iou), _ptr(scales), _ptr(gt_boxes), _ptr(gt_labels),
              _ptr(gt_off), _ptr(p2g), _ptr(pw), ldesc, nlvl, B, num_classes, alpha, gamma, lbw, giou_eps,
              _ptr(grad_scale), _ptr(losses), _ptr(dcls), dcls_ld, _ptr(dreg), dreg_ld, _ptr(diou), diou_ld,
              _ptr(dscales), _ptr(labels_out), _ptr(tgt_out), flags, _ptr(ws), _stream())


def scale_relu(reg_u, scales, out, ldesc, nlvl, B):
    _lib.call("radet_scale_relu", _ptr(reg_u), _ptr(scales), _ptr(out), ldesc, nlvl, B, _stream())


def grid_anchors(out, ldesc, nlvl, base_scale=8):
    _lib.call("radet_grid_anchors", _ptr(out), ldesc, nlvl, base_scale, _stream())


OVERLAP_MODES = dict(iou=0, iof=1, giou=2)


def bbox_overlaps(b1, b2, out, batch, M, N, mode, aligned, eps):
    _lib.call("radet_bbox_overlaps", _ptr(b1), _ptr(b2), _ptr(out), batch, M, N, OVERLAP_MODES[mode], int(aligned), eps,
              _stream())


def _norm4(normalizer):
    v = [float(normalizer)] * 4 if isinstance(normalizer, (int, float)) else [float(x) for x in normalizer]
    assert len(v) == 4, "Normalizer must have length = 4"
    return (C.c_float * 4)(*v)


def tblr_encode(priors, gts, out, normalizer, normalize_by_wh=True):
    _lib.call("radet_tblr_encode", _ptr(priors), _ptr(gts), _ptr(out), priors.shape[0], _norm4(normalizer),
              int(normalize_by_wh), _stream())


def tblr_decode(priors, tblr, out, normalizer, normalize_by_wh=True, max_shape=None, clip_border=True):
    clip = bool(clip_border and max_shape is not None)
    mh, mw = (float(max_shape[0]), float(max_shape[1])) if clip else (0.0, 0.0)
    _lib.call("radet_tblr_decode", _ptr(priors), _ptr(tblr), _ptr(out), priors.shape[0], _norm4(normalizer),
              int(normalize_by_wh), mh, mw, int(clip), _stream())


def loss_partials(n_elem):
    return _lib.load().radet_loss_partials(n_elem)


def loss_finalize(partials, avg_factor, scale, out):
    _lib.call("radet_loss_finalize", _ptr(partials), partials.numel(), _ptr(avg_factor), scale, _ptr(out), _stream())


def sigmoid_focal_loss(x, target, weight, wcols, N, Cc, gamma, alpha, elem, partials, elem_scale=1.0):
    _lib.call("radet_sigmoid_focal_loss", _ptr(x), _ptr(target), _ptr(weight), wcols, C.c_size_t(N), Cc, gamma, alpha,
              _ptr(elem), elem_scale, _ptr(partials), _stream())


def sigmoid_focal_loss_bwd(x, target, weight, wcols, N, Cc, gamma, alpha, grad_elem, grad_scalar, avg_factor, scale, dx):
    _lib.call("radet_sigmoid_focal_loss_bwd", _ptr(x), _ptr(target), _ptr(weight), wcols, C.c_size_t(N), Cc, gamma, alpha,
              _ptr(grad_elem), _ptr(grad_scalar), _ptr(avg_factor), scale, _ptr(dx), _stream())


def bce_logits_loss(x, target, weight, wcols, N, Cc, elem, partials, elem_scale=1.0):
    _lib.call("radet_bce_logits_loss", _ptr(x), _ptr(target), _ptr(weight), wcols, C.c_size_t(N), Cc, _ptr(elem),
              elem_scale, _ptr(partials), _stream())


def bce_logits_loss_bwd(x, target, weight, wcols, N, Cc, grad_elem, grad_scalar, avg_factor, scale, dx):
    _lib.call("radet_bce_logits_loss_bwd", _ptr(x), _ptr(target), _ptr(weight), wcols, C.c_size_t(N), Cc, _ptr(grad_elem),
              _ptr(grad_scalar), _ptr(avg_factor), scale, _ptr(dx), _stream())


def giou_loss(pred, target, weight, N, eps, elem, partials, elem_scale=1.0):
    _lib.call("radet_giou_loss", _ptr(pred), _ptr(target), _ptr(weight), C.c_size_t(N), eps, _ptr(elem), elem_scale, _ptr(partials),
              _stream())


def giou_loss_bwd(pred, target, weight, N, eps, grad_elem, grad_scalar, avg_factor, scale, dpred):
    _lib.call("radet_giou_loss_bwd", _ptr(pred), _ptr(target), _ptr(weight), C.c_size_t(N), eps, _ptr(grad_elem),
              _ptr(grad_scalar), _ptr(avg_factor), scale, _ptr(dpred), _stream())


def threshold_compact(scores, thr, idx, count):
    _lib.call("radet_threshold_compact", _ptr(scores), C.c_size_t(scores.numel()), thr, _ptr(idx), _ptr(count), _stream())


def sqnorm_partials(g, n, partials):
    _lib.call("radet_sqnorm_partials", _ptr(g), C.c_size_t(n), _ptr(partials), partials.numel(), _stream())


def adamw_step(p, g, m, v, n, lr, betas, eps, wd, step, max_norm, grad_div, partials, grad_norm_out):
# ... 373 lines not shown
```

### radet_amd/runtime.py

```python
import os

import numpy as np
import torch
import torch.distributed as dist

from . import _lib
from . import kernels as K
from .engine import Engine


def _align(n, a=4):
    return (n + a - 1) // a * a


class FlatParams:

    def __init__(self, module, device):
        named = [(n, p) for n, p in module.named_parameters()]
        train = [(n, p) for n, p in named if p.requires_grad]
        frozen = [(n, p) for n, p in named if not p.requires_grad]
        bufs = [(n, b) for n, b in module.named_buffers() if b.is_floating_point()]
        self.train_names = [n for n, _ in train]
        self.offsets = {}
        off = 0
# ... 182 lines not shown
                        t["done"].record()
            if self.bf16:
                self._convert(self.staging[b:e], self.grads[b:e])
        self.works = []


class DetectorRuntime:
    def __init__(self, det, depth, num_classes, frozen_stages, strides, stacked_convs=4, math=None):
        dev = next(det.parameters()).device
        if dev.type != "cuda":
            raise _lib.RadetHipError(
                "radet_amd runs on MI355X only: move the detector to a HIP device (model.cuda()) first; "
                "there is no CPU / PyTorch fallback path.")
        _lib.load()
        self.dev = dev
        self.flat = FlatParams(det, dev)
        self.engine = Engine(self.flat.p, self.flat.g, depth=depth, num_classes=num_classes,
                             frozen_stages=frozen_stages, strides=strides, stacked_convs=stacked_convs, math=math,
                             watch=self.flat.watch)
        self.num_classes, self.strides = num_classes, tuple(strides)
        self.opt_state = None
        self.step_count = 0
        self.comm_stream = None
        self.buckets = compute_buckets(self.flat, [c.name for c in self.engine.convs],
                                       [c.trainable for c in self.engine.convs])
        self.reducer = None
        self._replicas_synced = False

    def caller_stream(self):
        return self.engine.caller_stream()

    def sync_replicas(self, src=0):
        self._replicas_synced = True
        if not (dist.is_available() and dist.is_initialized()) or dist.get_world_size() == 1:
            return False
        arenas = [self.flat.params, self.flat.frozen]
        if self.opt_state is not None:
            arenas += [self.opt_state["m"], self.opt_state["v"]]
        for t in arenas:
            dist.broadcast(t, src)
        step = torch.tensor([self.step_count], dtype=torch.int64, device=self.dev)
        dist.broadcast(step, src)
        self.step_count = int(step.item())
        return True

    def pack_targets(self, gt_bboxes, gt_labels, points_to_gt_index, points_weight):
        dev = self.dev
        B = len(gt_bboxes)
        counts = [int(b.shape[0]) for b in gt_bboxes]
        off = np.zeros(B + 1, np.int32)
        off[1:] = np.cumsum(counts)
        boxes = torch.cat([b.reshape(-1, 4).float() for b in gt_bboxes]) if sum(counts) else torch.zeros(0, 4)
        labels = torch.cat([l.reshape(-1).long() for l in gt_labels]) if sum(counts) else torch.zeros(0, dtype=torch.long)
        boxes = boxes.to(dev).contiguous()
        labels = labels.to(dev).contiguous()
        if boxes.shape[0] == 0:
            boxes = torch.zeros(1, 4, device=dev)
            labels = torch.zeros(1, dtype=torch.long, device=dev)
        p2g = torch.stack([t.reshape(-1).long() for t in points_to_gt_index]).to(dev).contiguous()
        pw = torch.stack([t.reshape(-1).float() for t in points_weight]).to(dev).contiguous()
        return dict(boxes=boxes, labels=labels, off=torch.from_numpy(off).to(dev), p2g=p2g, pw=pw, B=B)

    def forward(self, img, fold=True):
        assert img.is_cuda and img.dtype == torch.float32 and img.dim() == 4 and img.shape[1] == 3
        img = img.contiguous()
        e = self.engine
        e.prepare(img.shape[0], img.shape[2], img.shape[3])
        if fold:
            e.fold()
        feats = e.backbone_forward(img)
        P = e.neck_forward(feats)
        return e.head_forward(P)

    loss_hparams = None
    loss_weights = None

    def set_loss_from_head(self, head):
        self.loss_hparams = dict(alpha=float(head.loss_cls.alpha), gamma=float(head.loss_cls.gamma),
                                 lbw=float(head.loss_bbox.loss_weight))
        wc, wi = float(head.loss_cls.loss_weight), float(head.loss_iou.loss_weight)
        self.loss_weights = None if (wc == 1.0 and wi == 1.0) else torch.tensor([wc, 1.0, wi], device=self.dev)
        return self

    def loss(self, tg, grad_scale=None, labels_out=None, tgt_out=None):
        hp = self.loss_hparams or dict(alpha=0.25, gamma=2.0, lbw=2.0)
        return self.engine.loss(tg["boxes"], tg["labels"], tg["off"], tg["p2g"], tg["pw"], grad_scale=grad_scale,
                                labels_out=labels_out, tgt_out=tgt_out, **hp)

    def backward(self, bucket_hook=None, next_img=None):
        e = self.engine
        if not self._replicas_synced:
            self._replicas_synced = True
            if dist.is_available() and dist.is_initialized() and dist.get_world_size() > 1:
                import warnings
                warnings.warn("radet_amd: backward pass under a process group of "
                              f"{dist.get_world_size()} ranks before DetectorRuntime.sync_replicas() / init_optimizer() was "
                              "called: the replicas still hold their own initial parameters (call "
                              "det.runtime().sync_replicas() on every rank once, see INTEGRATION.md)")

        def unfold(bucket):
            self._unfold_bucket(bucket, bucket_hook)

        bk = {b["prefix"]: b for b in self.buckets}
        per_block = {(b["blocks"][0], b["blocks"][1]): b for b in self.buckets if "blocks" in b}
        dP = e.head_backward()
        if next_img is not None and bucket_hook is None:
            e.prefetch_prefix(next_img)
        unfold(bk["bbox_head."])
        d_feats = e.neck_backward(dP)
        unfold(bk["neck."])

        def after(li, bi=None):
            if bi is not None:
                if (li, bi) in per_block:
                    unfold(per_block[(li, bi)])
                return
            pf = "backbone.conv1" if li == "stem" else f"backbone.layer{li + 1}."
            if pf in bk:
                unfold(bk[pf])
        e.backbone_backward(d_feats, after_stage=after, block_ends=set(per_block))
        e.join_side()
        if next_img is not None and bucket_hook is not None:
            e.prefetch_prefix(next_img)

    def _unfold_bucket(self, bucket, bucket_hook=None):
        import ctypes as C
        e = self.engine
        desc_bytes = C.sizeof(_lib.RadetConvDesc)
        a, b = bucket["convs"]
        if e.use_streams:
            side = e._side()
            e.side_collect()
            e._fork(side)
            with torch.cuda.stream(side):
                K.unfold_grads(e.table[a * desc_bytes:], b - a, e.max_cout)
                if bucket_hook is not None:
                    if _lib.TAPE is not None:
                        _lib.TAPE.cut(lambda: bucket_hook(bucket), side)
                    bucket_hook(bucket)
        else:
            K.unfold_grads(e.table[a * desc_bytes:], b - a, e.max_cout)
            if bucket_hook is not None:
                if _lib.TAPE is not None:
                    _lib.TAPE.cut(lambda: bucket_hook(bucket), None)
                bucket_hook(bucket)

    def init_optimizer(self, lr=4e-4, betas=(0.9, 0.999), eps=1e-8, weight_decay=0.05, max_norm=35.0, sync=True):
        n = self.flat.n_train
        self.opt_state = dict(m=torch.zeros(n, device=self.dev), v=torch.zeros(n, device=self.dev), lr=lr, betas=betas,
                              eps=eps, wd=weight_decay, max_norm=max_norm,
                              partials=torch.zeros(1024, device=self.dev), grad_norm=torch.zeros(1, device=self.dev))
        self.step_count = 0
        if sync:
            self.sync_replicas()

    def optimizer_step(self, lr=None, grad_div=1.0):
        st = self.opt_state
        self.step_count += 1
        K.sqnorm_partials(self.flat.grads, self.flat.n_train, st["partials"])
        K.adamw_step(self.flat.params, self.flat.grads, st["m"], st["v"], self.flat.n_train, st["lr"] if lr is None else lr,
                     st["betas"], st["eps"], st["wd"], self.step_count, st["max_norm"], grad_div, st["partials"],
                     st["grad_norm"])
        if _lib.TAPE is not None:
            _lib.TAPE.mark("lr", 5)
            _lib.TAPE.mark("step", 10)
        self.engine.params_changed()

    def bf16_buckets(self):
        env = os.environ.get("RADET_BF16_BUCKETS")
        if env is not None:
            return env == "1" and self.engine.math_name != "fp32"
        return self.engine.math_name == "bf16-storage"

    def comm_report(self):
        tr = self.reducer.trace if self.reducer is not None else None
        marks = self.__dict__.get("comm_marks")
        if not tr or not marks:
            return None
        torch.cuda.synchronize()
        n, lo = len(marks), 0
        acc = None
        fwd = bwd = exposed = 0.0
        for ev_b, ev0, ev1, hi in marks:
            step = tr[lo:hi]
            lo = hi
            def dur(w):
                try:
                    return float(w._get_duration())
                except Exception:
                    return -1.0
            rows = [(t["prefix"], t["bytes"], ev0.elapsed_time(t["ready"]), ev0.elapsed_time(t["done"]), dur(t["work"])) for t in step]
            b = ev0.elapsed_time(ev1)
            fwd += ev_b.elapsed_time(ev0); bwd += b
            exposed += max(0.0, max((r[3] for r in rows), default=0.0) - b)
            acc = rows if acc is None else [(a[0], a[1], a[2] + r[2], a[3] + r[3], a[4] + r[4]) for a, r in zip(acc, rows)]
        rep = dict(steps=n, forward_loss_ms=round(fwd / n, 3), backward_ms=round(bwd / n, 3),
                   exposed_comm_ms=round(exposed / n, 3), bf16_buckets=bool(self.reducer.bf16),
                   buckets=[dict(bucket=a[0], mbytes=round(a[1] / 1e6, 2), ready_ms=round(a[2] / n, 3), done_by_ms=round(a[3] / n, 3),
                                 allreduce_ms=(round(a[4] / n, 3) if a[4] >= 0 else None)) for a in acc])
        self.reducer.trace.clear()
        self.comm_marks.clear()
        return rep

    tape_mode = os.environ.get("RADET_TAPE", "1")
    tape_after = int(os.environ.get("RADET_TAPE_AFTER", "2"))

    def _tape_key(self, img, tg, world, use_reducer):
        e, st = self.engine, self.opt_state
        return (e.geo_key, getattr(e, "plan_id", None), tuple(img.shape), img.dtype, tuple(tg["p2g"].shape), int(tg["off"].numel()),
                world, use_reducer, self.loss_weights is None or self.loss_weights.data_ptr(),
                st["betas"], st["eps"], st["wd"], st["max_norm"], st["m"].data_ptr(), e.wgrad_streams, e.use_streams,
                tuple(sorted(self.loss_hparams.items())) if self.loss_hparams else None)

    def drop_tape(self):
        self._tape = None

    _tape = None

    def tape_stats(self):
        t = (self._tape or {}).get("tape")
        return None if t is None else dict(t.stats(), replays=t.replays)

    def train_step(self, img, tg, lr=None, next_img=None):
        world = dist.get_world_size() if dist.is_available() and dist.is_initialized() else 1
        use_reducer = world > 1 or (world == 1 and dist.is_available() and dist.is_initialized()
                                    and os.environ.get("RADET_FORCE_REDUCER") == "1")
        e = self.engine
        record = None
        tapeable = (self.tape_mode != "0" and next_img is None and K.EVENTS is None and e.tower_events is None
                    and not (self.reducer is not None and self.reducer.trace is not None) and e._pfx_ready is None
                    and img is not None and img.is_cuda and img.dtype == torch.float32 and img.is_contiguous()
                    and self.opt_state is not None and "partials" in self.opt_state
                    and all(tg[k].is_contiguous() for k in ("boxes", "labels", "off", "p2g", "pw")))
        if tapeable:
            key = self._tape_key(img, tg, world, use_reducer)
            st = self._tape
            if st is None or st["key"] != key:
                st = self._tape = dict(key=key, count=0, tape=None, failed=None)
            if st["tape"] is not None:
                if self._tape_still_valid():
                    return self._replay_step(st["tape"], img, tg, lr, world)
                st = self._tape = dict(key=key, count=0, tape=None, failed=None)
            st["count"] += 1
            if st["count"] > self.tape_after and st["failed"] is None and (not use_reducer or self.reducer is not None):
                from .tape import Tape
                record = Tape()
        if self.reducer is not None and self.reducer.trace is not None:
            self._ev_begin = torch.cuda.Event(enable_timing=True)
            self._ev_begin.record()
        if record is not None:
            torch.cuda.current_stream().synchronize()
            record.begin(self.dev)
        try:
            self.forward(img)
            self.loss(tg, grad_scale=self.loss_weights)
            if use_reducer:
                if self.reducer is None:
                    on_chain = self.engine.use_streams and self.flat.grads.is_cuda
                    if on_chain and not sync_collectives_run_on_current_stream():
                        import warnings
                        warnings.warn(f"torch {torch.__version__} runs synchronous collectives on the process group's own stream: "
                                      "the gradient exchange uses that stream and the engine drops its second weight-gradient "
                                      "stream to stay inside the four-stream budget of this device")
                        on_chain = False
                        self.engine.wgrad_streams = 1
                    self.reducer = GradReducer(self.flat.grads, self.dev, bf16=self.bf16_buckets(),
                                               comm_stream=self.engine._chain_stream() if on_chain else None)
                tr = self.reducer.trace is not None
                if tr:
                    ev0 = torch.cuda.Event(enable_timing=True)
                    ev0.record()
                self.backward(self.reducer.bucket_ready, next_img=next_img)
                if tr:
                    ev1 = torch.cuda.Event(enable_timing=True)
                    ev1.record()
                    self.__dict__.setdefault("comm_marks", []).append((self._ev_begin, ev0, ev1, len(self.reducer.trace)))
                if record is not None:
                    record.cut(self.reducer.finish, None)
                self.reducer.finish()
            else:
                self.backward(next_img=next_img)
            self.optimizer_step(lr=lr, grad_div=float(world))
        except BaseException:
            if record is not None:
                record.abort()
            raise
        if record is not None:
            record.end()
            st = self._tape
            if record.poisoned is None and (e._last_fold != (False, True) or e._pfx_ready is not None):
                record.poisoned = "the recorded step was not a steady-state step (frozen weights were folded in it)"
            if record.poisoned is None:
                record.bind("img", img)
                for k in ("boxes", "labels", "off", "p2g", "pw"):
                    record.bind(k, tg[k])
                st["tape"] = record
                st["nf"] = e._frozen_conv_count()
            else:
                st["failed"] = record.poisoned
                if os.environ.get("RADET_TAPE_STRICT") == "1":
                    raise _lib.RadetHipError(f"launch tape could not be recorded: {record.poisoned}")
        if self.loss_weights is not None:
            return self.engine.losses * self.loss_weights
        return self.engine.losses

    def _tape_still_valid(self):
        e, st = self.engine, self._tape
        nf = st["nf"]
        if nf > 0 and e._part_version(0, nf) != e._folded[0]:
            return False
        return self.flat.still_bound() and _lib.TAPE is None

    def _replay_step(self, tape, img, tg, lr, world):
        e, st = self.engine, self.opt_state
        self.step_count += 1
        tape.replay(tensors=dict(img=img, boxes=tg["boxes"], labels=tg["labels"], off=tg["off"], p2g=tg["p2g"], pw=tg["pw"]),
                    values=dict(lr=st["lr"] if lr is None else lr, step=self.step_count))
        e.params_changed()
        if self.loss_weights is not None:
            return e.losses * self.loss_weights
        return e.losses


class _DetectorLossFn(torch.autograd.Function):

    @staticmethod
    def forward(ctx, rt, img, tg, weights, *params):
        rt.forward(img)
        losses = rt.loss(tg)
        ctx.rt, ctx.tg, ctx.weights = rt, tg, weights
        out = losses * weights
        return out[0], out[1], out[2]

    @staticmethod
    def backward(ctx, g0, g1, g2):
        rt = ctx.rt
        gs = (torch.stack([g0.reshape(()), g1.reshape(()), g2.reshape(())]).float() * ctx.weights).contiguous()
        rt.loss(ctx.tg, grad_scale=gs)
# ... 473 lines not shown
```

Before: 504.0.

## Overlap loss target prep with forward on side stream and fuse loss epilogues

Splits head loss into a prepare phase (row labels, targets, scan) that is issued on a side stream at the start of the backbone forward, plus a main phase that waits on an event. The focal kernel now also zeroes the sparse reg/iou gradients and computes the dcls absmax, and the positive-loss kernel publishes the reg/iou absmax. This removes the zero_sparse and two absmax launches, and scale gradients can be written straight into the gradient buffer. The cost is extra cross-stream synchronisation, plus a risk of races if the side-stream prepare uses stale target pointers.

```diff
diff --git a/include/radet_hip.h b/include/radet_hip.h
--- a/include/radet_hip.h
+++ b/include/radet_hip.h
@@ -230,6 +230,15 @@
                     float gamma, float loss_bbox_weight, float giou_eps, const float* grad_scale, float* losses,
                     float* dcls, int dcls_ld, float* dreg_u, int dreg_ld, float* diou, int diou_ld, float* dscales,
                     int64_t* labels_out, float* bbox_targets_out, int flags, int* ws, void* stream);
+int radet_head_loss_prepare(const float* gt_boxes, const int64_t* gt_labels, const int* gt_off, const int64_t* p2g,
+                            const float* pw, const int* level_desc, int nlvl, int B, int num_classes,
+                            int64_t* labels_out, float* bbox_targets_out, int* ws, void* stream);
+int radet_head_loss_a(const float* cls, const float* reg_u, const float* iou, const float* scales,
+                      const float* gt_boxes, const int64_t* gt_labels, const int* gt_off, const int64_t* p2g,
+                      const float* pw, const int* level_desc, int nlvl, int B, int num_classes, float alpha,
+                      float gamma, float loss_bbox_weight, float giou_eps, const float* grad_scale, float* losses,
+                      float* dcls, int dcls_ld, float* dreg_u, int dreg_ld, float* diou, int diou_ld, float* dscales,
+                      void* dcls_amax, void* dri_amax, int flags, int* ws, void* stream);
 int radet_scale_relu(const float* reg_u, const float* scales, float* out, const int* level_desc, int nlvl, int B,
                      void* stream);
 
diff --git a/radet_amd/_lib.py b/radet_amd/_lib.py
--- a/radet_amd/_lib.py
+++ b/radet_amd/_lib.py
@@ -82,6 +82,9 @@
     "radet_head_loss_ws_ints": (_i, [_i]),
     "radet_head_loss": (_i, [_p, _p, _p, _p, _p, _p, _p, _p, _p, _p, _i, _i, _i, _f, _f, _f, _f, _p, _p, _p, _i, _p,
                              _i, _p, _i, _p, _p, _p, _i, _p, _p]),
+    "radet_head_loss_prepare": (_i, [_p, _p, _p, _p, _p, _p, _i, _i, _i, _p, _p, _p, _p]),
+    "radet_head_loss_a": (_i, [_p, _p, _p, _p, _p, _p, _p, _p, _p, _p, _i, _i, _i, _f, _f, _f, _f, _p, _p, _p, _i, _p,
+                               _i, _p, _i, _p, _p, _p, _i, _p, _p]),
     "radet_scale_relu": (_i, [_p, _p, _p, _p, _i, _i, _p]),
     "radet_decode_ws_bytes": (_sz, [_i, _i, _i]),
     "radet_decode_candidates": (_i, [_p, _p, _p, _p, _p, _i, _i, _i, _f, _i, _p, _p, _p, _p, _p, _p, _p, _p, _p]),
diff --git a/radet_amd/csrc/loss.hip b/radet_amd/csrc/loss.hip
--- a/radet_amd/csrc/loss.hip
+++ b/radet_amd/csrc/loss.hip
@@ -132,17 +132,20 @@
 
 __device__ __forceinline__ float softplus_f(float x) { return fmaxf(x, 0.f) + log1pf(expf(-fabsf(x))); }
 
+template <bool FUSED>
 __global__ __launch_bounds__(256) void focal_kernel(const float* __restrict__ cls, const int64_t* __restrict__ gt_labels,
                                                     const int* __restrict__ gt_off, const int64_t* __restrict__ p2g,
                                                     const float* __restrict__ pw, const LossLevels L, int B, int N,
                                                     int R, int C, float alpha, float gamma,
                                                     const float* __restrict__ grad_scale, float* __restrict__ dcls,
-                                                    int dcls_ld, int* __restrict__ ws) {
+                                                    int dcls_ld, int* __restrict__ ws, float* __restrict__ dreg,
+                                                    int dreg_ld, float* __restrict__ diou, int diou_ld,
+                                                    unsigned* __restrict__ dcls_amax) {
     const float num_pos = __int_as_float(ws[1]);
     const float avg = num_pos + (float)B;
     const float gs = (grad_scale ? grad_scale[0] : 1.f) / avg;
     const size_t total = (size_t)R * C;
-    float acc = 0.f;
+    float acc = 0.f, am = 0.f;
     for (size_t i = (size_t)blockIdx.x * 256 + threadIdx.x; i < total; i += (size_t)gridDim.x * 256) {
         const int r = (int)(i / C);
         const int c = (int)(i - (size_t)r * C);
@@ -168,8 +171,17 @@
             dx = (1.f - alpha) * mod * (p - gamma * (1.f - p) * log1mp);
         }
         acc += loss * wt;
-        dcls[(size_t)r * dcls_ld + c] = dx * wt * gs;
-    }
+        const float dv = dx * wt * gs;
+        dcls[(size_t)r * dcls_ld + c] = dv;
+        if (FUSED) {
+            am = fmaxf(am, fabsf(dv));
+            if (c == 0) {
+                *reinterpret_cast<float4*>(dreg + (size_t)r * dreg_ld) = make_float4(0.f, 0.f, 0.f, 0.f);
+                diou[(size_t)r * diou_ld] = 0.f;
+            }
+        }
+    }
+    if (FUSED && dcls_amax) radet_amax_publish(am, dcls_amax);
     __shared__ float red[4];
     acc = wave_sum(acc);
     if ((threadIdx.x & 63) == 0) red[threadIdx.x >> 6] = acc;
@@ -206,7 +218,8 @@
                                                        float* __restrict__ losses, float* __restrict__ dreg_u,
                                                        int dreg_ld, float* __restrict__ diou, int diou_ld,
                                                        float* __restrict__ dscales, const int* __restrict__ ws,
-                                                       int n_focal_partials, int postact) {
+                                                       int n_focal_partials, int postact,
+                                                       unsigned* __restrict__ dri_amax) {
     __shared__ float red[256];
     const int tid = threadIdx.x;
     const int P = ws[0];
@@ -222,7 +235,7 @@
         if (tid < L.n) dscales[tid] = 0.f;
         return;
     }
-    float sw = 0.f, swl = 0.f, sb = 0.f, sp = 0.f;
+    float sw = 0.f, swl = 0.f, sb = 0.f, sp = 0.f, am = 0.f;
     for (int pass = 0; pass < 2; ++pass) {
         float inv_sw = 0.f, inv_sp = 0.f, g1 = 1.f, g2 = 1.f;
         float ds[RADET_MAX_SEG];
@@ -307,7 +320,9 @@
                 for (int l = 0; l < RADET_MAX_SEG; ++l)
                     if (l == ri.lvl) ds[l] += dsv;
                 const float sig = 1.f / (1.f + expf(-x));
-                diou[(size_t)r * diou_ld] = pwt * (sig - iou) * inv_sp * g2;
+                const float di = pwt * (sig - iou) * inv_sp * g2;
+                diou[(size_t)r * diou_ld] = di;
+                am = fmaxf(fmaxf(fmaxf(am, fmaxf(fabsf(du.x), fabsf(du.y))), fmaxf(fabsf(du.z), fabsf(du.w))), fabsf(di));
             }
         }
         if (pass == 0) {
@@ -329,6 +344,7 @@
             }
         }
     }
+    if (dri_amax) radet_amax_publish(am, dri_amax);
 }
 
 __global__ void zero_sparse_kernel(float* __restrict__ dreg, int dreg_ld, float* __restrict__ diou, int diou_ld, int R) {
@@ -364,6 +380,57 @@
 extern "C" int radet_head_loss_ws_ints(int R) {
     const int nb = (R + LP_BLK - 1) / LP_BLK;
     return WS_HDR + R + FOCAL_BLOCKS + 16 + nb * LP_BLK + 2 * nb;
+}
+
+static int head_loss_prepare(const LossLevels& L, const float* gt_boxes, const int64_t* gt_labels, const int* gt_off,
+                             const int64_t* p2g, const float* pw, int B, int num_classes, int64_t* labels_out,
+                             float* bbox_targets_out, int* ws, hipStream_t st) {
+    const int R = L.row_off[L.n], N = L.pt_off[L.n];
+    hipLaunchKernelGGL(loss_prep_rows_kernel, dim3((R + LP_BLK - 1) / LP_BLK), dim3(LP_BLK), 0, st, gt_labels, gt_boxes,
+                       gt_off, p2g, pw, L, B, N, R, num_classes, labels_out, bbox_targets_out, ws);
+    hipLaunchKernelGGL(loss_prep_scan_kernel, dim3(1), dim3(1024), 0, st, R, ws);
+    return RADET_OK;
+}
+
+static int focal_blocks(int R, int num_classes) {
+    const size_t total = (size_t)R * num_classes;
+    const size_t fb = (total + 255) / 256;
+    return fb > FOCAL_BLOCKS ? FOCAL_BLOCKS : (int)fb;
+}
+
+extern "C" int radet_head_loss_prepare(const float* gt_boxes, const int64_t* gt_labels, const int* gt_off,
+                                       const int64_t* p2g, const float* pw, const int* level_desc, int nlvl, int B,
+                                       int num_classes, int64_t* labels_out, float* bbox_targets_out, int* ws,
+                                       void* stream) {
+    LossLevels L;
+    int rc = fill_levels(&L, level_desc, nlvl, B);
+    if (rc) return rc;
+    rc = head_loss_prepare(L, gt_boxes, gt_labels, gt_off, p2g, pw, B, num_classes, labels_out, bbox_targets_out, ws,
+                           (hipStream_t)stream);
+    return rc ? rc : radet_check_launch();
+}
+
+extern "C" int radet_head_loss_a(const float* cls, const float* reg_u, const float* iou, const float* scales,
+                                 const float* gt_boxes, const int64_t* gt_labels, const int* gt_off, const int64_t* p2g,
+                                 const float* pw, const int* level_desc, int nlvl, int B, int num_classes, float alpha,
+                                 float gamma, float loss_bbox_weight, float giou_eps, const float* grad_scale,
+                                 float* losses, float* dcls, int dcls_ld, float* dreg_u, int dreg_ld, float* diou,
+                                 int diou_ld, float* dscales, void* dcls_amax, void* dri_amax, int flags, int* ws,
+                                 void* stream) {
+    LossLevels L;
+    int rc = fill_levels(&L, level_desc, nlvl, B);
+    if (rc) return rc;
+    const int R = L.row_off[nlvl], N = L.pt_off[nlvl];
+    if (dcls_ld < num_classes || dreg_ld < 4 || (dreg_ld & 3) || diou_ld < 1) return RADET_ERR_ARG;
+    hipStream_t st = (hipStream_t)stream;
+    const int fb = focal_blocks(R, num_classes);
+    hipLaunchKernelGGL(focal_kernel<true>, dim3(fb), dim3(256), 0, st, cls, gt_labels, gt_off, p2g, pw, L, B, N, R,
+                       num_classes, alpha, gamma, grad_scale, dcls, dcls_ld, ws, dreg_u, dreg_ld, diou, diou_ld,
+                       (unsigned*)dcls_amax);
+    hipLaunchKernelGGL(pos_loss_kernel, dim3(1), dim3(256), 0, st, reg_u, iou, scales, gt_boxes, gt_off, p2g, pw, L, B, N,
+                       R, loss_bbox_weight, giou_eps, grad_scale, losses, dreg_u, dreg_ld, diou, diou_ld, dscales, ws,
+                       fb, flags & 1, (unsigned*)dri_amax);
+    return radet_check_launch();
 }
 
 extern "C" int radet_head_loss(const float* cls, const float* reg_u, const float* iou, const float* scales,
@@ -379,18 +446,15 @@
     const int R = L.row_off[nlvl], N = L.pt_off[nlvl];
     if (dcls_ld < num_classes || dreg_ld < 4 || (dreg_ld & 3) || diou_ld < 1) return RADET_ERR_ARG;
     hipStream_t st = (hipStream_t)stream;
-    hipLaunchKernelGGL(loss_prep_rows_kernel, dim3((R + LP_BLK - 1) / LP_BLK), dim3(LP_BLK), 0, st, gt_labels, gt_boxes,
-                       gt_off, p2g, pw, L, B, N, R, num_classes, labels_out, bbox_targets_out, ws);
-    hipLaunchKernelGGL(loss_prep_scan_kernel, dim3(1), dim3(1024), 0, st, R, ws);
-    const size_t total = (size_t)R * num_classes;
-    int fb = (int)((total + 255) / 256);
-    if (fb > FOCAL_BLOCKS) fb = FOCAL_BLOCKS;
-    hipLaunchKernelGGL(focal_kernel, dim3(fb), dim3(256), 0, st, cls, gt_labels, gt_off, p2g, pw, L, B, N, R, num_classes,
-                       alpha, gamma, grad_scale, dcls, dcls_ld, ws);
+    head_loss_prepare(L, gt_boxes, gt_labels, gt_off, p2g, pw, B, num_classes, labels_out, bbox_targets_out, ws, st);
+    const int fb = focal_blocks(R, num_classes);
+    hipLaunchKernelGGL(focal_kernel<false>, dim3(fb), dim3(256), 0, st, cls, gt_labels, gt_off, p2g, pw, L, B, N, R,
+                       num_classes, alpha, gamma, grad_scale, dcls, dcls_ld, ws, (float*)nullptr, 0, (float*)nullptr, 0,
+                       (unsigned*)nullptr);
     hipLaunchKernelGGL(zero_sparse_kernel, dim3((R + 255) / 256), dim3(256), 0, st, dreg_u, dreg_ld, diou, diou_ld, R);
     hipLaunchKernelGGL(pos_loss_kernel, dim3(1), dim3(256), 0, st, reg_u, iou, scales, gt_boxes, gt_off, p2g, pw, L, B, N,
                        R, loss_bbox_weight, giou_eps, grad_scale, losses, dreg_u, dreg_ld, diou, diou_ld, dscales, ws,
-                       fb, flags & 1);
+                       fb, flags & 1, (unsigned*)nullptr);
     return radet_check_launch();
 }
 
diff --git a/radet_amd/csrc/tape_thunks.c b/radet_amd/csrc/tape_thunks.c
--- a/radet_amd/csrc/tape_thunks.c
+++ b/radet_amd/csrc/tape_thunks.c
@@ -61,6 +61,8 @@
 static int t_radet_gn_workspace_floats(const uint64_t* a) { return radet_gn_workspace_floats((int)(int64_t)a[0], (void*)(uintptr_t)a[1], (int)(int64_t)a[2]); }
 static int t_radet_grid_anchors(const uint64_t* a) { return radet_grid_anchors((void*)(uintptr_t)a[0], (void*)(uintptr_t)a[1], (int)(int64_t)a[2], (int)(int64_t)a[3], (void*)(uintptr_t)a[4]); }
 static int t_radet_head_loss(const uint64_t* a) { return radet_head_loss((void*)(uintptr_t)a[0], (void*)(uintptr_t)a[1], (void*)(uintptr_t)a[2], (void*)(uintptr_t)a[3], (void*)(uintptr_t)a[4], (void*)(uintptr_t)a[5], (void*)(uintptr_t)a[6], (void*)(uintptr_t)a[7], (void*)(uintptr_t)a[8], (void*)(uintptr_t)a[9], (int)(int64_t)a[10], (int)(int64_t)a[11], (int)(int64_t)a[12], f32(a[13]), f32(a[14]), f32(a[15]), f32(a[16]), (void*)(uintptr_t)a[17], (void*)(uintptr_t)a[18], (void*)(uintptr_t)a[19], (int)(int64_t)a[20], (void*)(uintptr_t)a[21], (int)(int64_t)a[22], (void*)(uintptr_t)a[23], (int)(int64_t)a[24], (void*)(uintptr_t)a[25], (void*)(uintptr_t)a[26], (void*)(uintptr_t)a[27], (int)(int64_t)a[28], (void*)(uintptr_t)a[29], (void*)(uintptr_t)a[30]); }
+static int t_radet_head_loss_a(const uint64_t* a) { return radet_head_loss_a((void*)(uintptr_t)a[0], (void*)(uintptr_t)a[1], (void*)(uintptr_t)a[2], (void*)(uintptr_t)a[3], (void*)(uintptr_t)a[4], (void*)(uintptr_t)a[5], (void*)(uintptr_t)a[6], (void*)(uintptr_t)a[7], (void*)(uintptr_t)a[8], (void*)(uintptr_t)a[9], (int)(int64_t)a[10], (int)(int64_t)a[11], (int)(int64_t)a[12], f32(a[13]), f32(a[14]), f32(a[15]), f32(a[16]), (void*)(uintptr_t)a[17], (void*)(uintptr_t)a[18], (void*)(uintptr_t)a[19], (int)(int64_t)a[20], (void*)(uintptr_t)a[21], (int)(int64_t)a[22], (void*)(uintptr_t)a[23], (int)(int64_t)a[24], (void*)(uintptr_t)a[25], (void*)(uintptr_t)a[26], (void*)(uintptr_t)a[27], (int)(int64_t)a[28], (void*)(uintptr_t)a[29], (void*)(uintptr_t)a[30]); }
+static int t_radet_head_loss_prepare(const uint64_t* a) { return radet_head_loss_prepare((void*)(uintptr_t)a[0], (void*)(uintptr_t)a[1], (void*)(uintptr_t)a[2], (void*)(uintptr_t)a[3], (void*)(uintptr_t)a[4], (void*)(uintptr_t)a[5], (int)(int64_t)a[6], (int)(int64_t)a[7], (int)(int64_t)a[8], (void*)(uintptr_t)a[9], (void*)(uintptr_t)a[10], (void*)(uintptr_t)a[11], (void*)(uintptr_t)a[12]); }
 static int t_radet_head_loss_ws_ints(const uint64_t* a) { return radet_head_loss_ws_ints((int)(int64_t)a[0]); }
 static int t_radet_jpeg_decode(const uint64_t* a) { return radet_jpeg_decode((void*)(uintptr_t)a[0], (void*)(uintptr_t)a[1], (int)(int64_t)a[2], (void*)(uintptr_t)a[3], (int)(int64_t)a[4], (void*)(uintptr_t)a[5], (void*)(uintptr_t)a[6], (void*)(uintptr_t)a[7], (int)(int64_t)a[8], (void*)(uintptr_t)a[9], (void*)(uintptr_t)a[10], (void*)(uintptr_t)a[11], (void*)(uintptr_t)a[12], (int)(int64_t)a[13], (int)(int64_t)a[14], (int)(int64_t)a[15], (void*)(uintptr_t)a[16]); }
 static int t_radet_jpeg_index(const uint64_t* a) { return radet_jpeg_index((void*)(uintptr_t)a[0], (int)(int64_t)a[1], (int)(int64_t)a[2], (int)(int64_t)a[3], (void*)(uintptr_t)a[4], (void*)(uintptr_t)a[5], (int)(int64_t)a[6], (int)(int64_t)a[7], (int)(int64_t)a[8], (void*)(uintptr_t)a[9], (int)(int64_t)a[10]); }
@@ -177,6 +179,8 @@
     {"radet_gn_workspace_floats", t_radet_gn_workspace_floats, 3},
     {"radet_grid_anchors", t_radet_grid_anchors, 5},
     {"radet_head_loss", t_radet_head_loss, 31},
+    {"radet_head_loss_a", t_radet_head_loss_a, 31},
+    {"radet_head_loss_prepare", t_radet_head_loss_prepare, 13},
     {"radet_head_loss_ws_ints", t_radet_head_loss_ws_ints, 1},
     {"radet_jpeg_decode", t_radet_jpeg_decode, 17},
     {"radet_jpeg_index", t_radet_jpeg_index, 11},
@@ -235,4 +239,4 @@
     {"radet_upsample_add_h", t_radet_upsample_add_h, 9},
     {"radet_warp_affine_u8", t_radet_warp_affine_u8, 9},
 };
-const int radet_tape_nthunks = 113;
+const int radet_tape_nthunks = 115;
diff --git a/radet_amd/engine.py b/radet_amd/engine.py
--- a/radet_amd/engine.py
+++ b/radet_amd/engine.py
@@ -699,6 +699,7 @@
 
     def backbone_forward(self, img):
         b = self.buf
+        self._issue_loss_prepare()
         self._img = img if self.stem.trainable else None
         if self.h2:
             K.fill_zero(self.amax_act)
@@ -1022,21 +1023,69 @@
             return torch.as_strided(ts[0], (len(ts),), (1,))
         return torch.stack([t.reshape(()) for t in ts]).contiguous()
 
+    _loss_prepared = None
+    _prep_targets = None
+
+    def loss_prepare_async(self, gt_boxes, gt_labels, gt_off, p2g, pw):
+        if K.serial_fuse() and self.use_streams:
+            self._prep_targets = (gt_boxes, gt_labels, gt_off, p2g, pw)
+
+    def _issue_loss_prepare(self):
+        tg, self._prep_targets = self._prep_targets, None
+        if tg is None:
+            return
+        side = self._side()
+        self._fork(side)
+        if self._prep_event is None:
+            self._prep_event = torch.cuda.Event()
+        with torch.cuda.stream(side):
+            K.head_loss_prepare(*tg, self.ldesc, self.nlvl, self.B, self.num_classes, self.loss_ws)
+            K.ev_record(self._prep_event)
+        self._loss_prepared = (self._prep_event, self.loss_ws.data_ptr(), tg[3].data_ptr())
+
+    _prep_event = None
+
+    def _scale_grads_inplace(self):
+        ts = [self.g[f"bbox_head.scales.{i}.scale"] for i in range(len(self.strides))]
+        base = ts[0].data_ptr()
+        if all(t.data_ptr() == base + 4 * i for i, t in enumerate(ts)):
+            return torch.as_strided(ts[0], (len(ts),), (1,))
+        return None
+
     def loss(self, gt_boxes, gt_labels, gt_off, p2g, pw, grad_scale=None, alpha=0.25, gamma=2.0, lbw=2.0,
-             labels_out=None, tgt_out=None):
+             labels_out=None, tgt_out=None, scale_grads_inplace=False):
         b = self.buf
         dri = b["dregiou"]
-        K.head_loss(b["cls"], b["reg_u"], b["iou"], self.scales_tensor(), gt_boxes, gt_labels, gt_off, p2g, pw, self.ldesc,
-                    self.nlvl, self.B, self.num_classes, alpha, gamma, lbw, 1e-6, grad_scale, self.losses, b["dcls"],
-                    self.cls_pad, dri, 16, dri.view(-1)[4:], 16, self.dscales, self.loss_ws, labels_out, tgt_out)
-        if self.h2:
-            K.absmax(b["dcls"], K.amax_slot(b["dcls"]))
-            K.absmax(dri, K.amax_slot(dri))
+        prep, self._loss_prepared = self._loss_prepared, None
+        self._dscales_inplace = False
+        if K.serial_fuse():
+            if prep is not None:
+                K.ev_wait(prep[0])
+            if prep is None or prep[1:] != (self.loss_ws.data_ptr(), p2g.data_ptr()) or labels_out is not None or tgt_out is not None:
+                K.head_loss_prepare(gt_boxes, gt_labels, gt_off, p2g, pw, self.ldesc, self.nlvl, self.B, self.num_classes,
+                                    self.loss_ws, labels_out, tgt_out)
+            ds = self._scale_grads_inplace() if scale_grads_inplace else None
+            self._dscales_inplace = ds is not None
+            K.head_loss_a(b["cls"], b["reg_u"], b["iou"], self.scales_tensor(), gt_boxes, gt_labels, gt_off, p2g, pw,
+                          self.ldesc, self.nlvl, self.B, self.num_classes, alpha, gamma, lbw, 1e-6, grad_scale, self.losses,
+                          b["dcls"], self.cls_pad, dri, 16, dri.view(-1)[4:], 16, ds if ds is not None else self.dscales,
+                          self.loss_ws, K.amax_slot(b["dcls"]) if self.h2 else None, K.amax_slot(dri) if self.h2 else None)
+        else:
+            if prep is not None:
+                K.ev_wait(prep[0])
+            K.head_loss(b["cls"], b["reg_u"], b["iou"], self.scales_tensor(), gt_boxes, gt_labels, gt_off, p2g, pw, self.ldesc,
+                        self.nlvl, self.B, self.num_classes, alpha, gamma, lbw, 1e-6, grad_scale, self.losses, b["dcls"],
+                        self.cls_pad, dri, 16, dri.view(-1)[4:], 16, self.dscales, self.loss_ws, labels_out, tgt_out)
+            if self.h2:
+                K.absmax(b["dcls"], K.amax_slot(b["dcls"]))
+                K.absmax(dri, K.amax_slot(dri))
         if self.h16:
             K.convert_rows(b["dcls"], b["dcls16"])
             K.convert_rows(dri, b["dregiou16"], ncols=4)
             K.convert_rows(dri, b["dregiou16"], ncols=1, src_off=4, dst_off=self.iou_col)
         return self.losses
+
+    _dscales_inplace = False
 
     def _head_grads(self):
         b = self.buf
@@ -1206,6 +1255,8 @@
         return dP
 
     def _write_scale_grads(self):
+        if self._dscales_inplace:
+            return
         g = self.g
         ts = [g[f"bbox_head.scales.{i}.scale"] for i in range(len(self.strides))]
         base = ts[0].data_ptr()
diff --git a/radet_amd/kernels.py b/radet_amd/kernels.py
--- a/radet_amd/kernels.py
+++ b/radet_amd/kernels.py
@@ -1026,6 +1026,10 @@
     _lib.call("radet_unfold_grads", _ptr(table_dev), n, max_cout, _stream())
 
 
+def serial_fuse():
+    return os.environ.get("RADET_SERIAL_FUSE", "1") != "0"
+
+
 def _h(name, t):
     return name + "_h" if _is16(t) else name
 
@@ -1200,6 +1204,20 @@
               _ptr(gt_off), _ptr(p2g), _ptr(pw), ldesc, nlvl, B, num_classes, alpha, gamma, lbw, giou_eps,
               _ptr(grad_scale), _ptr(losses), _ptr(dcls), dcls_ld, _ptr(dreg), dreg_ld, _ptr(diou), diou_ld,
               _ptr(dscales), _ptr(labels_out), _ptr(tgt_out), flags, _ptr(ws), _stream())
+
+
+def head_loss_prepare(gt_boxes, gt_labels, gt_off, p2g, pw, ldesc, nlvl, B, num_classes, ws, labels_out=None, tgt_out=None):
+    _lib.call("radet_head_loss_prepare", _ptr(gt_boxes), _ptr(gt_labels), _ptr(gt_off), _ptr(p2g), _ptr(pw), ldesc, nlvl, B,
+              num_classes, _ptr(labels_out), _ptr(tgt_out), _ptr(ws), _stream())
+
+
+def head_loss_a(cls, reg_u, iou, scales, gt_boxes, gt_labels, gt_off, p2g, pw, ldesc, nlvl, B, num_classes, alpha, gamma,
+                lbw, giou_eps, grad_scale, losses, dcls, dcls_ld, dreg, dreg_ld, diou, diou_ld, dscales, ws,
+                dcls_amax=None, dri_amax=None, flags=0):
+    _lib.call("radet_head_loss_a", _ptr(cls), _ptr(reg_u), _ptr(iou), _ptr(scales), _ptr(gt_boxes), _ptr(gt_labels),
+              _ptr(gt_off), _ptr(p2g), _ptr(pw), ldesc, nlvl, B, num_classes, alpha, gamma, lbw, giou_eps,
+              _ptr(grad_scale), _ptr(losses), _ptr(dcls), dcls_ld, _ptr(dreg), dreg_ld, _ptr(diou), diou_ld,
+              _ptr(dscales), _ptr(dcls_amax), _ptr(dri_amax), flags, _ptr(ws), _stream())
 
 
 def scale_relu(reg_u, scales, out, ldesc, nlvl, B):
diff --git a/radet_amd/runtime.py b/radet_amd/runtime.py
--- a/radet_amd/runtime.py
+++ b/radet_amd/runtime.py
@@ -288,10 +288,10 @@
         self.loss_weights = None if (wc == 1.0 and wi == 1.0) else torch.tensor([wc, 1.0, wi], device=self.dev)
         return self
 
-    def loss(self, tg, grad_scale=None, labels_out=None, tgt_out=None):
+    def loss(self, tg, grad_scale=None, labels_out=None, tgt_out=None, scale_grads_inplace=False):
         hp = self.loss_hparams or dict(alpha=0.25, gamma=2.0, lbw=2.0)
         return self.engine.loss(tg["boxes"], tg["labels"], tg["off"], tg["p2g"], tg["pw"], grad_scale=grad_scale,
-                                labels_out=labels_out, tgt_out=tgt_out, **hp)
+                                labels_out=labels_out, tgt_out=tgt_out, scale_grads_inplace=scale_grads_inplace, **hp)
 
     def backward(self, bucket_hook=None, next_img=None):
         e = self.engine
@@ -416,7 +416,7 @@
         return (e.geo_key, getattr(e, "plan_id", None), tuple(img.shape), img.dtype, tuple(tg["p2g"].shape), int(tg["off"].numel()),
                 world, use_reducer, self.loss_weights is None or self.loss_weights.data_ptr(),
                 st["betas"], st["eps"], st["wd"], st["max_norm"], st["m"].data_ptr(), e.wgrad_streams, e.use_streams,
-                tuple(sorted(self.loss_hparams.items())) if self.loss_hparams else None)
+                tuple(sorted(self.loss_hparams.items())) if self.loss_hparams else None, K.serial_fuse())
 
     def drop_tape(self):
         self._tape = None
@@ -458,8 +458,10 @@
             torch.cuda.current_stream().synchronize()
             record.begin(self.dev)
         try:
+            if tg is not None:
+                e.loss_prepare_async(tg["boxes"], tg["labels"], tg["off"], tg["p2g"], tg["pw"])
             self.forward(img)
-            self.loss(tg, grad_scale=self.loss_weights)
+            self.loss(tg, grad_scale=self.loss_weights, scale_grads_inplace=True)
             if use_reducer:
                 if self.reducer is None:
                     on_chain = self.engine.use_streams and self.flat.grads.is_cuda
```

New measurement: 505.7, median of 6. About the same (+0.3%).
